# HipGraph/iSpLib

Hardware: AMD Instinct MI355X
Metric: edges_aggregated_per_sec (higher is better)
Workload: dtype f32

## Files before the change

include/isplib_hip.h:

```cpp
#ifndef ISPLIB_HIP_H
#define ISPLIB_HIP_H

#include <stddef.h>
#include <stdint.h>

#ifdef __cplusplus
extern "C" {
#endif

#define ISPLIB_HIP_ABI_VERSION 1
#define ISPLIB_MAX_SLICES 4096

#define ISPLIB_VOP_COPY_RHS 0x2
#define ISPLIB_ROP_NOOP     0x00
#define ISPLIB_SOP_COPY     0x100
#define ISPLIB_VSC_MUL      0x1000
#define ISPLIB_VSC_MEAN     0x3000
#define ISPLIB_AOP_ADD      0x10000
#define ISPLIB_AOP_MAX      0x20000
#define ISPLIB_AOP_MIN      0x30000
#define ISPLIB_MSG_SPMM_SUM  (ISPLIB_VOP_COPY_RHS | ISPLIB_ROP_NOOP | ISPLIB_SOP_COPY | ISPLIB_VSC_MUL  | ISPLIB_AOP_ADD)
#define ISPLIB_MSG_SPMM_MEAN (ISPLIB_VOP_COPY_RHS | ISPLIB_ROP_NOOP | ISPLIB_SOP_COPY | ISPLIB_VSC_MEAN | ISPLIB_AOP_ADD)
#define ISPLIB_MSG_SPMM_MAX  (ISPLIB_VOP_COPY_RHS | ISPLIB_ROP_NOOP | ISPLIB_SOP_COPY | ISPLIB_VSC_MUL  | ISPLIB_AOP_MAX)
#define ISPLIB_MSG_SPMM_MIN  (ISPLIB_VOP_COPY_RHS | ISPLIB_ROP_NOOP | ISPLIB_SOP_COPY | ISPLIB_VSC_MUL  | ISPLIB_AOP_MIN)
// ... 37 lines not shown
          (k % 2) == 0 && (ldy % 2) == 0 && (ldz % 2) == 0;
}
#define ISPLIB_MINMAX_BW_PAIRS_END     0xFFFFFFFEu
#define ISPLIB_MINMAX_BW_KEYS_MAX      0xFFFFFFFEu
#define ISPLIB_OWNER_WORLD_MAX         64
static inline int isplib_product_within(int64_t rows, int64_t k, uint64_t most) {
   return rows <= 0 || k <= 0 || (uint64_t)k <= most / (uint64_t)rows;
}
static inline int isplib_owner_exchange_serves(int64_t m, int64_t k, int world, const int64_t *cuts) {
   if (world < 1 || world > ISPLIB_OWNER_WORLD_MAX || m < 0 || k < 0 || !isplib_product_within(m, k, ISPLIB_MINMAX_BW_PAIRS_END - 1u)) return 0;
   for (int p = 0; p < world; p++)
      if (cuts[p + 1] < cuts[p] || !isplib_product_within(cuts[p + 1] - cuts[p], k, ISPLIB_MINMAX_BW_KEYS_MAX)) return 0;
   return 1;
}

int isplib_hip_set_empty_row(int init);
int isplib_hip_get_empty_row(void);

int fusedMM_csr_hip(int32_t imessage, int64_t m, int64_t n, int64_t k,
                    float alpha, int64_t nnz, int64_t rows, int64_t cols,
                    const float *val ,
                    const int64_t *indx ,
                    const int64_t *pntrb ,
                    const int64_t *pntre ,
                    const float *x , int64_t ldx,
                    const float *y , int64_t ldy, float beta,
                    float *z , int64_t ldz,
                    int64_t *z_arg , void *stream);

enum isplib_sop_udef {
   ISPLIB_SOP_NONE = 0,
   ISPLIB_SOP_SIGMOID = 1,
   ISPLIB_SOP_ONE_MINUS_SIGMOID = 2,
   ISPLIB_SOP_TDIST = 3,
   ISPLIB_SOP_SCALE = 4,
   ISPLIB_SOP_EXP = 5,
   ISPLIB_SOP_LEAKY_EXP = 6
};
int fusedMM_csr_udef_hip(int32_t imessage, int64_t m, int64_t n, int64_t k, float alpha, int64_t nnz,
                         int64_t rows, int64_t cols, const float *val ,
                         const int64_t *indx, const int64_t *pntrb, const int64_t *pntre,
                         const float *x , int64_t ldx,
                         const float *y , int64_t ldy, float beta,
                         float *z , int64_t ldz, int64_t *z_arg ,
                         int sop_udef , float sop_param, void *stream);

int fusedMM_csr_udef_tasks_hip(int32_t imessage, int64_t m, int64_t n, int64_t k, int64_t nnz,
                               const float *val, const int64_t *indx, const int32_t *indx32 ,
                               const int64_t *pntrb, const int64_t *pntre,
                               const float *x, int64_t ldx, int64_t n_tasks, const int32_t *task_row,
                               const int64_t *task_b, const int32_t *task_len, const int32_t *seg_off,
                               int slices, const int64_t *lane_off_host ,
                               const float *y, int64_t ldy, float *z, int64_t ldz, int64_t *z_arg,
                               int sop_udef, float sop_param, void *workspace, size_t workspace_bytes,
                               void *stream);

size_t isplib_spmm_slices_bytes(int64_t m, int slices);
int    isplib_spmm_slices_build_hip(int64_t m, int64_t n, int64_t nnz,
                                    const int64_t *pntrb, const int64_t *pntre,
                                    const int64_t *indx, int slices,
                                    int64_t *sliceptr ,
                                    int32_t *unsorted_flag ,
                                    void *stream);
size_t isplib_spmm_sliced_workspace_bytes(int32_t imessage, int64_t m, int64_t k, int slices);
int    fusedMM_csr_sliced_hip(int32_t imessage, int64_t m, int64_t n, int64_t k,
                              int64_t nnz, const float *val, const int64_t *indx,
                              const int64_t *pntrb, const int64_t *pntre,
                              const int64_t *sliceptr, int slices,
                              const float *y, int64_t ldy, float *z, int64_t ldz,
                              int64_t *z_arg, void *workspace,
                              size_t workspace_bytes, void *stream);

int    fusedMM_csr_sliced_phase_hip(int32_t imessage, int64_t m, int64_t n, int64_t k,
                                    int64_t nnz, const float *val, const int64_t *indx,
                                    const int64_t *pntrb, const int64_t *pntre,
                                    const int64_t *sliceptr, int slices,
                                    int slice_first, int slice_count, int combine,
                                    const float *y, int64_t ldy, float *z, int64_t ldz,
                                    int64_t *z_arg, void *workspace,
                                    size_t workspace_bytes, void *stream);

typedef struct isplib_task_plan_info {
   int64_t n_tasks;
   int64_t lane_off[9];
   int32_t slices, chunk, short_row, reserved;
} isplib_task_plan_info;

size_t isplib_spmm_tasks_plan_workspace_bytes(int64_t m, int slices);
int    isplib_spmm_tasks_count_hip(int64_t m, const int64_t *pntrb, const int64_t *pntre,
                                   const int64_t *sliceptr, int slices, int chunk, int short_row,
                                   int32_t *seg_off , void *workspace,
                                   size_t workspace_bytes, isplib_task_plan_info *info ,
                                   void *stream);
int    isplib_spmm_tasks_fill_hip(int64_t m, const int64_t *pntrb, const int64_t *pntre,
                                  const int64_t *sliceptr, const isplib_task_plan_info *info,
                                  const int32_t *seg_off, int32_t *task_row, int64_t *task_b,
                                  int32_t *task_len, void *stream);
size_t isplib_spmm_tasks_workspace_bytes(int32_t imessage, int64_t n_tasks, int64_t k);
int    isplib_pack_indices_hip(int64_t nnz, const int64_t *indx, int32_t *indx32, void *stream);
int    fusedMM_csr_tasks_hip(int32_t imessage, int64_t m, int64_t n, int64_t k, int64_t nnz,
                             const float *val, const int64_t *indx, const int32_t *indx32,
                             const int64_t *pntrb, const int64_t *pntre,
                             int64_t n_tasks, const int32_t *task_row,
                             const int64_t *task_b, const int32_t *task_len,
                             const int32_t *seg_off, int slices,
                             const int64_t *lane_off_host ,
                             const float *y, int64_t ldy, float *z, int64_t ldz,
                             int64_t *z_arg, void *workspace, size_t workspace_bytes,
                             void *stream);

typedef struct isplib_epilogue {
   const float *row_scale;
   const float *self;
   int64_t      ld_self;
   const float *bias;
   int          relu;
} isplib_epilogue;
int    fusedMM_csr_tasks_epilogue_hip(int32_t imessage, int64_t m, int64_t n, int64_t k, int64_t nnz,
                                      const float *val, const int64_t *indx, const int32_t *indx32,
                                      const int64_t *pntrb, const int64_t *pntre,
                                      int64_t n_tasks, const int32_t *task_row,
                                      const int64_t *task_b, const int32_t *task_len,
                                      const int32_t *seg_off, int slices,
                                      const int64_t *lane_off_host ,
                                      const float *y, int64_t ldy, float *z, int64_t ldz,
                                      void *workspace, size_t workspace_bytes,
                                      const isplib_epilogue *epilogue ,
                                      void *stream);

int    isplib_row_scale_hip(int64_t n, int64_t k, const float *x , int64_t ldx, const float *scale ,
                            float *y , int64_t ldy, void *stream);
size_t isplib_masked_scale_colsum_workspace_bytes(int64_t n, int64_t k);
int    isplib_masked_scale_colsum_hip(int64_t n, int64_t k, const float *dz, int64_t lddz, const float *out ,
                                      int64_t ldo, const float *scale , float *gy ,
                                      int64_t ldgy, float *grad_bias , void *workspace, size_t workspace_bytes,
                                      void *stream);

typedef struct isplib_stream_plan {
   int64_t rows, cols;
   int32_t slices, gens, waves_per_gen, rows_per_wave, streams , chunk ;
   int64_t n_steps, n_parts, n_hub;
   const int32_t *words;
   const float   *vals;
   const int64_t *wave_step_off;
   const int32_t *wave_row;
   const int32_t *wave_part;
   const int32_t *hub_row;
   const int32_t *hub_off;
   const int32_t *perm;
} isplib_stream_plan;
int  isplib_stream_plan_build_hip(int64_t m, int64_t n, int64_t nnz, const int64_t *rowptr, const int64_t *col,
                                  const float *val, int streams, int slices, int chunk, int waves_per_gen,
                                  isplib_stream_plan *out , void *stream);
int  isplib_stream_plan_set_values_hip(isplib_stream_plan *plan, const float *val , void *stream);
void isplib_stream_plan_free(isplib_stream_plan *plan);
int    isplib_spmm_stream_geometry(int streams, int *rows_per_wave , int *waves_resident );
int    isplib_suggest_stream(int64_t m, int64_t n, int64_t nnz, int64_t k, int *streams, int *slices, int *chunk);
int    isplib_suggest_stream_weighted(int64_t m, int64_t n, int64_t nnz, int64_t k, int weighted, int *streams, int *slices, int *chunk);
int    isplib_spmm_stream_minmax_geometry(int streams , int *rows_per_wave , int *waves_resident );
int    isplib_suggest_stream_minmax(int64_t m, int64_t n, int64_t nnz, int64_t k, int *streams, int *slices, int *chunk);
int    isplib_stream_plan_build_minmax_hip(int64_t m, int64_t n, int64_t nnz, const int64_t *rowptr, const int64_t *col,
                                           const float *val, int streams, int slices, int chunk, int waves_per_gen,
                                           isplib_stream_plan *out , void *stream);
size_t isplib_spmm_stream_minmax_workspace_bytes(const isplib_stream_plan *plan);
int    fusedMM_csr_stream_minmax_hip(int32_t imessage , int64_t m, int64_t n, int64_t k,
                                     int64_t nnz, const int64_t *pntrb, const int64_t *pntre,
                                     const isplib_stream_plan *plan ,
                                     const float *y, int64_t ldy, float *z, int64_t ldz, int64_t *z_arg,
                                     void *workspace, size_t workspace_bytes, void *stream);
size_t isplib_spmm_stream_workspace_bytes(const isplib_stream_plan *plan);
int    fusedMM_csr_stream_hip(int32_t imessage , int64_t m, int64_t n, int64_t k,
                              int64_t nnz, const int64_t *pntrb, const int64_t *pntre,
                              const isplib_stream_plan *plan ,
                              const float *y, int64_t ldy, float *z, int64_t ldz,
                              void *workspace, size_t workspace_bytes,
                              const isplib_epilogue *epilogue , void *stream);
#define ISPLIB_DTYPE_BF16 1
#define ISPLIB_DTYPE_F16  2
int    fusedMM_csr_stream16_hip(int32_t imessage , int dtype, int64_t m, int64_t n, int64_t k,
                                int64_t nnz, const int64_t *pntrb, const int64_t *pntre,
                                const isplib_stream_plan *plan ,
                                const void *y, int64_t ldy, void *z, int64_t ldz,
                                void *workspace, size_t workspace_bytes, void *stream);
static inline int isplib_stream16_native_pays(int streams, int weighted) {
   (void)streams; (void)weighted;
   return 0;
}
int    isplib_stream16_auto(int streams, int weighted);
int    fusedMM_csr_rows16_hip(int32_t imessage , int dtype ,
                              int64_t m, int64_t n, int64_t k, int64_t nnz, const float *val ,
                              const int64_t *indx, const int64_t *pntrb, const int64_t *pntre,
                              const int32_t *row_order , const void *y, int64_t ldy, void *z, int64_t ldz, void *stream);
static inline int isplib_rows16_native_pays(int64_t n, int64_t ldy, int ordered, int weighted) {
   const int beyond = n > 0 && ldy > 0 && (double)n * (double)ldy * 2.0 > 256.0 * 1048576.0;
   (void)weighted;
   return (beyond || !ordered) ? 1 : 0;
}
int    isplib_rows16_auto(int64_t n, int64_t ldy, int ordered, int weighted);
int    isplib_rows16_domain(int64_t n, int64_t k, int64_t ldy, int64_t ldz);
int    fusedMM_csr_rows16_colscale_hip(int32_t imessage , int dtype ,
                                       int64_t m, int64_t n, int64_t k, int64_t nnz, const float *col_scale ,
                                       const int64_t *indx, const int64_t *pntrb, const int64_t *pntre,
                                       const int32_t *row_order , const void *y, int64_t ldy, void *z, int64_t ldz, void *stream);
static inline int isplib_rows16_colscale_native_pays(int64_t n, int64_t ldy, int ordered) {
   const int beyond = n > 0 && ldy > 0 && (double)n * (double)ldy * 2.0 > 256.0 * 1048576.0;
   return (beyond || !ordered) ? 1 : 0;
}
int    isplib_rows16_colscale_auto(int64_t n, int64_t ldy, int ordered);
typedef struct isplib_epilogue16 {
   const float *row_scale;
   const float *self_scale;
   const float *bias;
   int          relu;
} isplib_epilogue16;
int    fusedMM_csr_rows16_epilogue_hip(int dtype , int64_t m, int64_t n, int64_t k, int64_t nnz,
                                       const float *col_scale , const int64_t *indx, const int64_t *pntrb,
                                       const int64_t *pntre, const int32_t *row_order , const void *y, int64_t ldy, void *z,
                                       int64_t ldz, const isplib_epilogue16 *epilogue , void *stream);
static inline int isplib_rows16_gcn_native_pays(int64_t n, int64_t ldy, int ordered) {
   (void)ordered;
   return (n > 0 && ldy > 0 && (double)n * (double)ldy * 2.0 > 256.0 * 1048576.0) ? 1 : 0;
}
int    isplib_rows16_gcn_auto(int64_t n, int64_t ldy, int ordered);
size_t isplib_masked_colsum16_workspace_bytes(int64_t n, int64_t k);
int    isplib_masked_colsum16_hip(int dtype, int64_t n, int64_t k, const void *dz, int64_t lddz, const void *out , int64_t ldo,
                                  void *g , int64_t ldg, float *grad_bias , void *workspace,
                                  size_t workspace_bytes, void *stream);
int    fusedMM_csr_rows16_minmax_hip(int32_t imessage , int dtype ,
                                     int64_t m, int64_t n, int64_t k, int64_t nnz, const float *val ,
                                     const int64_t *indx, const int64_t *pntrb, const int64_t *pntre,
                                     const int32_t *row_order , const void *y, int64_t ldy, void *z, int64_t ldz,
                                     int64_t *z_arg , int64_t ldarg, void *stream);
static inline int isplib_rows16_minmax_native_pays(int64_t n, int64_t ldy, int ordered, int weighted, int want_arg) {
   const int beyond = n > 0 && ldy > 0 && (double)n * (double)ldy * 2.0 > 256.0 * 1048576.0;
   (void)ordered; (void)weighted; (void)want_arg;
   return beyond ? 1 : 0;
}
int    isplib_rows16_minmax_auto(int64_t n, int64_t ldy, int ordered, int weighted, int want_arg);
int    isplib_sddmm_csr_rows16_hip(int dtype , int64_t m, int64_t n, int64_t k, int64_t nnz,
                                   const int64_t *indx, const int64_t *pntrb, const int64_t *pntre,
                                   const int32_t *row_order , const void *y, int64_t ldy,
                                   const void *g, int64_t ldg, int mean, float *dval, void *stream);
static inline int isplib_sddmm_rows16_serves(int64_t n, int64_t k, int64_t ldy, int64_t ldg) {
   return k <= ISPLIB_SDDMM_TASKS_K_MAX && isplib_rows16_serves(n, k, ldy, ldg);
}
static inline int isplib_sddmm_rows16_native_pays(int64_t n, int64_t ldy, int ordered) {
   const int beyond = n > 0 && ldy > 0 && (double)n * (double)ldy * 2.0 > 256.0 * 1048576.0;
   (void)ordered;
   return beyond ? 1 : 0;
}
int    isplib_sddmm_rows16_auto(int64_t n, int64_t ldy, int ordered);
static inline int isplib_attention_serves(int64_t rows_gathered, int64_t k, int64_t ld) {
   return k >= 1 && k <= ISPLIB_ATTENTION_K_MAX && ld >= k && rows_gathered < (1LL << 31) && isplib_dense_in_descriptor(rows_gathered, ld);
}
int    isplib_attention_domain(int64_t rows_gathered, int64_t k, int64_t ld);
int    isplib_attention_csr_hip(int64_t m, int64_t n, int64_t k, int64_t nnz, const int64_t *indx, const int64_t *pntrb,
                                const int64_t *pntre, const float *x, int64_t ldx, const float *y, int64_t ldy, float scale,
                                float *z, int64_t ldz, float *lse , void *stream);
int    isplib_attention_bw_rows_hip(int64_t m, int64_t n, int64_t k, int64_t nnz, const int64_t *indx, const int64_t *pntrb,
                                    const int64_t *pntre, const float *x, int64_t ldx, const float *y, int64_t ldy, float scale,
                                    const float *g, int64_t ldg, const float *z, int64_t ldz, const float *lse, float *dx,
                                    int64_t lddx, float *dsum , void *stream);
int    isplib_attention_bw_cols_hip(int64_t m, int64_t n, int64_t k, int64_t nnz, const int64_t *row_t, const int64_t *colb,
                                    const int64_t *cole, const float *x, int64_t ldx, const float *y, int64_t ldy, float scale,
                                    const float *g, int64_t ldg, const float *lse, const float *dsum, float *dy, int64_t lddy,
                                    void *stream);
#define ISPLIB_ATTENTION16_K_MIN       8
#define ISPLIB_ATTENTION16_K_MAX       512
static inline int isplib_attention16_serves(int64_t rows_gathered, int64_t k, int64_t ld) {
   return k >= ISPLIB_ATTENTION16_K_MIN && k <= ISPLIB_ATTENTION16_K_MAX && (k % 2) == 0 && (ld % 2) == 0 && ld >= k &&
          rows_gathered < (1LL << 31) && isplib_rows_within(rows_gathered, ld, 2ull * ISPLIB_DENSE_BYTES_MAX);
}
int    isplib_attention16_domain(int64_t rows_gathered, int64_t k, int64_t ld);
int    isplib_attention16_csr_hip(int dtype , int64_t m, int64_t n, int64_t k, int64_t nnz,
                                  const int64_t *indx, const int64_t *pntrb, const int64_t *pntre, const void *x, int64_t ldx,
                                  const void *y, int64_t ldy, float scale, void *z, int64_t ldz, float *lse , void *stream);
int    isplib_attention16_bw_rows_hip(int dtype, int64_t m, int64_t n, int64_t k, int64_t nnz, const int64_t *indx, const int64_t *pntrb,
                                      const int64_t *pntre, const void *x, int64_t ldx, const void *y, int64_t ldy, float scale,
                                      const void *g, int64_t ldg, const float *lse, void *dx, int64_t lddx, float *dsum ,
                                      void *stream);
int    isplib_attention16_bw_cols_hip(int dtype, int64_t m, int64_t n, int64_t k, int64_t nnz, const int64_t *row_t, const int64_t *colb,
                                      const int64_t *cole, const void *x, int64_t ldx, const void *y, int64_t ldy, float scale,
                                      const void *g, int64_t ldg, const float *lse, const float *dsum, void *dy, int64_t lddy,
                                      void *stream);
static inline int isplib_attention16_native_pays(int64_t rows_gathered, int64_t ld) {
   return (rows_gathered > 0 && ld > 0) ? 1 : 0;
}
int    isplib_attention16_auto(int64_t rows_gathered, int64_t ld);
#define ISPLIB_STAGE_OFF   0
#define ISPLIB_STAGE_FORCE 1
#define ISPLIB_STAGE_AUTO  2
#define ISPLIB_STREAM_STAGE_PITCH      512
#define ISPLIB_STREAM_STAGE_BYTES_MAX  (1u << 30)
#define ISPLIB_STREAM_STAGE_MIN_DEGREE 128
static inline int isplib_stream_stage_panel(uint64_t y_addr, int64_t ldy, int64_t c0, int64_t k, int streams, int64_t n, int64_t nnz,
                                            uint64_t room_bytes, int mode) {
   const uint64_t addr = y_addr + 4u * (uint64_t)c0;
   if (mode == ISPLIB_STAGE_OFF || streams != 4 || n <= 0 || c0 < 0 || c0 + 64 > k) return 0;
   if (((uint64_t)ldy * 4u) % ISPLIB_STREAM_STAGE_PITCH != 0 || (addr & 255u) != 0) return 0;
   if ((uint64_t)n > ISPLIB_STREAM_STAGE_BYTES_MAX / ISPLIB_STREAM_STAGE_PITCH || (uint64_t)n * ISPLIB_STREAM_STAGE_PITCH > room_bytes) return 0;
   if (mode == ISPLIB_STAGE_FORCE) return 1;
   if ((addr & 256u) == 0 || ((((uint64_t)ldy * 4u) % 1024u) == 0 && (addr & 512u) != 0)) return 0;
   return nnz / n >= ISPLIB_STREAM_STAGE_MIN_DEGREE;
}

int    isplib_fusedmm_stream_geometry(int streams, int *rows_per_wave , int *waves_resident );
// ... 102 lines not shown
```

isplib_amd/cabi.py:

```python
from __future__ import annotations

import ctypes
import os
from typing import Optional

import torch

from . import _lib

MSG_SPMM_SUM = 0x2 | 0x00 | 0x100 | 0x1000 | 0x10000
MSG_SPMM_MEAN = 0x2 | 0x00 | 0x100 | 0x3000 | 0x10000
MSG_SPMM_MAX = 0x2 | 0x00 | 0x100 | 0x1000 | 0x20000
MSG_SPMM_MIN = 0x2 | 0x00 | 0x100 | 0x1000 | 0x30000
MESSAGE = {"sum": MSG_SPMM_SUM, "add": MSG_SPMM_SUM, "mean": MSG_SPMM_MEAN, "max": MSG_SPMM_MAX, "min": MSG_SPMM_MIN}

SUCCESS, FAIL, NOT_ENOUGH_MEM, NO_OPT_IMPL, HIP_ERROR = 0, 1, -1, 128, 256
UNDEFINED_USER_FUNCTION = 64
ISPLIB_SUCCESS, ISPLIB_FAIL, ISPLIB_NOT_ENOUGH_MEM, ISPLIB_NO_OPT_IMPL, ISPLIB_HIP_ERROR = SUCCESS, FAIL, NOT_ENOUGH_MEM, NO_OPT_IMPL, HIP_ERROR

DENSE_BYTES_MAX = 7 * 2 ** 29
DENSE_OOB_OFFSET = 15 * 2 ** 28
STREAM_N_END = 2 ** 24
STREAM_LDY_END = 2 ** 22
STREAM_NNZ_END = 2 ** 31
STREAM_MINMAX_BYTES_END = 2 ** 31
K_MIN = 4
SDDMM_TASKS_K_MAX = 1024
MINMAX_BW_PAIRS_END = 2 ** 32 - 2
MINMAX_BW_KEYS_MAX = 2 ** 32 - 2
OWNER_WORLD_MAX = 64
DTYPE_BF16, DTYPE_F16 = 1, 2


def stream16_serves(n: int, k: int, ldy: int, ldz: int, nnz: int) -> bool:
    return (k >= K_MIN and n < STREAM_N_END and ldy < STREAM_LDY_END and nnz < STREAM_NNZ_END and
            (n <= 0 or n * ldy * 2 <= DENSE_BYTES_MAX) and k % 2 == 0 and ldy % 2 == 0 and ldz % 2 == 0)


def stream16_native_pays(streams: int, weighted: bool) -> bool:
    return False


ROWS16_K_MIN, ROWS16_K_END = 8, 2 ** 24


def rows16_serves(n: int, k: int, ldy: int, ldz: int) -> bool:
    return (ROWS16_K_MIN <= k < ROWS16_K_END and n < 2 ** 31 and (n <= 0 or n * ldy * 2 <= DENSE_BYTES_MAX) and
            k % 2 == 0 and ldy % 2 == 0 and ldz % 2 == 0)


def rows16_native_pays(n: int, ldy: int, ordered: bool, weighted: bool) -> bool:
    beyond = n > 0 and ldy > 0 and n * ldy * 2 > (256 << 20)
    return bool(beyond or not ordered)


def rows16_minmax_native_pays(n: int, ldy: int, ordered: bool, weighted: bool, want_arg: bool) -> bool:
    return bool(n > 0 and ldy > 0 and n * ldy * 2 > (256 << 20))


def rows16_colscale_native_pays(n: int, ldy: int, ordered: bool) -> bool:
    beyond = n > 0 and ldy > 0 and n * ldy * 2 > (256 << 20)
    return bool(beyond or not ordered)


def rows16_gcn_native_pays(n: int, ldy: int, ordered: bool) -> bool:
    return bool(n > 0 and ldy > 0 and n * ldy * 2 > (256 << 20))


def sddmm_rows16_serves(n: int, k: int, ldy: int, ldg: int) -> bool:
    return k <= SDDMM_TASKS_K_MAX and rows16_serves(n, k, ldy, ldg)


def sddmm_rows16_native_pays(n: int, ldy: int, ordered: bool) -> bool:
    return bool(n > 0 and ldy > 0 and n * ldy * 2 > (256 << 20))


ATTENTION_K_MAX = 512


def attention_serves(rows_gathered: int, k: int, ld: int) -> bool:
    return (1 <= k <= ATTENTION_K_MAX and ld >= k and rows_gathered < 2 ** 31 and
            (rows_gathered <= 0 or rows_gathered * ld * 4 <= DENSE_BYTES_MAX))


ATTENTION16_K_MIN, ATTENTION16_K_MAX = 8, 512


def attention16_serves(rows_gathered: int, k: int, ld: int) -> bool:
    return (ATTENTION16_K_MIN <= k <= ATTENTION16_K_MAX and k % 2 == 0 and ld % 2 == 0 and ld >= k and rows_gathered < 2 ** 31 and
            (rows_gathered <= 0 or rows_gathered * ld * 2 <= DENSE_BYTES_MAX))


def attention16_native_pays(rows_gathered: int, ld: int) -> bool:
    return bool(rows_gathered > 0 and ld > 0)


def owner_exchange_serves(m: int, k: int, world: int, cuts) -> bool:
    if not 1 <= world <= OWNER_WORLD_MAX or m < 0 or k < 0 or m * k >= MINMAX_BW_PAIRS_END:
        return False
    return all(cuts[p + 1] >= cuts[p] and (cuts[p + 1] - cuts[p]) * k <= MINMAX_BW_KEYS_MAX for p in range(world))


def scatter_keys_serves(total: int, n: int, k: int) -> bool:
    return 0 <= total < MINMAX_BW_PAIRS_END and n >= 0 and k >= 0 and n * k <= MINMAX_BW_KEYS_MAX

VOP = {"copy_lhs": 0x1, "copy_rhs": 0x2, "add": 0x3, "subl": 0x4, "subr": 0x5, "max": 0x6, "min": 0x7, "udef": 0xF}
ROP = {"noop": 0x00, "dot": 0x10, "add_lhs": 0x20, "add_rhs": 0x30, "norml": 0x40, "normr": 0x50, "udef": 0xF0}
SOP = {"noop": 0x000, "copy": 0x100, "udef": 0xF00}
VSC = {"noop": 0x0000, "mul": 0x1000, "add": 0x2000, "mean": 0x3000, "udef": 0xF000}
AOP = {"add": 0x10000, "max": 0x20000, "min": 0x30000, "udef": 0xF0000}
SOP_UDEF = {"none": 0, "sigmoid": 1, "one_minus_sigmoid": 2, "tdist": 3, "scale": 4, "exp": 5, "leaky_exp": 6}
PATTERNS = {
    "spmm": (MSG_SPMM_SUM, "none"),
    "sigmoid_embedding": (VOP["copy_rhs"] | ROP["dot"] | SOP["udef"] | VSC["mul"] | AOP["add"], "sigmoid"),
    "tdist_embedding": (VOP["subr"] | ROP["normr"] | SOP["udef"] | VSC["mul"] | AOP["add"], "tdist"),
    "attention_sum": (VOP["copy_rhs"] | ROP["dot"] | SOP["udef"] | VSC["mul"] | AOP["add"], "leaky_exp"),
}

EXPORTS = (
    "isplib_hip_abi_version", "isplib_hip_last_error", "isplib_hip_set_empty_row", "isplib_hip_get_empty_row", "fusedMM_csr_hip", "performDummySpMM_hip",
    "isplib_spmm_minmax_bw_hip", "isplib_sddmm_csr_hip", "isplib_csr_row_ids_hip",
    "isplib_csr2csc_workspace_bytes", "isplib_csr2csc_hip",
    "isplib_spmm_slices_bytes", "isplib_spmm_slices_build_hip", "isplib_spmm_sliced_workspace_bytes",
    "fusedMM_csr_sliced_hip", "fusedMM_csr_sliced_phase_hip", "isplib_hip_tune",
    "isplib_spmm_tasks_workspace_bytes", "fusedMM_csr_tasks_hip",
    "isplib_spmm_tasks_plan_workspace_bytes", "isplib_spmm_tasks_count_hip", "isplib_spmm_tasks_fill_hip",
    "isplib_sddmm_csr_tasks_hip", "fusedMM_csr_tasks_epilogue_hip", "fusedMM_csr_udef_hip", "fusedMM_csr_udef_tasks_hip", "isplib_pack_indices_hip",
    "isplib_suggest_slices", "isplib_graph_create", "isplib_graph_set_slices", "isplib_graph_set_values", "isplib_graph_spmm", "isplib_graph_spmm_backward",
    "isplib_graph_destroy", "isplib_suggest_slices_whole_rows", "isplib_graph_sddmm",
    "fusedMM_csr_stream_hip", "isplib_spmm_stream_workspace_bytes", "isplib_spmm_stream_geometry", "isplib_suggest_stream", "isplib_suggest_stream_weighted", "isplib_stream_plan_build_hip", "isplib_stream_plan_build_minmax_hip", "fusedMM_csr_stream_minmax_hip", "isplib_spmm_stream_minmax_geometry", "isplib_suggest_stream_minmax", "isplib_spmm_stream_minmax_workspace_bytes", "isplib_stream_plan_set_values_hip", "isplib_stream_plan_free", "isplib_spmm_minmax_bw_det_hip", "isplib_spmm_minmax_bw_workspace_bytes", "isplib_scatter_rows_det_hip",
    "isplib_minmax_bw_bucket_workspace_bytes", "isplib_minmax_bw_bucket_hip", "isplib_scatter_keys_workspace_bytes", "isplib_scatter_keys_det_hip",
    "isplib_fusedmm_stream_geometry", "isplib_suggest_fusedmm_stream", "isplib_stream_plan_build_fusedmm_hip", "fusedMM_csr_udef_stream_hip",
    "isplib_row_scale_hip", "isplib_masked_scale_colsum_hip", "isplib_masked_scale_colsum_workspace_bytes",
    "fusedMM_csr_ordered_hip", "isplib_community_order_hip", "isplib_community_order_workspace_bytes", "isplib_order_locality_hip",
    "isplib_graph_set_row_order", "isplib_plain_panels",
    "fusedMM_csr_stream16_hip", "isplib_stream16_auto",
    "fusedMM_csr_rows16_hip", "isplib_rows16_auto", "isplib_rows16_domain",
    "fusedMM_csr_rows16_minmax_hip", "isplib_rows16_minmax_auto",
    "fusedMM_csr_rows16_colscale_hip", "isplib_rows16_colscale_auto",
    "fusedMM_csr_rows16_epilogue_hip", "isplib_rows16_gcn_auto", "isplib_masked_colsum16_hip", "isplib_masked_colsum16_workspace_bytes",
    "isplib_sddmm_csr_rows16_hip", "isplib_sddmm_rows16_auto",
    "isplib_attention_csr_hip", "isplib_attention_bw_rows_hip", "isplib_attention_bw_cols_hip", "isplib_attention_domain",
    "isplib_attention16_csr_hip", "isplib_attention16_bw_rows_hip", "isplib_attention16_bw_cols_hip", "isplib_attention16_domain",
    "isplib_attention16_auto",
)

EXP_EXPORTS = ("fusedMM_csr_sweep_hip", "isplib_spmm_sweep_workspace_bytes", "isplib_spmm_sweep_resident_waves",
               "fusedMM_csr_hybrid_hip", "isplib_spmm_hybrid_geometry", "isplib_spmm_hybrid_workspace_bytes", "isplib_sddmm_stream_hip",
               "isplib_hip_tune_experimental")

_i64, _f32, _vp, _i32 = ctypes.c_int64, ctypes.c_float, ctypes.c_void_p, ctypes.c_int32


class Epilogue(ctypes.Structure):
    _fields_ = [("row_scale", ctypes.c_void_p), ("self", ctypes.c_void_p), ("ld_self", ctypes.c_int64),
                ("bias", ctypes.c_void_p), ("relu", ctypes.c_int)]


class TaskPlanInfo(ctypes.Structure):
    _fields_ = [("n_tasks", ctypes.c_int64), ("lane_off", ctypes.c_int64 * 9), ("slices", ctypes.c_int32),
                ("chunk", ctypes.c_int32), ("short_row", ctypes.c_int32), ("reserved", ctypes.c_int32)]


class SweepPlanStruct(ctypes.Structure):
    _fields_ = [("rows", ctypes.c_int64), ("slices", ctypes.c_int32), ("gens", ctypes.c_int32),
                ("waves_per_gen", ctypes.c_int32), ("rows_per_wave", ctypes.c_int32), ("n_tasks", ctypes.c_int64),
                ("n_parts", ctypes.c_int64), ("n_hub", ctypes.c_int64), ("wave_row", ctypes.c_void_p),
                ("wave_part", ctypes.c_void_p), ("wave_task_off", ctypes.c_void_p), ("task_b", ctypes.c_void_p),
                ("task_meta", ctypes.c_void_p), ("hub_row", ctypes.c_void_p), ("hub_off", ctypes.c_void_p)]


class StreamPlanStruct(ctypes.Structure):
    _fields_ = [("rows", ctypes.c_int64), ("cols", ctypes.c_int64), ("slices", ctypes.c_int32), ("gens", ctypes.c_int32),
                ("waves_per_gen", ctypes.c_int32), ("rows_per_wave", ctypes.c_int32), ("streams", ctypes.c_int32),
                ("chunk", ctypes.c_int32), ("n_steps", ctypes.c_int64), ("n_parts", ctypes.c_int64), ("n_hub", ctypes.c_int64),
                ("words", ctypes.c_void_p), ("vals", ctypes.c_void_p), ("wave_step_off", ctypes.c_void_p),
                ("wave_row", ctypes.c_void_p), ("wave_part", ctypes.c_void_p),
                ("hub_row", ctypes.c_void_p), ("hub_off", ctypes.c_void_p), ("perm", ctypes.c_void_p)]


class HybridPlanStruct(ctypes.Structure):
    _fields_ = [("cold", StreamPlanStruct), ("table_rows", ctypes.c_int32), ("hot_cap", ctypes.c_int32), ("n_hot_steps", ctypes.c_int64),
                ("hot_rows", ctypes.c_void_p), ("hot_words", ctypes.c_void_p), ("hot_step_off", ctypes.c_void_p),
                ("hot_perm", ctypes.c_void_p)]


_sigs_set = False


def lib() -> ctypes.CDLL:
    global _sigs_set
    L = _lib.cdll()
    if not _sigs_set:
        L.isplib_hip_abi_version.restype = ctypes.c_int
        L.isplib_hip_last_error.restype = ctypes.c_char_p
        L.fusedMM_csr_hip.restype = ctypes.c_int
        L.fusedMM_csr_hip.argtypes = [_i32, _i64, _i64, _i64, _f32, _i64, _i64, _i64, _vp, _vp, _vp, _vp,
                                      _vp, _i64, _vp, _i64, _f32, _vp, _i64, _vp, _vp]
        L.fusedMM_csr_udef_hip.restype = ctypes.c_int
        L.fusedMM_csr_udef_hip.argtypes = [_i32, _i64, _i64, _i64, _f32, _i64, _i64, _i64, _vp, _vp, _vp, _vp,
                                           _vp, _i64, _vp, _i64, _f32, _vp, _i64, _vp, ctypes.c_int, _f32, _vp]
        L.fusedMM_csr_udef_tasks_hip.restype = ctypes.c_int
        L.fusedMM_csr_udef_tasks_hip.argtypes = [_i32, _i64, _i64, _i64, _i64, _vp, _vp, _vp, _vp, _vp, _vp, _i64, _i64, _vp, _vp,
                                                 _vp, _vp, ctypes.c_int, _vp, _vp, _i64, _vp, _i64, _vp, ctypes.c_int, _f32,
                                                 _vp, ctypes.c_size_t, _vp]
        L.performDummySpMM_hip.restype = None
        L.performDummySpMM_hip.argtypes = [_i64, _vp]
        L.isplib_spmm_minmax_bw_hip.restype = ctypes.c_int
        L.isplib_spmm_minmax_bw_hip.argtypes = [_i64, _i64, _i64, _i64, _vp, _vp, _vp, _vp, _vp, _vp, _vp, _vp]
        L.isplib_sddmm_csr_hip.restype = ctypes.c_int
        L.isplib_sddmm_csr_hip.argtypes = [_i64, _i64, _vp, _vp, _vp, _vp, _i64, _vp, _i64, ctypes.c_int, _vp, _vp]
        L.isplib_csr_row_ids_hip.restype = ctypes.c_int
        L.isplib_csr_row_ids_hip.argtypes = [_i64, _i64, _vp, _vp, _vp]
        L.isplib_csr2csc_workspace_bytes.restype = ctypes.c_size_t
        L.isplib_csr2csc_workspace_bytes.argtypes = [_i64, _i64, _i64]
        L.isplib_csr2csc_hip.restype = ctypes.c_int
        L.isplib_csr2csc_hip.argtypes = [_i64, _i64, _i64, _vp, _vp, _vp, ctypes.c_int, _vp, _vp, _vp, _vp,
                                         _vp, ctypes.c_size_t, _vp]
        L.isplib_spmm_slices_bytes.restype = ctypes.c_size_t
        L.isplib_spmm_slices_bytes.argtypes = [_i64, ctypes.c_int]
        L.isplib_spmm_slices_build_hip.restype = ctypes.c_int
        L.isplib_spmm_slices_build_hip.argtypes = [_i64, _i64, _i64, _vp, _vp, _vp, ctypes.c_int, _vp, _vp, _vp]
        L.isplib_spmm_sliced_workspace_bytes.restype = ctypes.c_size_t
        L.isplib_spmm_sliced_workspace_bytes.argtypes = [_i32, _i64, _i64, ctypes.c_int]
        L.fusedMM_csr_sliced_hip.restype = ctypes.c_int
        L.fusedMM_csr_sliced_hip.argtypes = [_i32, _i64, _i64, _i64, _i64, _vp, _vp, _vp, _vp, _vp, ctypes.c_int,
                                             _vp, _i64, _vp, _i64, _vp, _vp, ctypes.c_size_t, _vp]
        L.fusedMM_csr_sliced_phase_hip.restype = ctypes.c_int
        L.fusedMM_csr_sliced_phase_hip.argtypes = [_i32, _i64, _i64, _i64, _i64, _vp, _vp, _vp, _vp, _vp, ctypes.c_int,
                                                   ctypes.c_int, ctypes.c_int, ctypes.c_int, _vp, _i64, _vp, _i64, _vp,
                                                   _vp, ctypes.c_size_t, _vp]
        L.isplib_spmm_tasks_workspace_bytes.restype = ctypes.c_size_t
        L.isplib_spmm_tasks_workspace_bytes.argtypes = [_i32, _i64, _i64]
        L.fusedMM_csr_tasks_hip.restype = ctypes.c_int
        L.isplib_pack_indices_hip.restype = ctypes.c_int
        L.isplib_pack_indices_hip.argtypes = [_i64, _vp, _vp, _vp]
        L.fusedMM_csr_tasks_hip.argtypes = [_i32, _i64, _i64, _i64, _i64, _vp, _vp, _vp, _vp, _vp, _i64, _vp, _vp, _vp, _vp,
                                            ctypes.c_int, _vp, _vp, _i64, _vp, _i64, _vp, _vp, ctypes.c_size_t, _vp]
        L.isplib_spmm_tasks_plan_workspace_bytes.restype = ctypes.c_size_t
        L.isplib_spmm_tasks_plan_workspace_bytes.argtypes = [_i64, ctypes.c_int]
        L.isplib_spmm_tasks_count_hip.restype = ctypes.c_int
        L.isplib_spmm_tasks_count_hip.argtypes = [_i64, _vp, _vp, _vp, ctypes.c_int, ctypes.c_int, ctypes.c_int, _vp, _vp,
                                                  ctypes.c_size_t, ctypes.POINTER(TaskPlanInfo), _vp]
        L.isplib_spmm_tasks_fill_hip.restype = ctypes.c_int
        L.isplib_spmm_tasks_fill_hip.argtypes = [_i64, _vp, _vp, _vp, ctypes.POINTER(TaskPlanInfo), _vp, _vp, _vp, _vp, _vp]
        L.isplib_sddmm_csr_tasks_hip.restype = ctypes.c_int
        L.isplib_sddmm_csr_tasks_hip.argtypes = [_i64, _i64, _i64, _vp, _vp, _vp, _vp, _i64, _vp, _vp, _vp, _vp, _vp, _i64, _vp,
                                                 _i64, ctypes.c_int, _vp, _vp]
        L.fusedMM_csr_tasks_epilogue_hip.restype = ctypes.c_int
        L.fusedMM_csr_tasks_epilogue_hip.argtypes = [_i32, _i64, _i64, _i64, _i64, _vp, _vp, _vp, _vp, _vp, _i64, _vp, _vp, _vp, _vp,
                                                     ctypes.c_int, _vp, _vp, _i64, _vp, _i64, _vp, ctypes.c_size_t,
                                                     ctypes.POINTER(Epilogue), _vp]
        L.isplib_suggest_slices.restype = ctypes.c_int
        L.isplib_suggest_slices.argtypes = [_i64, _i64, _i64, _i64, ctypes.c_int]
        L.isplib_graph_create.restype = ctypes.c_int
        L.isplib_graph_create.argtypes = [_i64, _i64, _i64, _vp, _vp, _vp, ctypes.POINTER(_vp)]
        L.isplib_graph_set_slices.restype = ctypes.c_int
        L.isplib_graph_set_slices.argtypes = [_vp, ctypes.c_int]
        L.isplib_graph_set_values.restype = ctypes.c_int
        L.isplib_graph_set_values.argtypes = [_vp, _vp]
        L.isplib_graph_spmm.restype = ctypes.c_int
        L.isplib_graph_spmm.argtypes = [_vp, _i32, _i64, _vp, _i64, _vp, _i64, _vp, _vp]
        L.isplib_graph_spmm_backward.restype = ctypes.c_int
        L.isplib_graph_spmm_backward.argtypes = [_vp, ctypes.c_int, _i64, _vp, _i64, _vp, _i64, _vp]
        L.isplib_suggest_slices_whole_rows.restype = ctypes.c_int
        L.isplib_suggest_slices_whole_rows.argtypes = [_i64, _i64, _i64, _i64]
        L.isplib_graph_sddmm.restype = ctypes.c_int
        L.isplib_graph_sddmm.argtypes = [_vp, ctypes.c_int, _i64, _vp, _i64, _vp, _i64, _vp, _vp]
        L.isplib_graph_destroy.restype = None
        L.isplib_graph_destroy.argtypes = [_vp]
        L.isplib_hip_tune.restype = ctypes.c_int
        L.isplib_hip_tune.argtypes = [ctypes.c_int, ctypes.c_int]
        L.isplib_spmm_minmax_bw_workspace_bytes.restype = ctypes.c_size_t
        L.isplib_spmm_minmax_bw_workspace_bytes.argtypes = [_i64, _i64, _i64]
        L.isplib_spmm_minmax_bw_det_hip.restype = ctypes.c_int
        L.isplib_spmm_minmax_bw_det_hip.argtypes = [_i64, _i64, _i64, _i64, _vp, _vp, _vp, _vp, _vp, _vp, _vp, _vp, ctypes.c_size_t, _vp]
        L.isplib_fusedmm_stream_geometry.restype = ctypes.c_int
        L.isplib_fusedmm_stream_geometry.argtypes = [ctypes.c_int, ctypes.POINTER(ctypes.c_int), ctypes.POINTER(ctypes.c_int)]
        L.isplib_suggest_fusedmm_stream.restype = ctypes.c_int
        L.isplib_suggest_fusedmm_stream.argtypes = [_i32, _i64, _i64, _i64, _i64] + [ctypes.POINTER(ctypes.c_int)] * 3
        L.isplib_stream_plan_build_fusedmm_hip.restype = ctypes.c_int
        L.isplib_stream_plan_build_fusedmm_hip.argtypes = [_i64, _i64, _i64, _vp, _vp, ctypes.c_int, ctypes.c_int, ctypes.c_int, ctypes.c_int,
                                                           ctypes.POINTER(StreamPlanStruct), _vp]
        L.fusedMM_csr_udef_stream_hip.restype = ctypes.c_int
        L.fusedMM_csr_udef_stream_hip.argtypes = [_i32, _i64, _i64, _i64, _i64, _vp, _vp, ctypes.POINTER(StreamPlanStruct), _vp, _i64, _vp, _i64,
                                                  _vp, _i64, ctypes.c_int, _f32, _vp, ctypes.c_size_t, _vp]
        L.isplib_row_scale_hip.restype = ctypes.c_int
        L.isplib_row_scale_hip.argtypes = [_i64, _i64, _vp, _i64, _vp, _vp, _i64, _vp]
        L.isplib_masked_scale_colsum_workspace_bytes.restype = ctypes.c_size_t
        L.isplib_masked_scale_colsum_workspace_bytes.argtypes = [_i64, _i64]
        L.isplib_masked_scale_colsum_hip.restype = ctypes.c_int
        L.isplib_masked_scale_colsum_hip.argtypes = [_i64, _i64, _vp, _i64, _vp, _i64, _vp, _vp, _i64, _vp, _vp, ctypes.c_size_t, _vp]
        L.isplib_scatter_rows_det_hip.restype = ctypes.c_int
        L.isplib_scatter_rows_det_hip.argtypes = [_i64, _i64, _i64, _i64, _vp, _vp, _vp, _vp, ctypes.c_size_t, _vp]
        L.isplib_minmax_bw_bucket_workspace_bytes.restype = ctypes.c_size_t
        L.isplib_minmax_bw_bucket_workspace_bytes.argtypes = [_i64, _i64, ctypes.c_int]
        L.isplib_minmax_bw_bucket_hip.restype = ctypes.c_int
        L.isplib_minmax_bw_bucket_hip.argtypes = [_i64, _i64, _i64, _i64, _vp, _vp, _vp, _vp, ctypes.c_int, ctypes.POINTER(_i64), _vp, _vp, _vp,
                                                  _vp, ctypes.c_size_t, _vp]
        L.isplib_scatter_keys_workspace_bytes.restype = ctypes.c_size_t
        L.isplib_scatter_keys_workspace_bytes.argtypes = [_i64, _i64, _i64]
        L.isplib_scatter_keys_det_hip.restype = ctypes.c_int
        L.isplib_scatter_keys_det_hip.argtypes = [_i64, _i64, _i64, _vp, _vp, _vp, _vp, ctypes.c_size_t, _vp]
        L.isplib_stream_plan_build_hip.restype = ctypes.c_int
        L.isplib_stream_plan_build_hip.argtypes = [_i64, _i64, _i64, _vp, _vp, _vp, ctypes.c_int, ctypes.c_int, ctypes.c_int, ctypes.c_int,
                                                   ctypes.POINTER(StreamPlanStruct), _vp]
        L.isplib_stream_plan_build_minmax_hip.restype = ctypes.c_int
        L.isplib_stream_plan_build_minmax_hip.argtypes = [_i64, _i64, _i64, _vp, _vp, _vp, ctypes.c_int, ctypes.c_int, ctypes.c_int, ctypes.c_int,
                                                          ctypes.POINTER(StreamPlanStruct), _vp]
        L.isplib_spmm_stream_minmax_geometry.restype = ctypes.c_int
        L.isplib_spmm_stream_minmax_geometry.argtypes = [ctypes.c_int, ctypes.POINTER(ctypes.c_int), ctypes.POINTER(ctypes.c_int)]
        L.isplib_suggest_stream_minmax.restype = ctypes.c_int
        L.isplib_suggest_stream_minmax.argtypes = [_i64, _i64, _i64, _i64, ctypes.POINTER(ctypes.c_int), ctypes.POINTER(ctypes.c_int), ctypes.POINTER(ctypes.c_int)]
        L.isplib_spmm_stream_minmax_workspace_bytes.restype = ctypes.c_size_t
        L.isplib_spmm_stream_minmax_workspace_bytes.argtypes = [ctypes.POINTER(StreamPlanStruct)]
        L.fusedMM_csr_stream_minmax_hip.restype = ctypes.c_int
        L.fusedMM_csr_stream_minmax_hip.argtypes = [_i32, _i64, _i64, _i64, _i64, _vp, _vp, ctypes.POINTER(StreamPlanStruct), _vp, _i64,
                                                    _vp, _i64, _vp, _vp, ctypes.c_size_t, _vp]
        L.isplib_stream_plan_set_values_hip.restype = ctypes.c_int
        L.isplib_stream_plan_set_values_hip.argtypes = [ctypes.POINTER(StreamPlanStruct), _vp, _vp]
        L.isplib_stream_plan_free.restype = None
        L.isplib_stream_plan_free.argtypes = [ctypes.POINTER(StreamPlanStruct)]
        L.isplib_community_order_workspace_bytes.restype = ctypes.c_size_t
        L.isplib_community_order_workspace_bytes.argtypes = [_i64, _i64]
        L.isplib_community_order_hip.restype = ctypes.c_int
        L.isplib_community_order_hip.argtypes = [_i64, _i64, _vp, _vp, ctypes.c_int, ctypes.c_int, _vp, _vp, ctypes.POINTER(ctypes.c_int), _vp,
                                                 ctypes.c_size_t, _vp]
        L.isplib_order_locality_hip.restype = ctypes.c_int
        L.isplib_order_locality_hip.argtypes = [_i64, _i64, _vp, _vp, _vp, _i64, ctypes.POINTER(ctypes.c_double), _vp, ctypes.c_size_t, _vp]
        L.isplib_graph_set_row_order.restype = ctypes.c_int
        L.isplib_graph_set_row_order.argtypes = [_vp, _vp, _vp]
        L.fusedMM_csr_ordered_hip.restype = ctypes.c_int
        L.fusedMM_csr_ordered_hip.argtypes = [_i32, _i64, _i64, _i64, _i64, _vp, _vp, _vp, _vp, _vp, _vp, _i64, _vp, _i64, _vp, _vp]
        L.isplib_plain_panels.restype = ctypes.c_int
        L.isplib_plain_panels.argtypes = [_i64, _i64]
        L.isplib_suggest_stream.restype = ctypes.c_int
        L.isplib_suggest_stream.argtypes = [_i64, _i64, _i64, _i64, ctypes.POINTER(ctypes.c_int), ctypes.POINTER(ctypes.c_int), ctypes.POINTER(ctypes.c_int)]
        L.isplib_suggest_stream_weighted.restype = ctypes.c_int
        L.isplib_suggest_stream_weighted.argtypes = [_i64, _i64, _i64, _i64, ctypes.c_int, ctypes.POINTER(ctypes.c_int), ctypes.POINTER(ctypes.c_int), ctypes.POINTER(ctypes.c_int)]
        L.isplib_spmm_stream_geometry.restype = ctypes.c_int
        L.isplib_spmm_stream_geometry.argtypes = [ctypes.c_int, ctypes.POINTER(ctypes.c_int), ctypes.POINTER(ctypes.c_int)]
        L.isplib_spmm_stream_workspace_bytes.restype = ctypes.c_size_t
        L.isplib_spmm_stream_workspace_bytes.argtypes = [ctypes.POINTER(StreamPlanStruct)]
        L.fusedMM_csr_stream_hip.restype = ctypes.c_int
        L.fusedMM_csr_stream_hip.argtypes = [_i32, _i64, _i64, _i64, _i64, _vp, _vp, ctypes.POINTER(StreamPlanStruct), _vp, _i64,
                                             _vp, _i64, _vp, ctypes.c_size_t, ctypes.POINTER(Epilogue), _vp]
        L.fusedMM_csr_stream16_hip.restype = ctypes.c_int
        L.fusedMM_csr_stream16_hip.argtypes = [_i32, ctypes.c_int, _i64, _i64, _i64, _i64, _vp, _vp, ctypes.POINTER(StreamPlanStruct), _vp, _i64,
                                               _vp, _i64, _vp, ctypes.c_size_t, _vp]
        L.isplib_stream16_auto.restype = ctypes.c_int
        L.isplib_stream16_auto.argtypes = [ctypes.c_int, ctypes.c_int]
        L.fusedMM_csr_rows16_hip.restype = ctypes.c_int
        L.fusedMM_csr_rows16_hip.argtypes = [_i32, ctypes.c_int, _i64, _i64, _i64, _i64, _vp, _vp, _vp, _vp, _vp, _vp, _i64, _vp, _i64, _vp]
        L.isplib_rows16_auto.restype = ctypes.c_int
        L.isplib_rows16_auto.argtypes = [_i64, _i64, ctypes.c_int, ctypes.c_int]
        L.isplib_rows16_domain.restype = ctypes.c_int
        L.isplib_rows16_domain.argtypes = [_i64, _i64, _i64, _i64]
        L.fusedMM_csr_rows16_minmax_hip.restype = ctypes.c_int
        L.fusedMM_csr_rows16_minmax_hip.argtypes = [_i32, ctypes.c_int, _i64, _i64, _i64, _i64, _vp, _vp, _vp, _vp, _vp, _vp, _i64, _vp, _i64, _vp, _i64, _vp]
        L.isplib_rows16_minmax_auto.restype = ctypes.c_int
        L.isplib_rows16_minmax_auto.argtypes = [_i64, _i64, ctypes.c_int, ctypes.c_int, ctypes.c_int]
        L.fusedMM_csr_rows16_colscale_hip.restype = ctypes.c_int
        L.fusedMM_csr_rows16_colscale_hip.argtypes = [_i32, ctypes.c_int, _i64, _i64, _i64, _i64, _vp, _vp, _vp, _vp, _vp, _vp, _i64, _vp, _i64, _vp]
        L.isplib_rows16_colscale_auto.restype = ctypes.c_int
        L.isplib_rows16_colscale_auto.argtypes = [_i64, _i64, ctypes.c_int]
        L.fusedMM_csr_rows16_epilogue_hip.restype = ctypes.c_int
        L.fusedMM_csr_rows16_epilogue_hip.argtypes = [ctypes.c_int, _i64, _i64, _i64, _i64, _vp, _vp, _vp, _vp, _vp, _vp, _i64, _vp, _i64, _vp, _vp]
        L.isplib_rows16_gcn_auto.restype = ctypes.c_int
        L.isplib_rows16_gcn_auto.argtypes = [_i64, _i64, ctypes.c_int]
        L.isplib_masked_colsum16_workspace_bytes.restype = ctypes.c_size_t
        L.isplib_masked_colsum16_workspace_bytes.argtypes = [_i64, _i64]
        L.isplib_masked_colsum16_hip.restype = ctypes.c_int
        L.isplib_masked_colsum16_hip.argtypes = [ctypes.c_int, _i64, _i64, _vp, _i64, _vp, _i64, _vp, _i64, _vp, _vp, ctypes.c_size_t, _vp]
        L.isplib_sddmm_csr_rows16_hip.restype = ctypes.c_int
        L.isplib_sddmm_csr_rows16_hip.argtypes = [ctypes.c_int, _i64, _i64, _i64, _i64, _vp, _vp, _vp, _vp, _vp, _i64, _vp, _i64, ctypes.c_int, _vp, _vp]
        L.isplib_sddmm_rows16_auto.restype = ctypes.c_int
        L.isplib_sddmm_rows16_auto.argtypes = [_i64, _i64, ctypes.c_int]
        L.isplib_attention_domain.restype = ctypes.c_int
        L.isplib_attention_domain.argtypes = [_i64, _i64, _i64]
        L.isplib_attention_csr_hip.restype = ctypes.c_int
        L.isplib_attention_csr_hip.argtypes = [_i64, _i64, _i64, _i64, _vp, _vp, _vp, _vp, _i64, _vp, _i64, _f32, _vp, _i64, _vp, _vp]
        L.isplib_attention_bw_rows_hip.restype = ctypes.c_int
        L.isplib_attention_bw_rows_hip.argtypes = [_i64, _i64, _i64, _i64, _vp, _vp, _vp, _vp, _i64, _vp, _i64, _f32, _vp, _i64, _vp, _i64, _vp,
                                                   _vp, _i64, _vp, _vp]
        L.isplib_attention_bw_cols_hip.restype = ctypes.c_int
        L.isplib_attention_bw_cols_hip.argtypes = [_i64, _i64, _i64, _i64, _vp, _vp, _vp, _vp, _i64, _vp, _i64, _f32, _vp, _i64, _vp, _vp, _vp,
                                                   _i64, _vp]
        L.isplib_attention16_domain.restype = ctypes.c_int
        L.isplib_attention16_domain.argtypes = [_i64, _i64, _i64]
        L.isplib_attention16_auto.restype = ctypes.c_int
        L.isplib_attention16_auto.argtypes = [_i64, _i64]
        L.isplib_attention16_csr_hip.restype = ctypes.c_int
        L.isplib_attention16_csr_hip.argtypes = [ctypes.c_int, _i64, _i64, _i64, _i64, _vp, _vp, _vp, _vp, _i64, _vp, _i64, _f32, _vp, _i64, _vp, _vp]
        L.isplib_attention16_bw_rows_hip.restype = ctypes.c_int
        L.isplib_attention16_bw_rows_hip.argtypes = [ctypes.c_int, _i64, _i64, _i64, _i64, _vp, _vp, _vp, _vp, _i64, _vp, _i64, _f32, _vp, _i64, _vp,
                                                     _vp, _i64, _vp, _vp]
        L.isplib_attention16_bw_cols_hip.restype = ctypes.c_int
        L.isplib_attention16_bw_cols_hip.argtypes = [ctypes.c_int, _i64, _i64, _i64, _i64, _vp, _vp, _vp, _vp, _i64, _vp, _i64, _f32, _vp, _i64, _vp,
                                                     _vp, _vp, _i64, _vp]
        _sigs_set = True
    return L


_exp = None


def exp_lib() -> ctypes.CDLL:
    global _exp
    if _exp is None:
        lib()
        path = os.path.join(os.path.dirname(_lib.CABI_PATH), "libisplib_hip_exp.so")
        if not os.path.exists(path):
            raise ImportError(f"isplib_amd: '{os.path.basename(path)}' not found; build it with `make -C isplib_amd/csrc`")
        L = ctypes.CDLL(path, mode=ctypes.RTLD_GLOBAL)
        L.isplib_hip_tune_experimental.restype = ctypes.c_int
        L.isplib_hip_tune_experimental.argtypes = [ctypes.c_int, ctypes.c_int]
        L.isplib_spmm_hybrid_geometry.restype = ctypes.c_int
        L.isplib_spmm_hybrid_geometry.argtypes = [ctypes.c_int] + [ctypes.POINTER(ctypes.c_int)] * 4
        L.isplib_spmm_hybrid_workspace_bytes.restype = ctypes.c_size_t
        L.isplib_spmm_hybrid_workspace_bytes.argtypes = [ctypes.POINTER(HybridPlanStruct)]
        L.fusedMM_csr_hybrid_hip.restype = ctypes.c_int
        L.fusedMM_csr_hybrid_hip.argtypes = [_i32, _i64, _i64, _i64, _i64, _vp, _vp, ctypes.POINTER(HybridPlanStruct), _vp, _i64, _vp, _i64,
                                             _vp, ctypes.c_size_t, _vp, _vp]
        L.isplib_sddmm_stream_hip.restype = ctypes.c_int
        L.isplib_sddmm_stream_hip.argtypes = [_i64, _i64, _i64, _i64, _vp, _vp, ctypes.POINTER(StreamPlanStruct), _vp, _i64, _vp, _i64,
                                              ctypes.c_int, _vp, _vp]
        L.isplib_spmm_sweep_resident_waves.restype = ctypes.c_int
        L.isplib_spmm_sweep_resident_waves.argtypes = [_i32, _i64, ctypes.c_int]
        L.isplib_spmm_sweep_workspace_bytes.restype = ctypes.c_size_t
        L.isplib_spmm_sweep_workspace_bytes.argtypes = [_i32, ctypes.POINTER(SweepPlanStruct), _i64]
        L.fusedMM_csr_sweep_hip.restype = ctypes.c_int
        L.fusedMM_csr_sweep_hip.argtypes = [_i32, _i64, _i64, _i64, _i64, _vp, _vp, _vp, _vp, _vp, ctypes.POINTER(SweepPlanStruct),
                                            _vp, _i64, _vp, _i64, _vp, _vp, ctypes.c_size_t, ctypes.POINTER(Epilogue), _vp]
        _exp = L
    return _exp


def last_error() -> str:
    return lib().isplib_hip_last_error().decode()


class IsplibError(RuntimeError):

    def __init__(self, status: int, what: str, message: str):
        super().__init__(f"{what} failed with status {status}: {message}")
        self.status = int(status)


def _check(status: int, what: str) -> None:
    if status != 0:
        raise IsplibError(status, what, last_error())


def _ptr(t: Optional[torch.Tensor]):
    return None if t is None else ctypes.c_void_p(t.data_ptr())


def _stream(device) -> ctypes.c_void_p:
    return ctypes.c_void_p(torch.cuda.current_stream(device).cuda_stream)
# ... 1204 lines not shown
            dsum.zero_()
        return dx, dsum
    rp = rowptr.data_ptr()
    with torch.cuda.device(x.device):
        st = lib().isplib_attention16_bw_rows_hip(HALF_DTYPES[x.dtype], m, n, k, col.numel(), _ptr(col), ctypes.c_void_p(rp),
                                                  ctypes.c_void_p(rp + 8), _ptr(x), ldx, _ptr(y), ldy, _attn_scale(scale, k), _ptr(g), ldg,
                                                  _ptr(lse), _ptr(dx), lddx, _ptr(dsum), _stream(x.device))
    _check(st, "isplib_attention16_bw_rows_hip")
    return dx, dsum


def attention16_bw_cols(colptr, row_t, x, y, g, lse, dsum, scale: Optional[float] = None, *, out=None, check: bool = True):
    if not isinstance(colptr, torch.Tensor) or colptr.dim() != 1 or colptr.numel() < 1:
        raise ValueError("isplib_amd: `colptr` (n + 1 entries) must be a 1-D tensor")
    n = colptr.numel() - 1
    ldy = _attn16_dense(y, "y", n, None, "one row per column of the sparse operand")
    k = y.size(1)
    if not isinstance(x, torch.Tensor) or x.dim() != 2:
        raise ValueError("isplib_amd: `x` must be a 2-D tensor [m, k]")
    m = x.size(0)
    ldx = _attn16_dense(x, "x", m, k, "y's width", y.dtype)
    ldg = _attn16_dense(g, "g", m, k, "the gradient of z", y.dtype)
    _attn_vector(lse, "lse", m)
    _attn_vector(dsum, "dsum", m)
    colptr, row_t = _attn_structure(colptr, row_t, "colptr", "row_t", m, check)
    if out is not None:
        lddy = _attn16_dense(out, "out", n, k, "dy", y.dtype)
    _attn16_domain(m, k, (ldx, ldg))
    _same_gpu((("x", x), ("y", y), ("g", g), ("lse", lse), ("dsum", dsum), ("colptr", colptr), ("row_t", row_t), ("out", out)))
    if out is None:
        out = torch.empty((n, k), dtype=y.dtype, device=y.device)
        lddy = max(k, 1)
    if n == 0 or k == 0:
        return out
    cp = colptr.data_ptr()
    with torch.cuda.device(y.device):
        st = lib().isplib_attention16_bw_cols_hip(HALF_DTYPES[y.dtype], m, n, k, row_t.numel(), _ptr(row_t), ctypes.c_void_p(cp),
                                                  ctypes.c_void_p(cp + 8), _ptr(x), ldx, _ptr(y), ldy, _attn_scale(scale, k), _ptr(g), ldg,
                                                  _ptr(lse), _ptr(dsum), _ptr(out), lddy, _stream(y.device))
    _check(st, "isplib_attention16_bw_cols_hip")
    return out


def fusedMM_csr_rows16_minmax_hip(imessage: int, rowptr, col, val, order, y, z, z_arg=None, check: bool = True, dtype=None, k=None, ldy=None,
                                  ldz=None, ldarg=None) -> int:
    if ldarg is None:
        m, kk = rowptr.numel() - 1, y.size(1) if k is None else int(k)
        ldarg = 0 if z_arg is None else (z_arg.stride(0) if m > 1 else max(kk, z_arg.stride(0)))
    return _rows16_raw("fusedMM_csr_rows16_minmax_hip", imessage, rowptr, col, val, order, y, z, check, dtype, k, ldy, ldz, _ptr(z_arg), int(ldarg))


def spmm_rows16_minmax(rowptr, col, val, y, reduce: str = "max", order=None, out=None, arg=None, want_arg: bool = True):
    if reduce not in ("max", "min"):
        raise ValueError(f"isplib_amd: spmm_rows16_minmax serves max / min, got '{reduce}' (sum / mean: spmm_rows16)")
    rowptr, col, val, order, out, arg = _rows16_operands(rowptr, col, val, False, y, order, out, arg, want_arg)
    fusedMM_csr_rows16_minmax_hip(MESSAGE[reduce], rowptr, col, val, order, y, out, arg)
    return out, arg


def fusedMM_csr_stream_minmax_hip(imessage: int, rowptr, nnz: int, plan, y, z, z_arg=None, workspace=None, check: bool = True) -> int:
    assert y.is_cuda and y.dtype == torch.float32 and y.dim() == 2 and y.stride(1) == 1
    m, n, k = rowptr.numel() - 1, y.size(0), y.size(1)
    rp = rowptr.data_ptr()
    ps = plan.struct()
    with torch.cuda.device(y.device):
        st = lib().fusedMM_csr_stream_minmax_hip(int(imessage), m, n, k, int(nnz), ctypes.c_void_p(rp), ctypes.c_void_p(rp + 8),
                                                 ctypes.byref(ps), _ptr(y), y.stride(0) if n > 1 else max(k, y.stride(0)), _ptr(z),
                                                 z.stride(0) if m > 1 else max(k, z.stride(0)), _ptr(z_arg), _ptr(workspace),
                                                 0 if workspace is None else workspace.numel(), _stream(y.device))
    if check:
        _check(st, "fusedMM_csr_stream_minmax_hip")
    return st


def spmm_stream_minmax(rowptr, nnz: int, plan, y, reduce: str = "max", workspace=None, want_arg: bool = True):
    rowptr = _dev(rowptr, "rowptr", torch.int64)
    y = y.contiguous()
    m, k = rowptr.numel() - 1, y.size(1)
    out = torch.empty((m, k), dtype=torch.float32, device=y.device)
    arg = torch.empty((m, k), dtype=torch.int64, device=y.device) if want_arg else None
    if workspace is None:
        workspace = plan.workspace(minmax=True)
    fusedMM_csr_stream_minmax_hip(MESSAGE[reduce], rowptr, nnz, plan, y, out, arg, workspace)
    return out, arg


def suggest_stream_minmax(m: int, n: int, nnz: int, k: int):
    st, sl, ch = ctypes.c_int(0), ctypes.c_int(0), ctypes.c_int(0)
    if not lib().isplib_suggest_stream_minmax(int(m), int(n), int(nnz), int(k), ctypes.byref(st), ctypes.byref(sl), ctypes.byref(ch)):
        return None
    return st.value, sl.value, ch.value


def stream_minmax_geometry(streams: int = 4):
    rpw, res = ctypes.c_int(0), ctypes.c_int(0)
    _check(lib().isplib_spmm_stream_minmax_geometry(int(streams), ctypes.byref(rpw), ctypes.byref(res)), "isplib_spmm_stream_minmax_geometry")
    return rpw.value, res.value


def hybrid_geometry(streams: int = 4):
    v = [ctypes.c_int(0) for _ in range(4)]
    _check(exp_lib().isplib_spmm_hybrid_geometry(int(streams), *[ctypes.byref(x) for x in v]), "isplib_spmm_hybrid_geometry")
    return tuple(x.value for x in v)


def fusedMM_csr_hybrid_hip(imessage: int, rowptr, nnz: int, plan, y, z, workspace=None, epilogue=None, check: bool = True) -> int:
    assert y.is_cuda and y.dtype == torch.float32 and y.dim() == 2 and y.stride(1) == 1
    m, n, k = rowptr.numel() - 1, y.size(0), y.size(1)
    rp = rowptr.data_ptr()
    ps = plan.struct()
    with torch.cuda.device(y.device):
        st = exp_lib().fusedMM_csr_hybrid_hip(int(imessage), m, n, k, int(nnz), ctypes.c_void_p(rp), ctypes.c_void_p(rp + 8),
                                          ctypes.byref(ps), _ptr(y), y.stride(0) if n > 1 else max(k, y.stride(0)), _ptr(z),
                                          z.stride(0) if m > 1 else max(k, z.stride(0)), _ptr(workspace),
                                          0 if workspace is None else workspace.numel(),
                                          None if epilogue is None else ctypes.byref(epilogue), _stream(y.device))
    if check:
        _check(st, "fusedMM_csr_hybrid_hip")
    return st


def spmm_hybrid(rowptr, nnz: int, plan, y, reduce: str = "sum", workspace=None, row_scale=None, self_term=None, bias=None, relu=False):
    rowptr = _dev(rowptr, "rowptr", torch.int64)
    y = y.contiguous()
    m, k = rowptr.numel() - 1, y.size(1)
    out = torch.empty((m, k), dtype=torch.float32, device=y.device)
    if workspace is None:
        workspace = plan.workspace()
    ep = None
    if row_scale is not None or self_term is not None or bias is not None or relu:
        ep = Epilogue(None if row_scale is None else row_scale.data_ptr(), None if self_term is None else self_term.data_ptr(),
                      k if self_term is None else self_term.stride(0), None if bias is None else bias.data_ptr(), int(bool(relu)))
    fusedMM_csr_hybrid_hip(MESSAGE[reduce], rowptr, nnz, plan, y, out, workspace, ep)
    return out


def suggest_stream(m: int, n: int, nnz: int, k: int, weighted: bool = False):
    st, sl, ch = ctypes.c_int(0), ctypes.c_int(0), ctypes.c_int(0)
    if not lib().isplib_suggest_stream_weighted(int(m), int(n), int(nnz), int(k), int(bool(weighted)), ctypes.byref(st), ctypes.byref(sl), ctypes.byref(ch)):
        return None
    return st.value, sl.value, ch.value


class _DevView:

    def __init__(self, ptr: int, count: int, typestr: str, owner=None):
        self.__cuda_array_interface__ = {"shape": (count,), "typestr": typestr, "data": (ptr, False), "version": 2}
        self._owner = owner


class NativeStreamPlan:

    def __init__(self, rowptr, col, val, ncols: int, streams: int, slices: int, chunk: int, waves_per_gen: int = 0,
                 minmax: bool = False, fusedmm: bool = False):
        self._s = StreamPlanStruct()
        self.device = col.device
        m = rowptr.numel() - 1
        with torch.cuda.device(col.device):
            if fusedmm:
                _check(lib().isplib_stream_plan_build_fusedmm_hip(m, int(ncols), col.numel(), _ptr(rowptr), _ptr(col), int(streams), int(slices),
                                                                  int(chunk), int(waves_per_gen), ctypes.byref(self._s), _stream(col.device)),
                       "isplib_stream_plan_build_fusedmm_hip")
            elif minmax:
                _check(lib().isplib_stream_plan_build_minmax_hip(m, int(ncols), col.numel(), _ptr(rowptr), _ptr(col), _ptr(val),
                                                                 int(streams), int(slices), int(chunk), int(waves_per_gen), ctypes.byref(self._s),
                                                                 _stream(col.device)), "isplib_stream_plan_build_minmax_hip")
            else:
                _check(lib().isplib_stream_plan_build_hip(m, int(ncols), col.numel(), _ptr(rowptr), _ptr(col), _ptr(val), int(streams),
                                                          int(slices), int(chunk), int(waves_per_gen), ctypes.byref(self._s),
                                                          _stream(col.device)), "isplib_stream_plan_build_hip")
        for name in ("rows", "cols", "slices", "gens", "waves_per_gen", "rows_per_wave", "streams", "n_steps", "n_parts", "n_hub"):
            setattr(self, name, int(getattr(self._s, name)))

    def struct(self):
        return self._s

    def workspace(self, minmax: bool = False):
        L = lib()
        nbytes = (L.isplib_spmm_stream_minmax_workspace_bytes if minmax else L.isplib_spmm_stream_workspace_bytes)(ctypes.byref(self._s))
        return torch.empty(nbytes, dtype=torch.uint8, device=self.device)

    def set_values(self, val):
        with torch.cuda.device(self.device):
            _check(lib().isplib_stream_plan_set_values_hip(ctypes.byref(self._s), _ptr(val), _stream(self.device)), "isplib_stream_plan_set_values_hip")

    def array(self, name: str) -> torch.Tensor:
        nw = self.gens * self.waves_per_gen
        count, typestr = {"words": (self.n_steps * self.streams, "<i4"), "perm": (self.n_steps * self.streams, "<i4"),
                          "vals": (self.n_steps * self.streams, "<f4"), "wave_step_off": (nw + 1, "<i8"),
                          "wave_row": (nw * self.rows_per_wave, "<i4"), "wave_part": (nw * self.rows_per_wave, "<i4"),
                          "hub_row": (self.n_hub, "<i4"), "hub_off": (self.n_hub + 1, "<i4")}[name]
        ptr = getattr(self._s, name)
        if not ptr or count == 0:
            return torch.empty(0, device=self.device)
        return torch.as_tensor(_DevView(ptr, count, typestr), device=self.device).clone()

    def view(self, name: str, dtype: torch.dtype) -> torch.Tensor:
        nw = self.gens * self.waves_per_gen
        count, typestr = {"words": (self.n_steps * self.streams, "<i4"), "perm": (self.n_steps * self.streams, "<i4"),
                          "wave_step_off": (nw + 1, "<i8"), "wave_row": (nw * self.rows_per_wave, "<i4"),
                          "wave_part": (nw * self.rows_per_wave, "<i4"), "hub_row": (self.n_hub, "<i4"),
                          "hub_off": (self.n_hub + 1, "<i4")}[name]
        ptr = getattr(self._s, name)
        if not ptr or count == 0:
            return torch.empty(0, dtype=dtype, device=self.device)
        t = torch.as_tensor(_DevView(ptr, count, typestr, owner=self), device=self.device)
        assert t.dtype == dtype and t.data_ptr() == ptr, "zero-copy view of a library array"
        return t

    def close(self):
        if self._s.words or self._s.wave_row:
            lib().isplib_stream_plan_free(ctypes.byref(self._s))

    def __del__(self):
        try:
            self.close()
        except Exception:
            pass


def stream_geometry(streams: int = 4):
    rpw, res = ctypes.c_int(0), ctypes.c_int(0)
    _check(lib().isplib_spmm_stream_geometry(int(streams), ctypes.byref(rpw), ctypes.byref(res)), "isplib_spmm_stream_geometry")
    return rpw.value, res.value


def sweep_resident_waves(reduce: str, k: int, rows_per_wave: int = 16) -> int:
    return int(exp_lib().isplib_spmm_sweep_resident_waves(MESSAGE[reduce], int(k), int(rows_per_wave)))


class GraphHandle:

    def __init__(self, rowptr, col, val, ncols: int):
        self.rowptr = _dev(rowptr, "rowptr", torch.int64)
        self.col = _dev(col, "col", torch.int64)
        self.val = None if val is None else _dev(val, "val", torch.float32)
        self.m, self.n = self.rowptr.numel() - 1, int(ncols)
        self._cols_ok = None
        self._h = ctypes.c_void_p()
        with torch.cuda.device(self.col.device):
            _check(lib().isplib_graph_create(self.m, self.n, self.col.numel(), _ptr(self.rowptr), _ptr(self.col),
                                             _ptr(self.val), ctypes.byref(self._h)), "isplib_graph_create")

    def set_slices(self, slices: int) -> None:
        _check(lib().isplib_graph_set_slices(self._h, int(slices)), "isplib_graph_set_slices")

    def set_row_order(self, order, order_t=None) -> None:
        self.order = None if order is None else _dev(order, "order", torch.int32)
        self.order_t = None if order_t is None else _dev(order_t, "order_t", torch.int32)
        assert self.order is None or self.order.numel() == self.m
        assert self.order_t is None or self.order_t.numel() == self.n
        _check(lib().isplib_graph_set_row_order(self._h, _ptr(self.order), _ptr(self.order_t)), "isplib_graph_set_row_order")

    def set_values(self, val) -> None:
        self.val = None if val is None else _dev(val, "val", torch.float32)
        assert self.val is None or self.val.numel() == self.col.numel()
        _check(lib().isplib_graph_set_values(self._h, _ptr(self.val)), "isplib_graph_set_values")

    def spmm(self, y: torch.Tensor, reduce: str = "sum"):
        if not (y.is_cuda and y.dtype == torch.float32 and y.dim() == 2 and y.stride(1) == 1 and y.stride(0) >= y.size(1)):
            y = _dev(y, "y", torch.float32)
        k = y.size(1)
        ldy = y.stride(0) if y.size(0) > 1 else max(k, y.stride(0))
        out = torch.empty((self.m, k), dtype=torch.float32, device=y.device)
        arg = torch.empty((self.m, k), dtype=torch.int64, device=y.device) if reduce in ("max", "min") else None
        with torch.cuda.device(y.device):
            _check(lib().isplib_graph_spmm(self._h, MESSAGE[reduce], k, _ptr(y), ldy, _ptr(out), k, _ptr(arg), _stream(y.device)),
                   "isplib_graph_spmm")
        return out, arg

    def spmm_backward(self, dy: torch.Tensor, mean: bool = False) -> torch.Tensor:
        dy = _dev(dy, "dy", torch.float32)
        k = dy.size(1)
        dx = torch.empty((self.n, k), dtype=torch.float32, device=dy.device)
        with torch.cuda.device(dy.device):
            _check(lib().isplib_graph_spmm_backward(self._h, int(bool(mean)), k, _ptr(dy), k, _ptr(dx), k, _stream(dy.device)),
                   "isplib_graph_spmm_backward")
        return dx

    def sddmm(self, y: torch.Tensor, g: torch.Tensor, mean: bool = False, *, out=None, check: bool = True) -> torch.Tensor:
        _, _, out, ldy, ldg = _sddmm_operands(self.rowptr, self.col, y, g, out, False, self.n, "the handle")
        if check and self._cols_ok is None:
            self._cols_ok = self.col.numel() == 0 or (int(self.col.min()) >= 0 and int(self.col.max()) < self.n)
        if check and not self._cols_ok:
            raise ValueError(f"isplib_amd: the handle's column ids must lie in [0, {self.n})")
        k = y.size(1)
        with torch.cuda.device(y.device):
            _check(lib().isplib_graph_sddmm(self._h, int(bool(mean)), k, _ptr(y), ldy, _ptr(g), ldg, _ptr(out), _stream(y.device)),
                   "isplib_graph_sddmm")
        return out

    def close(self) -> None:
        if self._h:
            lib().isplib_graph_destroy(self._h)
            self._h = ctypes.c_void_p()

    def __del__(self):
        try:
            self.close()
        except Exception:
            pass
```

isplib_amd/csrc/common.h:

```cpp
#pragma once
#include <hip/hip_runtime.h>
#include <stdio.h>
#include <string.h>

#include "../../include/isplib_hip.h"

namespace isplib {

char *error_buffer();
int empty_row_init();

int stream_stage_mode();
void stream_stage_report(unsigned panels);

inline void clear_error() { error_buffer()[0] = '\0'; }

inline int fail(int code, const char *msg) {
   snprintf(error_buffer(), 512, "%s", msg);
   return code;
}

inline int fail(int code, const char *entry, const char *msg) {
   snprintf(error_buffer(), 512, "%s: %s", entry, msg);
   return code;
}

inline int hip_fail(hipError_t e, const char *what) {
   snprintf(error_buffer(), 512, "%s: %s", what, hipGetErrorString(e));
   return ISPLIB_HIP_ERROR;
}

__attribute__((noinline)) inline int check_launch(const char *what) {
   const hipError_t e = hipGetLastError();
   return e == hipSuccess ? ISPLIB_SUCCESS : hip_fail(e, what);
}

#define ISPLIB_HIP_TRY(expr)                                        \
   do {                                                             \
      const hipError_t e_ = (expr);                                 \
      if (e_ != hipSuccess) return ::isplib::hip_fail(e_, #expr);   \
   } while (0)

}
```

isplib_amd/csrc/runtime.hip:

```cpp
#include <stdlib.h>
#include <string.h>

#include "common.h"

namespace isplib {
char *error_buffer() {
   static thread_local char buf[512] = {0};
   return buf;
}
}

namespace isplib {
static int g_empty_row = -1;
int empty_row_init() {
   if (g_empty_row < 0) {
      const char *e = getenv("ISPLIB_EMPTY_ROW");
      g_empty_row = (e && (strcmp(e, "init") == 0 || strcmp(e, "1") == 0)) ? 1 : 0;
   }
   return g_empty_row;
}
}

extern "C" int isplib_hip_set_empty_row(int init) {
   isplib::clear_error();
   if (init != 0 && init != 1) return isplib::fail(ISPLIB_FAIL, "isplib_hip_set_empty_row: 0 (zero) or 1 (the launcher's init value)");
   isplib::g_empty_row = init;
   return ISPLIB_SUCCESS;
}
extern "C" int isplib_hip_get_empty_row(void) { return isplib::empty_row_init(); }

namespace isplib {
static int g_stream_stage = -1;
static thread_local unsigned g_stream_stage_last = 0;
int stream_stage_mode() {
   if (g_stream_stage < 0) {
      const char *e = getenv("ISPLIB_STREAM_STAGE");
      g_stream_stage = !e ? ISPLIB_STAGE_AUTO : strcmp(e, "0") == 0 ? ISPLIB_STAGE_OFF : strcmp(e, "1") == 0 ? ISPLIB_STAGE_FORCE : ISPLIB_STAGE_AUTO;
   }
   return g_stream_stage;
}
void stream_stage_report(unsigned panels) { g_stream_stage_last = panels; }
}

extern "C" int isplib_stream_stage_set(int mode) {
   isplib::clear_error();
   if (mode != ISPLIB_STAGE_OFF && mode != ISPLIB_STAGE_FORCE && mode != ISPLIB_STAGE_AUTO) return isplib::fail(ISPLIB_FAIL, "isplib_stream_stage_set: 0 (off), 1 (force) or 2 (auto)");
   isplib::g_stream_stage = mode;
   return ISPLIB_SUCCESS;
}
extern "C" unsigned isplib_stream_stage_last(void) { return isplib::g_stream_stage_last; }

extern "C" int isplib_hip_abi_version(void) { return ISPLIB_HIP_ABI_VERSION; }
extern "C" const char *isplib_hip_last_error(void) { return isplib::error_buffer(); }
```

isplib_amd/csrc/spmm_sweep.hip:

```cpp
#include "sweep_common.h"

namespace isplib {

template <int LPR, bool HAS_VAL, int NVMAX, int NBW, int WGS>
__global__ __launch_bounds__(256, (stream_wgs_per_cu<LPR, NVMAX, WGS>())) void spmm_stream_kernel(const SweepArgs a) {
   using Wave = StreamWave<LPR, NVMAX, NBW>;
   constexpr int WAVES = Wave::WAVES, G = Wave::G, PANEL = Wave::PANEL, U = Wave::U, PER = Wave::PER;
   constexpr int WAVE_FLOATS = NVMAX * PANEL;
   static_assert(NVMAX <= 256 && NVMAX % G == 0, "the local row is the top byte of a word");
   __shared__ __attribute__((aligned(16))) float s_all[WAVES * WAVE_FLOATS];
   Wave sw;
   if (!stream_wave_id(a, sw)) return;
   const int lane = sw.lane;
#ifdef ISPLIB_EXP_WAVE_TIMES
   const unsigned long long t_start = __builtin_amdgcn_s_memtime();
#endif
   float *my = s_all + sw.wave * WAVE_FLOATS;
   for (int i = lane * 4; i < WAVE_FLOATS; i += 256)
      *reinterpret_cast<float4 *>(my + i) = make_float4(0.0f, 0.0f, 0.0f, 0.0f);
   __amdgpu_buffer_rsrc_t rsrc = dense_rsrc(a);
   stream_columns<true>(a, sw);
   float *lane_base = my + sw.lc * 4;
   stream_bounds(a, sw);
   const float *vp = HAS_VAL ? a.vals + sw.s0 * G : nullptr;
   unsigned w1[NBW], w2[NBW];
   float v0[NBW] = {}, v1[NBW] = {};
   v4i_t t[U];
   unsigned la[U];
   const unsigned pad_word = stream_pad_own_row(a, sw);
   stream_load_batch(sw, sw.wp, 0, pad_word, w1);
   if (HAS_VAL) stream_load_batch(sw, vp, 0, 0.0f, v0);
#pragma unroll
   for (int u = 0; u < U; u++) stream_issue<ISPLIB_EXP_GATHER_AUX>(sw, rsrc, w1, u, la[u], t[u]);
   stream_load_batch(sw, sw.wp, 64 * NBW, pad_word, w1);
   if (HAS_VAL) stream_load_batch(sw, vp, 64 * NBW, 0.0f, v1);
   stream_load_batch(sw, sw.wp, 128 * NBW, pad_word, w2);
   unsigned cur = (unsigned)(sw.g * PER * PANEL);
   float acc[4] = {0.0f, 0.0f, 0.0f, 0.0f};
   const int64_t nb = (sw.nwords + 64 * NBW - 1) / (64 * NBW);
#ifdef ISPLIB_EXP_WAVE_TIMES
   const unsigned long long t_loop = __builtin_amdgcn_s_memtime();
#endif
   for (int64_t b = 0; b < nb; b++) {
      float vnext = HAS_VAL ? __shfl(v0[0], sw.g) : 0.0f;
#pragma unroll
      for (int u = 0; u < U; u++) {
         const float vcur = vnext;
         if (HAS_VAL && u + 1 < U) vnext = __shfl(v0[((u + 1) * G) / 64], ((u + 1) * G) % 64 + sw.g);
         if (la[u] != cur) {
            stream_flush(lane_base + cur, acc);
            cur = la[u];
            acc[0] = acc[1] = acc[2] = acc[3] = 0.0f;
         }
#pragma unroll
         for (int v = 0; v < 4; v++) {
            const float x = __int_as_float(t[u][v]);
            acc[v] = HAS_VAL ? fmaf(vcur, x, acc[v]) : acc[v] + x;
         }
         stream_issue<ISPLIB_EXP_GATHER_AUX>(sw, rsrc, w1, u, la[u], t[u]);
      }
#pragma unroll
      for (int q = 0; q < NBW; q++) { w1[q] = w2[q]; v0[q] = v1[q]; }
      stream_load_batch(sw, sw.wp, (b + 3) * 64 * NBW, pad_word, w2);
      if (HAS_VAL) stream_load_batch(sw, vp, (b + 2) * 64 * NBW, 0.0f, v1);
   }
   stream_flush(lane_base + cur, acc);
#ifdef ISPLIB_EXP_WAVE_TIMES
   const unsigned long long t_loop_end = __builtin_amdgcn_s_memtime();
#endif
   int row_[PER], part_[PER];
#pragma unroll
   for (int jj = 0; jj < PER; jj++) {
      row_[jj] = sw.cok ? a.wave_row[(size_t)sw.w * NVMAX + sw.g * PER + jj] : -1;
      part_[jj] = a.wave_part[(size_t)sw.w * NVMAX + sw.g * PER + jj];
   }
#pragma unroll 4
   for (int jj = 0; jj < PER; jj++) {
      const int lrow = sw.g * PER + jj;
      const int row = row_[jj];
      if (row < 0) continue;
      const int part = part_[jj];
      const float4 t4 = *reinterpret_cast<const float4 *>(lane_base + lrow * PANEL);
      float v[4] = {t4.x, t4.y, t4.z, t4.w};
      int bi[4] = {INT_MAX, INT_MAX, INT_MAX, INT_MAX};
      const int c = sw.ccol;
      if (part >= 0) {
         store_tail<4>(a.part_val + (size_t)part * (size_t)a.k + c, v, sw.vfirst);
         continue;
      }
      int64_t arg[4];
      finish_row<OP_ADD>(a, row, c, v, bi, arg);
      store_tail<4>(a.z + (size_t)row * (size_t)a.ldz + c, v, sw.vfirst);
   }
#ifdef ISPLIB_EXP_WAVE_TIMES
   if (a.dbg && lane == 0) {
      a.dbg[(size_t)sw.wl * 4 + 0] = t_start;
      a.dbg[(size_t)sw.wl * 4 + 1] = t_loop;
      a.dbg[(size_t)sw.wl * 4 + 2] = t_loop_end;
      a.dbg[(size_t)sw.wl * 4 + 3] = __builtin_amdgcn_s_memtime();
   }
#endif
}

typedef float v2f_t __attribute__((ext_vector_type(2)));

template <int OP, int LPR, bool HAS_VAL, int NVMAX, int NBW, int WGS, bool ARG>
__global__ __launch_bounds__(256, (stream_wgs_per_cu<LPR, 2 * (NVMAX + 1), WGS>())) void spmm_stream_minmax_kernel(const SweepArgs a) {
   using Wave = StreamWave<LPR, NVMAX, NBW>;
   constexpr int WAVES = Wave::WAVES, G = Wave::G, PANEL = Wave::PANEL, U = Wave::U, PER = Wave::PER;
   constexpr int ROWS = NVMAX + 1;
   constexpr int WAVE_DWORDS = 2 * ROWS * PANEL;
   constexpr int IDX0 = ROWS * PANEL;
   constexpr int NONE = INT_MAX;
   static_assert(ROWS <= 256 && NVMAX % G == 0, "the local row (and the spare row) is the top byte of a word");
   __shared__ __attribute__((aligned(16))) float s_all[WAVES * WAVE_DWORDS];
   Wave sw;
   if (!stream_wave_id(a, sw)) return;
   const int lane = sw.lane;
   float *my = s_all + sw.wave * WAVE_DWORDS;
   for (int i = lane * 4; i < ROWS * PANEL; i += 256)
      *reinterpret_cast<float4 *>(my + i) = make_float4(identity<OP>(), identity<OP>(), identity<OP>(), identity<OP>());
   if (ARG)
      for (int i = lane * 4; i < ROWS * PANEL; i += 256)
         *reinterpret_cast<int4 *>(my + IDX0 + i) = make_int4(INT_MAX, INT_MAX, INT_MAX, INT_MAX);
   __amdgpu_buffer_rsrc_t rsrc = dense_rsrc(a);
   stream_columns<true>(a, sw);
   const unsigned cbyte = sw.cok ? sw.cbyte : 0x80000000u;
   float *lane_base = my + sw.lc * 4;
   int *lane_idx = reinterpret_cast<int *>(my + IDX0) + sw.lc * 4;
   stream_bounds(a, sw);
   const float *vp = HAS_VAL ? a.vals + sw.s0 * G : nullptr;
   const unsigned pad_word = stream_pad_spare_row(a, sw);
   const int g4 = sw.g * 4;
   unsigned w1[NBW], w2[NBW];
   float v0[NBW] = {}, v1[NBW] = {};
   v4i_t t[U];
   unsigned la[U];
   auto fetch = [&](int u, const unsigned (&word_l)[NBW]) {
      return (unsigned)__builtin_amdgcn_ds_bpermute(g4 + (int)(((u * G) % 64) * 4), (int)word_l[(u * G) / 64]);
   };
   auto issue = [&](int u, unsigned word) {
      const unsigned o = __umul24(word, sw.ldyb) + cbyte;
      la[u] = word;
      t[u] = __builtin_amdgcn_raw_buffer_load_b128(rsrc, (int)o, 0, 0);
   };
   stream_load_batch(sw, sw.wp, 0, pad_word, w1);
   if (HAS_VAL) stream_load_batch(sw, vp, 0, 0.0f, v0);
#pragma unroll
   for (int u = 0; u < U; u++) issue(u, fetch(u, w1));
   stream_load_batch(sw, sw.wp, 64 * NBW, pad_word, w1);
   if (HAS_VAL) stream_load_batch(sw, vp, 64 * NBW, 0.0f, v1);
   stream_load_batch(sw, sw.wp, 128 * NBW, pad_word, w2);
   unsigned cur = (unsigned)(sw.g * PER * PANEL);
   unsigned curw = (unsigned)(sw.g * PER) << 24;
   float acc[4];
   int bi[4];
#pragma unroll
   for (int v = 0; v < 4; v++) { acc[v] = identity<OP>(); bi[v] = NONE; }
   auto swap_to = [&](unsigned nxt_word) {
      asm volatile("" : "+v"(nxt_word));
      const unsigned nxt = (nxt_word >> 24) * (unsigned)PANEL;
      curw = nxt_word;
      const float4 o = *reinterpret_cast<const float4 *>(lane_base + nxt);
      if constexpr (ARG) {
         const int4 oi = *reinterpret_cast<const int4 *>(lane_idx + nxt);
         *reinterpret_cast<float4 *>(lane_base + cur) = make_float4(acc[0], acc[1], acc[2], acc[3]);
         *reinterpret_cast<int4 *>(lane_idx + cur) = make_int4(bi[0], bi[1], bi[2], bi[3]);
         bi[0] = oi.x; bi[1] = oi.y; bi[2] = oi.z; bi[3] = oi.w;
      } else {
         *reinterpret_cast<float4 *>(lane_base + cur) = make_float4(acc[0], acc[1], acc[2], acc[3]);
      }
      acc[0] = o.x; acc[1] = o.y; acc[2] = o.z; acc[3] = o.w;
      cur = nxt;
   };
   const int64_t nb = (sw.nwords + 64 * NBW - 1) / (64 * NBW);
   for (int64_t b = 0; b < nb; b++) {
      const int widx0 = (int)(b * (64 * NBW)) + sw.g;
      float vnext = HAS_VAL ? __int_as_float(__builtin_amdgcn_ds_bpermute(g4, __float_as_int(v0[0]))) : 0.0f;
      unsigned wnext = fetch(0, w1);
#pragma unroll
      for (int u = 0; u < U; u++) {
         const float vcur = vnext;
         const unsigned wcur = wnext;
         if (HAS_VAL && u + 1 < U)
            vnext = __int_as_float(__builtin_amdgcn_ds_bpermute(g4 + (int)((((u + 1) * G) % 64) * 4), __float_as_int(v0[((u + 1) * G) / 64])));
         if (u + 1 < U) wnext = fetch(u + 1, w1);
         unsigned long long row_changes;
         asm("v_cmp_ne_u32_sdwa %0, %1, %2 src0_sel:BYTE_3 src1_sel:BYTE_3" : "=s"(row_changes) : "v"(la[u]), "v"(curw));
         if (__builtin_amdgcn_inverse_ballot_w64(row_changes)) swap_to(la[u]);
         const int mark = widx0 + u * G;
         v2f_t x01 = {__int_as_float(t[u][0]), __int_as_float(t[u][1])};
         v2f_t x23 = {__int_as_float(t[u][2]), __int_as_float(t[u][3])};
         if (HAS_VAL) {
            const v2f_t vv = {vcur, vcur};
            x01 *= vv;
            x23 *= vv;
         }
         const float tt[4] = {x01.x, x01.y, x23.x, x23.y};
#pragma unroll
         for (int v = 0; v < 4; v++) {
            const bool win = OP == OP_MAX ? tt[v] > acc[v] : tt[v] < acc[v];
            acc[v] = win ? tt[v] : acc[v];
            if (ARG) bi[v] = win ? mark : bi[v];
         }
         issue(u, wcur);
      }
#pragma unroll
      for (int q = 0; q < NBW; q++) { w1[q] = w2[q]; v0[q] = v1[q]; }
      stream_load_batch(sw, sw.wp, (b + 3) * 64 * NBW, pad_word, w2);
      if (HAS_VAL) stream_load_batch(sw, vp, (b + 2) * 64 * NBW, 0.0f, v1);
   }
   *reinterpret_cast<float4 *>(lane_base + cur) = make_float4(acc[0], acc[1], acc[2], acc[3]);
   if (ARG) *reinterpret_cast<int4 *>(lane_idx + cur) = make_int4(bi[0], bi[1], bi[2], bi[3]);
   const int32_t *ids = a.ids + sw.s0 * G;
   int row_[PER], part_[PER], best_[PER][4];
   float val_[PER][4];
#pragma unroll
   for (int jj = 0; jj < PER; jj++) {
      const int lrow = sw.g * PER + jj;
      row_[jj] = sw.cok ? a.wave_row[(size_t)sw.w * NVMAX + lrow] : -1;
      part_[jj] = a.wave_part[(size_t)sw.w * NVMAX + lrow];
      const float4 t4 = *reinterpret_cast<const float4 *>(lane_base + lrow * PANEL);
      val_[jj][0] = t4.x; val_[jj][1] = t4.y; val_[jj][2] = t4.z; val_[jj][3] = t4.w;
      if constexpr (ARG) {
         const int4 i4 = *reinterpret_cast<const int4 *>(lane_idx + lrow * PANEL);
         best_[jj][0] = i4.x; best_[jj][1] = i4.y; best_[jj][2] = i4.z; best_[jj][3] = i4.w;
      } else {
         best_[jj][0] = best_[jj][1] = best_[jj][2] = best_[jj][3] = INT_MAX;
      }
   }
   if constexpr (ARG) {
#pragma unroll
      for (int jj = 0; jj < PER; jj++)
#pragma unroll
         for (int i = 0; i < 4; i++)
            best_[jj][i] = (row_[jj] >= 0 && (unsigned)best_[jj][i] < (unsigned)sw.nwords) ? ids[best_[jj][i]] : INT_MAX;
   }
#pragma unroll
   for (int jj = 0; jj < PER; jj++) {
      const int row = row_[jj];
      if (row < 0) continue;
      const int c = sw.ccol;
      if (part_[jj] >= 0) {
         const size_t po = (size_t)part_[jj] * (size_t)a.k + c;
         store_tail<4>(a.part_val + po, val_[jj], sw.vfirst);
         if constexpr (ARG) {
#pragma unroll
            for (int i = 0; i < 4; i++) if (i >= sw.vfirst) a.part_idx[po + i] = best_[jj][i];
         }
         continue;
      }
      int64_t arg[4];
      finish_row<OP>(a, row, c, val_[jj], best_[jj], arg);
      store_tail<4>(a.z + (size_t)row * (size_t)a.ldz + c, val_[jj], sw.vfirst);
      if (a.z_arg) {
         int64_t *ar = a.z_arg + (size_t)row * (size_t)a.ldz + c;
#pragma unroll
         for (int i = 0; i < 4; i++) if (i >= sw.vfirst) ar[i] = arg[i];
      }
   }
}


__global__ __launch_bounds__(256) void stream_stage_copy_kernel(const float *__restrict__ y, int64_t ldy, int64_t n, float *__restrict__ dst) {
   const int64_t total = n * 16;
   const int64_t stride = (int64_t)gridDim.x * blockDim.x;
   for (int64_t i = (int64_t)blockIdx.x * blockDim.x + threadIdx.x; i < total; i += stride) {
      const int64_t r = i >> 4;
      const int j = (int)(i & 15) * 4;
      *reinterpret_cast<float4 *>(dst + r * (ISPLIB_STREAM_STAGE_PITCH / 4) + j) = *reinterpret_cast<const float4 *>(y + r * ldy + j);
   }
}

static int launch_stage_copy(const float *y, int64_t ldy, int64_t n, float *dst, hipStream_t st) {
   int64_t blocks = (n * 16 + 255) / 256;
   if (blocks > 4096) blocks = 4096;
   if (blocks <= 0) return ISPLIB_SUCCESS;
   hipLaunchKernelGGL(stream_stage_copy_kernel, dim3((unsigned)blocks), dim3(256), 0, st, y, ldy, n, dst);
   return check_launch("stream_stage_copy_kernel");
}

#ifdef ISPLIB_EXP_WAVE_TIMES
static unsigned long long *g_dbg = nullptr;
static int g_dbg_launch = 0;
#endif
template <int STREAMS, bool HAS_VAL>
static int launch_stream(const SweepArgs &a_in, hipStream_t st) {
   constexpr StreamGeom ge = stream_geom(STREAM_SUM, STREAMS);
   SweepArgs a = a_in;
#ifdef ISPLIB_EXP_WAVE_TIMES
   a.dbg = g_dbg ? g_dbg + (size_t)(g_dbg_launch++ % 4) * (size_t)a.wave_count * 4 : nullptr;
#endif
   const unsigned blocks = (unsigned)((a.wave_count + 3) / 4);
   if (blocks == 0) return ISPLIB_SUCCESS;
   hipLaunchKernelGGL((spmm_stream_kernel<ge.lpr, HAS_VAL, ge.nvmax, ge.nbw, ge.wgs>), dim3(blocks), dim3(256), 0, st, a);
   return check_launch("spmm_stream_kernel");
}

template <int OP, int STREAMS, bool HAS_VAL, bool ARG>
static void launch_minmax_kernel(const SweepArgs &a, unsigned blocks, hipStream_t st) {
   constexpr StreamGeom ge = stream_geom(STREAM_MINMAX, STREAMS);
   hipLaunchKernelGGL((spmm_stream_minmax_kernel<OP, ge.lpr, HAS_VAL, ge.nvmax, ge.nbw, ge.wgs, ARG>), dim3(blocks), dim3(256), 0, st, a);
}

template <int OP, bool HAS_VAL>
static int launch_stream_minmax(const SweepArgs &a, hipStream_t st, int streams) {
   const unsigned blocks = (unsigned)((a.wave_count + 3) / 4);
   if (blocks == 0) return ISPLIB_SUCCESS;
   return with_streams<STREAM_MINMAX>(streams, [&](auto s) {
      if (a.z_arg) launch_minmax_kernel<OP, s(), HAS_VAL, true>(a, blocks, st);
      else launch_minmax_kernel<OP, s(), HAS_VAL, false>(a, blocks, st);
      return check_launch("spmm_stream_minmax_kernel");
   });
}

}

using namespace isplib;


extern "C" int isplib_spmm_stream_geometry(int streams, int *rows_per_wave, int *waves_resident) {
   return stream_geometry("isplib_spmm_stream_geometry", STREAM_SUM, streams, rows_per_wave, waves_resident);
}

extern "C" int isplib_spmm_stream_minmax_geometry(int streams, int *rows_per_wave, int *waves_resident) {
   return stream_geometry("isplib_spmm_stream_minmax_geometry", STREAM_MINMAX, streams, rows_per_wave, waves_resident);
}

extern "C" int isplib_suggest_stream_weighted(int64_t m, int64_t n, int64_t nnz, int64_t k, int weighted, int *streams, int *slices, int *chunk) {
   clear_error();
   if (m <= 0 || n <= 0 || nnz < STREAM_MIN_NNZ) return 0;
   if (!isplib_stream_serves(n, k, k, nnz, 0)) return 0;
   int st = k <= 32 ? 8 : (k <= 64 ? 4 : (k < 128 ? 2 : 4));
   if (weighted && k >= 128 && (k % 128) == 0) st = 2;
   int rpw = 0, resident = 0;
   if (isplib_spmm_stream_geometry(st, &rpw, &resident) != ISPLIB_SUCCESS || rpw <= 0 || resident <= 0) return 0;
   if (!suggest_stream_geom(m, n, nnz, st, rpw, resident, 1.9e6, 3.4, slices, chunk)) {
      if (st != 2 || k < 128) return 0;
      st = 4;
      if (isplib_spmm_stream_geometry(st, &rpw, &resident) != ISPLIB_SUCCESS || rpw <= 0 || resident <= 0) return 0;
      if (!suggest_stream_geom(m, n, nnz, st, rpw, resident, 1.9e6, 3.4, slices, chunk)) return 0;
   }
   if (streams) *streams = st;
   return 1;
}

extern "C" int isplib_suggest_stream(int64_t m, int64_t n, int64_t nnz, int64_t k, int *streams, int *slices, int *chunk) {
   return isplib_suggest_stream_weighted(m, n, nnz, k, 0, streams, slices, chunk);
}

extern "C" int isplib_suggest_stream_minmax(int64_t m, int64_t n, int64_t nnz, int64_t k, int *streams, int *slices, int *chunk) {
   clear_error();
   if (m <= 0 || n <= 0 || nnz < STREAM_MIN_NNZ) return 0;
   if (!isplib_stream_serves(n, k, k, nnz, 1)) return 0;
   const int st = k <= 32 ? 8 : 4;
   int rpw = 0, resident = 0;
   if (isplib_spmm_stream_minmax_geometry(st, &rpw, &resident) != ISPLIB_SUCCESS || rpw <= 0 || resident <= 0) return 0;
   if (!suggest_stream_geom(m, n, nnz, st, rpw, resident, 3.3e6, st == 8 ? 1.7 : 1.17, slices, chunk)) return 0;
   if (streams) *streams = st;
   return 1;
}

extern "C" size_t isplib_spmm_stream_workspace_bytes(const isplib_stream_plan *plan) {
   size_t bytes = stream_parts_bytes(plan);
   if (plan && plan->streams == 4 && plan->cols > 0 && (uint64_t)plan->cols <= (ISPLIB_STREAM_STAGE_BYTES_MAX - ISPLIB_STREAM_STAGE_PITCH) / ISPLIB_STREAM_STAGE_PITCH)
      bytes += (size_t)plan->cols * ISPLIB_STREAM_STAGE_PITCH + ISPLIB_STREAM_STAGE_PITCH;
   return bytes;
}

extern "C" size_t isplib_spmm_stream_minmax_workspace_bytes(const isplib_stream_plan *plan) {
   return 2 * stream_parts_bytes(plan);
}

static int stream_run(int32_t imessage, int64_t m, int64_t n, int64_t k, int64_t nnz, const int64_t *pntrb, const int64_t *pntre,
                      const isplib_stream_plan *plan, const float *y, int64_t ldy, float *z, int64_t ldz, int64_t *z_arg,
                      void *workspace, size_t workspace_bytes, const isplib_epilogue *ep, void *stream) {
   clear_error();
   const char *entry = "fusedMM_csr_stream_hip";
   const bool mm = imessage == ISPLIB_MSG_SPMM_MAX || imessage == ISPLIB_MSG_SPMM_MIN;
   if (imessage != ISPLIB_MSG_SPMM_SUM && imessage != ISPLIB_MSG_SPMM_MEAN && !mm) return fail(ISPLIB_NO_OPT_IMPL, entry, "message outside the SpMM set");
   const StreamCall c = {entry, "fusedMM_csr_hip", mm ? STREAM_MINMAX : STREAM_SUM, m, n, k, nnz,  m == 0 || k == 0, pntrb, pntre, plan, y, ldy,
                          ldz,  z != nullptr,  true, workspace, workspace_bytes, (mm ? 2 : 1) * stream_parts_bytes(plan)};
   bool done;
   int rc = check_stream_call(c, &done);
   if (done) return rc;
   if (mm && plan->n_steps > 0 && !plan->perm) return fail(ISPLIB_FAIL, entry, "max / min need the plan's perm array (the winners' CSR positions)");
   if (mm && nnz >= ISPLIB_STREAM_NNZ_END) return fail(ISPLIB_FAIL, entry, "max / min need nnz < 2^31");
   if (mm && !isplib_rows_within(n, ldy, ISPLIB_STREAM_MINMAX_BYTES_END - 1u))
      return fail(ISPLIB_FAIL, "fusedMM_csr_stream_minmax_hip", "dense operand of 2 GiB or more (use fusedMM_csr_tasks_hip)");
   if ((rc = check_stream_workspace(c)) != ISPLIB_SUCCESS) return rc;
   SweepArgs a = stream_args(c, z, ldz);
   a.z_arg = z_arg;
   a.mean = imessage == ISPLIB_MSG_SPMM_MEAN ? 1 : 0;
   a.part_idx = mm && workspace ? (int *)((char *)workspace + stream_parts_bytes(plan)) : nullptr;
   if ((rc = set_epilogue(entry, ep, a)) != ISPLIB_SUCCESS) return rc;
   hipStream_t st = (hipStream_t)stream;
   const bool has_val = plan->vals != nullptr;
   const int stage_mode = mm ? ISPLIB_STAGE_OFF : stream_stage_mode();
   float *stage_base = nullptr;
   uint64_t stage_room = 0;
   if (stage_mode != ISPLIB_STAGE_OFF && workspace) {
      const uintptr_t lo = ((uintptr_t)workspace + stream_parts_bytes(plan) + (ISPLIB_STREAM_STAGE_PITCH - 1)) & ~(uintptr_t)(ISPLIB_STREAM_STAGE_PITCH - 1);
      const uintptr_t hi = (uintptr_t)workspace + workspace_bytes;
      if (lo < hi) { stage_base = (float *)lo; stage_room = hi - lo; }
   }
   unsigned staged = 0;
   auto stage = [&](SweepArgs &p, int64_t c0) {
      if (!isplib_stream_stage_panel((uint64_t)(uintptr_t)y, ldy, c0, k, plan->streams, n, nnz, stage_room, stage_mode)) return (int)ISPLIB_SUCCESS;
      const int rc = launch_stage_copy(p.y, ldy, n, stage_base, st);
      if (rc) return rc;
      p.y = stage_base;
      p.ldy = ISPLIB_STREAM_STAGE_PITCH / 4;
      p.ybytes = (unsigned)((uint64_t)n * ISPLIB_STREAM_STAGE_PITCH);
      staged |= 1u << ((c0 / 64) & 31);
      return (int)ISPLIB_SUCCESS;
   };
   const int rc_run = run_stream_panels(plan, a,
      [&](const SweepArgs &p) {
         if (imessage == ISPLIB_MSG_SPMM_MAX) return has_val ? launch_stream_minmax<OP_MAX, true>(p, st, plan->streams) : launch_stream_minmax<OP_MAX, false>(p, st, plan->streams);
         if (imessage == ISPLIB_MSG_SPMM_MIN) return has_val ? launch_stream_minmax<OP_MIN, true>(p, st, plan->streams) : launch_stream_minmax<OP_MIN, false>(p, st, plan->streams);
         return with_streams<STREAM_SUM>(plan->streams, [&](auto s) { return has_val ? launch_stream<s(), true>(p, st) : launch_stream<s(), false>(p, st); });
      },
      [&](const SweepArgs &p) {
         return imessage == ISPLIB_MSG_SPMM_MAX ? launch_hub_fold<OP_MAX, true>(p, st)
              : imessage == ISPLIB_MSG_SPMM_MIN ? launch_hub_fold<OP_MIN, true>(p, st) : launch_hub_fold<OP_ADD, true>(p, st);
      }, stage);
   if (!mm) stream_stage_report(staged);
   return rc_run;
}

extern "C" int fusedMM_csr_stream_hip(int32_t imessage, int64_t m, int64_t n, int64_t k, int64_t nnz,
                                      const int64_t *pntrb, const int64_t *pntre, const isplib_stream_plan *plan,
                                      const float *y, int64_t ldy, float *z, int64_t ldz, void *workspace,
                                      size_t workspace_bytes, const isplib_epilogue *ep, void *stream) {
   if (imessage != ISPLIB_MSG_SPMM_SUM && imessage != ISPLIB_MSG_SPMM_MEAN) {
      clear_error();
      return fail(ISPLIB_NO_OPT_IMPL, "fusedMM_csr_stream_hip: sum and mean only (max / min: fusedMM_csr_stream_minmax_hip)");
   }
   return stream_run(imessage, m, n, k, nnz, pntrb, pntre, plan, y, ldy, z, ldz, nullptr, workspace, workspace_bytes, ep, stream);
}

extern "C" int fusedMM_csr_stream_minmax_hip(int32_t imessage, int64_t m, int64_t n, int64_t k, int64_t nnz,
                                             const int64_t *pntrb, const int64_t *pntre, const isplib_stream_plan *plan,
                                             const float *y, int64_t ldy, float *z, int64_t ldz, int64_t *z_arg,
                                             void *workspace, size_t workspace_bytes, void *stream) {
   if (imessage != ISPLIB_MSG_SPMM_MAX && imessage != ISPLIB_MSG_SPMM_MIN) {
      clear_error();
      return fail(ISPLIB_NO_OPT_IMPL, "fusedMM_csr_stream_minmax_hip: max and min only");
   }
   return stream_run(imessage, m, n, k, nnz, pntrb, pntre, plan, y, ldy, z, ldz, z_arg, workspace, workspace_bytes, nullptr, stream);
}

#ifdef ISPLIB_EXP_WAVE_TIMES
extern "C" void isplib_debug_wave_times(unsigned long long *buf) { isplib::g_dbg = buf; isplib::g_dbg_launch = 0; }
#endif
```

isplib_amd/csrc/stream_plan.hip:

```cpp
#include <hip/hip_runtime.h>
#include <stdint.h>
#include <string.h>

#include <new>
#include <vector>

#include "../../include/isplib_hip.h"
#include "common.h"

#include "prims.h"

namespace isplib {

static inline unsigned sp_grid(int64_t n) {
   int64_t b = (n + 255) / 256;
   if (b < 1) b = 1;
   if (b > 256 * 64) b = 256 * 64;
   return (unsigned)b;
}

static inline unsigned sp_bits(uint64_t n) {
   unsigned b = 1;
   while (b < 32 && ((uint64_t)1 << b) < n) b++;
   return b;
}

__global__ __launch_bounds__(256) void sp_row_chunks_kernel(int64_t m, int64_t chunk, const int64_t *__restrict__ rowptr,
                                                            int *__restrict__ nchunk, int *__restrict__ hub_flag) {
   const int64_t stride = (int64_t)gridDim.x * blockDim.x;
   for (int64_t i = (int64_t)blockIdx.x * blockDim.x + threadIdx.x; i < m; i += stride) {
      const int64_t deg = rowptr[i + 1] - rowptr[i];
      const int64_t c = (deg + chunk - 1) / chunk;
      nchunk[i] = c < 1 ? 1 : (int)c;
      hub_flag[i] = c > 1 ? 1 : 0;
   }
}

__global__ __launch_bounds__(256) void sp_vrows_kernel(int64_t m, const int64_t *__restrict__ rowptr, const int *__restrict__ nchunk,
                                                       const int *__restrict__ first, const int *__restrict__ hub_idx,
                                                       const int *__restrict__ hub_flag, int *__restrict__ vrow_row,
                                                       int *__restrict__ vlen, uint32_t *__restrict__ sort_key,
                                                       uint32_t *__restrict__ sort_val, int *__restrict__ vhub,
                                                       int *__restrict__ hub_row) {
   const int64_t stride = (int64_t)gridDim.x * blockDim.x;
   for (int64_t i = (int64_t)blockIdx.x * blockDim.x + threadIdx.x; i < m; i += stride) {
      const int64_t deg = rowptr[i + 1] - rowptr[i];
      const int nc = nchunk[i], f = first[i];
      for (int ci = 0; ci < nc; ci++) {
         const int len = (int)((deg - ci + nc - 1) / nc);
         vrow_row[f + ci] = (int)i;
         vlen[f + ci] = len;
         sort_key[f + ci] = ~(uint32_t)len;
         sort_val[f + ci] = (uint32_t)(f + ci);
         vhub[f + ci] = nc > 1 ? 1 : 0;
      }
      if (hub_flag[i]) hub_row[hub_idx[i]] = (int)i;
   }
}

__global__ __launch_bounds__(256) void sp_iota_kernel(int64_t n, uint32_t *__restrict__ out) {
   const int64_t stride = (int64_t)gridDim.x * blockDim.x;
   for (int64_t i = (int64_t)blockIdx.x * blockDim.x + threadIdx.x; i < n; i += stride) out[i] = (uint32_t)i;
}

__global__ __launch_bounds__(256) void sp_deal_kernel(int64_t cnt, int round, const uint32_t *__restrict__ order,
                                                      const uint32_t *__restrict__ streams_by_load, const int *__restrict__ vlen,
                                                      int *__restrict__ sid, int *__restrict__ rnd, uint32_t *loads) {
   const int64_t stride = (int64_t)gridDim.x * blockDim.x;
   for (int64_t i = (int64_t)blockIdx.x * blockDim.x + threadIdx.x; i < cnt; i += stride) {
      const uint32_t item = order[i], s = streams_by_load[i];
      sid[item] = (int)s;
      rnd[item] = round;
      loads[s] += (uint32_t)vlen[item];
   }
}

__global__ __launch_bounds__(256) void sp_wave_steps_kernel(int64_t nw, int streams, const uint32_t *__restrict__ loads,
                                                            int64_t *__restrict__ steps, int64_t *__restrict__ loads64) {
   const int64_t stride = (int64_t)gridDim.x * blockDim.x;
   for (int64_t w = (int64_t)blockIdx.x * blockDim.x + threadIdx.x; w < nw; w += stride) {
      uint32_t mx = 0;
      for (int g = 0; g < streams; g++) {
         const uint32_t l = loads[w * streams + g];
         loads64[w * streams + g] = (int64_t)l;
         mx = l > mx ? l : mx;
      }
      steps[w] = (int64_t)mx;
   }
}

__device__ __forceinline__ int64_t sp_row_of(int64_t e, int64_t m, const int64_t *rowptr) {
   int64_t lo = 0, hi = m;
   while (hi - lo > 1) {
      const int64_t mid = lo + (hi - lo) / 2;
      if (rowptr[mid] <= e) lo = mid; else hi = mid;
   }
   return lo;
}

__global__ __launch_bounds__(256) void sp_edge_keys_kernel(int64_t m, int64_t nnz, int64_t width, int slices, int per, int snake,
                                                           const int64_t *__restrict__ rowptr, const int64_t *__restrict__ col,
                                                           const int *__restrict__ nchunk, const int *__restrict__ first,
                                                           const int *__restrict__ sid, const int *__restrict__ rnd,
                                                           uint32_t *__restrict__ keys, uint32_t *__restrict__ vals) {
   const int64_t stride = (int64_t)gridDim.x * blockDim.x;
   for (int64_t e = (int64_t)blockIdx.x * blockDim.x + threadIdx.x; e < nnz; e += stride) {
      const int64_t row = sp_row_of(e, m, rowptr);
      const int v = first[row] + (int)((e - rowptr[row]) % nchunk[row]);
      const int64_t sl = col[e] / width;
      keys[e] = (uint32_t)(((int64_t)sid[v] * slices + sl) * per + ((snake && (sl & 1)) ? per - 1 - rnd[v] : rnd[v]));
      vals[e] = (uint32_t)e;
   }
}

__global__ __launch_bounds__(256) void sp_pad_kernel(int64_t n_words, int streams, int per, int pad_row, uint32_t null_col, int32_t *__restrict__ words,
                                                     int32_t *__restrict__ perm, float *__restrict__ vals) {
   const int64_t stride = (int64_t)gridDim.x * blockDim.x;
   for (int64_t i = (int64_t)blockIdx.x * blockDim.x + threadIdx.x; i < n_words; i += stride) {
      const uint32_t lrow = pad_row >= 0 ? (uint32_t)pad_row : (uint32_t)(i % streams) * (uint32_t)per;
      words[i] = (int32_t)((lrow << 24) | null_col);
      perm[i] = -1;
      if (vals) vals[i] = 0.0f;
   }
}

__global__ __launch_bounds__(256) void sp_place_kernel(int64_t m, int64_t nnz, int streams, int per, const int64_t *__restrict__ rowptr,
                                                       const int64_t *__restrict__ col, const float *__restrict__ val,
                                                       const int *__restrict__ nchunk, const int *__restrict__ first,
                                                       const int *__restrict__ sid, const int *__restrict__ rnd,
                                                       const uint32_t *__restrict__ sorted_e, const int64_t *__restrict__ stream_start,
                                                       const int64_t *__restrict__ wave_step_off, int32_t *__restrict__ words,
                                                       int32_t *__restrict__ perm, float *__restrict__ vals) {
   const int64_t stride = (int64_t)gridDim.x * blockDim.x;
   for (int64_t q = (int64_t)blockIdx.x * blockDim.x + threadIdx.x; q < nnz; q += stride) {
      const int64_t e = (int64_t)sorted_e[q];
      const int64_t row = sp_row_of(e, m, rowptr);
      const int v = first[row] + (int)((e - rowptr[row]) % nchunk[row]);
      const int s = sid[v];
      const int64_t p = q - stream_start[s];
      const int64_t idx = (wave_step_off[s / streams] + p) * streams + s % streams;
      const uint32_t lrow = (uint32_t)((s % streams) * per + rnd[v]);
      words[idx] = (int32_t)((lrow << 24) | (uint32_t)col[e]);
      perm[idx] = (int32_t)e;
      if (vals) vals[idx] = val[e];
   }
}

__global__ __launch_bounds__(256) void sp_wave_rows_kernel(int64_t nv, int streams, int per, int rows_per_wave,
                                                           const int *__restrict__ vrow_row, const int *__restrict__ vhub,
                                                           const int *__restrict__ part_of, const int *__restrict__ sid,
                                                           const int *__restrict__ rnd, int32_t *__restrict__ wave_row,
                                                           int32_t *__restrict__ wave_part, const int *__restrict__ first,
                                                           const int *__restrict__ hub_idx, int32_t *__restrict__ hub_off) {
   const int64_t stride = (int64_t)gridDim.x * blockDim.x;
   for (int64_t v = (int64_t)blockIdx.x * blockDim.x + threadIdx.x; v < nv; v += stride) {
      const int s = sid[v];
      const int64_t at = (int64_t)(s / streams) * rows_per_wave + (s % streams) * per + rnd[v];
      const int row = vrow_row[v];
      wave_row[at] = row;
      wave_part[at] = vhub[v] ? part_of[v] : -1;
      if (vhub[v] && first[row] == (int)v) hub_off[hub_idx[row]] = part_of[v];
   }
}

__global__ __launch_bounds__(256) void sp_gather_vals_kernel(int64_t n_words, const int32_t *__restrict__ perm, const float *__restrict__ src,
                                                             float *__restrict__ vals) {
   const int64_t stride = (int64_t)gridDim.x * blockDim.x;
   for (int64_t i = (int64_t)blockIdx.x * blockDim.x + threadIdx.x; i < n_words; i += stride) vals[i] = perm[i] >= 0 ? src[perm[i]] : 0.0f;
}

struct SpTemp {
   std::vector<void *> ptrs;
   ~SpTemp() { for (void *p : ptrs) (void)hipFree(p); }
   template <class T> bool alloc(T **out, size_t count) {
      void *p = nullptr;
      if (hipMalloc(&p, (count ? count : 1) * sizeof(T)) != hipSuccess) { (void)hipGetLastError(); *out = nullptr; return false; }
      ptrs.push_back(p);
      *out = (T *)p;
      return true;
   }
};

template <class T> static bool sp_alloc_out(T **out, size_t count) {
   void *p = nullptr;
   if (hipMalloc(&p, (count ? count : 1) * sizeof(T)) != hipSuccess) { (void)hipGetLastError(); *out = nullptr; return false; }
   *out = (T *)p;
   return true;
}

static hipError_t sp_sort(void *temp, size_t &temp_bytes, const uint32_t *kin, uint32_t *kout, const uint32_t *vin, uint32_t *vout,
                          size_t n, unsigned bits, hipStream_t st) {
   return sort_pairs_u32(temp, temp_bytes, kin, kout, vin, vout, n, 0u, bits, st);
}

}

using namespace isplib;

extern "C" void isplib_stream_plan_free(isplib_stream_plan *plan) {
   if (!plan) return;
   (void)hipDeviceSynchronize();
   (void)hipFree(const_cast<int32_t *>(plan->words)); (void)hipFree(const_cast<float *>(plan->vals));
   (void)hipFree(const_cast<int64_t *>(plan->wave_step_off)); (void)hipFree(const_cast<int32_t *>(plan->wave_row));
   (void)hipFree(const_cast<int32_t *>(plan->wave_part)); (void)hipFree(const_cast<int32_t *>(plan->hub_row));
   (void)hipFree(const_cast<int32_t *>(plan->hub_off)); (void)hipFree(const_cast<int32_t *>(plan->perm));
   memset(plan, 0, sizeof(*plan));
}

extern "C" int isplib_stream_plan_set_values_hip(isplib_stream_plan *plan, const float *val, void *stream) {
   clear_error();
   if (!plan || !plan->perm) return fail(ISPLIB_FAIL, "isplib_stream_plan_set_values_hip: not a plan built by isplib_stream_plan_build_hip");
   const int64_t n_words = plan->n_steps * plan->streams;
   if (!val) {
      if (plan->vals) { (void)hipStreamSynchronize((hipStream_t)stream); (void)hipFree(const_cast<float *>(plan->vals)); plan->vals = nullptr; }
      return ISPLIB_SUCCESS;
   }
   if (!plan->vals) {
      float *v = nullptr;
      if (!sp_alloc_out(&v, (size_t)n_words)) return fail(ISPLIB_NOT_ENOUGH_MEM, "isplib_stream_plan_set_values_hip: device allocation failed");
      plan->vals = v;
   }
   if (n_words > 0) {
      hipLaunchKernelGGL(sp_gather_vals_kernel, dim3(sp_grid(n_words)), dim3(256), 0, (hipStream_t)stream, n_words, plan->perm, val,
                         const_cast<float *>(plan->vals));
      return check_launch("sp_gather_vals_kernel");
   }
   return ISPLIB_SUCCESS;
}

static int stream_plan_build(int64_t m, int64_t n, int64_t nnz, const int64_t *rowptr, const int64_t *col, const float *val,
                             int streams, int rpw, int resident, int slices, int chunk, int waves_per_gen,
                             isplib_stream_plan *out, void *stream, int pad_row = -1) {
   if (!out) return fail(ISPLIB_FAIL, "isplib_stream_plan_build_hip: out is NULL");
   memset(out, 0, sizeof(*out));
   if (m <= 0 || n <= 0 || nnz < 0 || !rowptr || (nnz > 0 && !col)) return fail(ISPLIB_FAIL, "isplib_stream_plan_build_hip: bad operand");
   if (n >= ISPLIB_STREAM_N_END || nnz >= ISPLIB_STREAM_NNZ_END || m >= (1LL << 31)) return fail(ISPLIB_FAIL, "isplib_stream_plan_build_hip: n < 2^24, nnz < 2^31, m < 2^31 required");
   if (slices < 1 || slices > 4096 || chunk < 1 || chunk >= (1 << 24)) return fail(ISPLIB_FAIL, "isplib_stream_plan_build_hip: slices in [1, 4096], chunk in [1, 2^24)");
   if (waves_per_gen <= 0) waves_per_gen = resident;
   const int per = rpw / streams;
   hipStream_t st = (hipStream_t)stream;
   SpTemp T;
   int *nchunk, *hub_flag, *first, *hub_idx;
   if (!T.alloc(&nchunk, (size_t)m) || !T.alloc(&hub_flag, (size_t)m) || !T.alloc(&first, (size_t)m + 1) || !T.alloc(&hub_idx, (size_t)m + 1))
      return fail(ISPLIB_NOT_ENOUGH_MEM, "isplib_stream_plan_build_hip: device allocation failed");
   hipLaunchKernelGGL(sp_row_chunks_kernel, dim3(sp_grid(m)), dim3(256), 0, st, m, (int64_t)chunk, rowptr, nchunk, hub_flag);
   int rc = check_launch("sp_row_chunks_kernel");
   if (rc) return rc;
   size_t scan_bytes = 0;
   ISPLIB_HIP_TRY(scan_exclusive_i32(nullptr, scan_bytes, nullptr, nullptr, (size_t)m, st));
   void *scan_tmp;
   {
      char *p;
      if (!T.alloc(&p, scan_bytes + 256)) return fail(ISPLIB_NOT_ENOUGH_MEM, "isplib_stream_plan_build_hip: device allocation failed");
      scan_tmp = p;
   }
   size_t sb = scan_bytes;
   ISPLIB_HIP_TRY(scan_exclusive_i32(scan_tmp, sb, (const int *)nchunk, first, (size_t)m, st));
   sb = scan_bytes;
   ISPLIB_HIP_TRY(scan_exclusive_i32(scan_tmp, sb, (const int *)hub_flag, hub_idx, (size_t)m, st));
   int last[4];
   ISPLIB_HIP_TRY(hipMemcpyAsync(&last[0], first + (m - 1), sizeof(int), hipMemcpyDeviceToHost, st));
   ISPLIB_HIP_TRY(hipMemcpyAsync(&last[1], nchunk + (m - 1), sizeof(int), hipMemcpyDeviceToHost, st));
   ISPLIB_HIP_TRY(hipMemcpyAsync(&last[2], hub_idx + (m - 1), sizeof(int), hipMemcpyDeviceToHost, st));
   ISPLIB_HIP_TRY(hipMemcpyAsync(&last[3], hub_flag + (m - 1), sizeof(int), hipMemcpyDeviceToHost, st));
   ISPLIB_HIP_TRY(hipStreamSynchronize(st));
   const int64_t nv = (int64_t)last[0] + last[1], n_hub = (int64_t)last[2] + last[3];
   const int64_t per_gen = (int64_t)waves_per_gen * rpw;
   const int64_t gens = (nv + per_gen - 1) / per_gen;
   const int64_t nw = gens * waves_per_gen, ns = nw * streams;
   if (gens > 4096 || ns >= (1LL << 31) || (double)ns * slices * per >= 4294967295.0)
      return fail(ISPLIB_FAIL, "isplib_stream_plan_build_hip: graph too large for this geometry (32-bit stream keys)");
   int *vrow_row, *vlen, *vhub, *part_of, *sid, *rnd;
   uint32_t *k_in, *k_out, *v_in, *v_out, *loads, *lk_out, *lv_in, *lv_out;
   const size_t big = (size_t)(nnz > nv ? nnz : nv) + 1;
   if (!T.alloc(&vrow_row, (size_t)nv) || !T.alloc(&vlen, (size_t)nv) || !T.alloc(&vhub, (size_t)nv) || !T.alloc(&part_of, (size_t)nv + 1) ||
       !T.alloc(&sid, (size_t)nv) || !T.alloc(&rnd, (size_t)nv) || !T.alloc(&k_in, big) || !T.alloc(&k_out, big) || !T.alloc(&v_in, big) ||
       !T.alloc(&v_out, big) || !T.alloc(&loads, (size_t)ns) || !T.alloc(&lk_out, (size_t)ns) || !T.alloc(&lv_in, (size_t)ns) ||
       !T.alloc(&lv_out, (size_t)ns))
      return fail(ISPLIB_NOT_ENOUGH_MEM, "isplib_stream_plan_build_hip: device allocation failed");
   int32_t *hub_row = nullptr, *hub_off = nullptr;
   if (!sp_alloc_out(&hub_row, (size_t)n_hub) || !sp_alloc_out(&hub_off, (size_t)n_hub + 1)) {
      (void)hipFree(hub_row); (void)hipFree(hub_off);
      return fail(ISPLIB_NOT_ENOUGH_MEM, "isplib_stream_plan_build_hip: device allocation failed");
   }
   out->hub_row = hub_row; out->hub_off = hub_off;
#define SP_FAIL(code, msg) do { const int c_ = fail(code, msg); isplib_stream_plan_free(out); return c_; } while (0)
#define SP_TRY(expr) do { const hipError_t e_ = (expr); if (e_ != hipSuccess) { const int c_ = hip_fail(e_, #expr); isplib_stream_plan_free(out); return c_; } } while (0)
#define SP_LAUNCHED(name) do { const int c_ = check_launch(name); if (c_) { isplib_stream_plan_free(out); return c_; } } while (0)
   hipLaunchKernelGGL(sp_vrows_kernel, dim3(sp_grid(m)), dim3(256), 0, st, m, rowptr, nchunk, first, hub_idx, hub_flag, vrow_row, vlen, k_in, v_in,
                      vhub, hub_row);
   SP_LAUNCHED("sp_vrows_kernel");
   size_t sbv = 0;
   SP_TRY(scan_exclusive_i32(nullptr, sbv, nullptr, nullptr, (size_t)nv, st));
   char *scan_tmp2;
   if (!T.alloc(&scan_tmp2, sbv + 256)) SP_FAIL(ISPLIB_NOT_ENOUGH_MEM, "isplib_stream_plan_build_hip: device allocation failed");
   SP_TRY(scan_exclusive_i32(scan_tmp2, sbv, (const int *)vhub, part_of, (size_t)nv, st));
   int part_last[2];
   SP_TRY(hipMemcpyAsync(&part_last[0], part_of + (nv - 1), sizeof(int), hipMemcpyDeviceToHost, st));
   SP_TRY(hipMemcpyAsync(&part_last[1], vhub + (nv - 1), sizeof(int), hipMemcpyDeviceToHost, st));
   size_t sort_bytes = 0, sort_small = 0;
   SP_TRY(sp_sort(nullptr, sort_bytes, nullptr, nullptr, nullptr, nullptr, big, 32, st));
   SP_TRY(sp_sort(nullptr, sort_small, nullptr, nullptr, nullptr, nullptr, (size_t)ns, 32, st));
   char *sort_tmp;
   if (!T.alloc(&sort_tmp, (sort_bytes > sort_small ? sort_bytes : sort_small) + 256)) SP_FAIL(ISPLIB_NOT_ENOUGH_MEM, "isplib_stream_plan_build_hip: device allocation failed");
   size_t tb = sort_bytes;
   SP_TRY(sp_sort(sort_tmp, tb, k_in, k_out, v_in, v_out, (size_t)nv, 32, st));
   SP_TRY(hipMemsetAsync(loads, 0, (size_t)ns * sizeof(uint32_t), st));
   hipLaunchKernelGGL(sp_iota_kernel, dim3(sp_grid(ns)), dim3(256), 0, st, ns, lv_in);
   SP_LAUNCHED("sp_iota_kernel");
   const int rounds = (int)((nv + ns - 1) / ns);
   if (rounds > per) SP_FAIL(ISPLIB_FAIL, "isplib_stream_plan_build_hip: internal: more rounds than rows per stream");
   for (int r = 0; r < rounds; r++) {
      const int64_t cnt = nv - (int64_t)r * ns < ns ? nv - (int64_t)r * ns : ns;
      tb = sort_small;
      SP_TRY(sp_sort(sort_tmp, tb, loads, lk_out, lv_in, lv_out, (size_t)ns, 32, st));
      hipLaunchKernelGGL(sp_deal_kernel, dim3(sp_grid(cnt)), dim3(256), 0, st, cnt, r, v_out + (int64_t)r * ns, lv_out, vlen, sid, rnd, loads);
      SP_LAUNCHED("sp_deal_kernel");
   }
   int64_t *steps, *loads64, *stream_start, *wave_step_off = nullptr;
   if (!T.alloc(&steps, (size_t)nw) || !T.alloc(&loads64, (size_t)ns) || !T.alloc(&stream_start, (size_t)ns) || !sp_alloc_out(&wave_step_off, (size_t)nw + 1))
      SP_FAIL(ISPLIB_NOT_ENOUGH_MEM, "isplib_stream_plan_build_hip: device allocation failed");
   out->wave_step_off = wave_step_off;
   hipLaunchKernelGGL(sp_wave_steps_kernel, dim3(sp_grid(nw)), dim3(256), 0, st, nw, streams, loads, steps, loads64);
   SP_LAUNCHED("sp_wave_steps_kernel");
   size_t s64 = 0;
   SP_TRY(scan_exclusive_i64(nullptr, s64, nullptr, nullptr, (size_t)ns, st));
   char *scan_tmp3;
   if (!T.alloc(&scan_tmp3, s64 + 256)) SP_FAIL(ISPLIB_NOT_ENOUGH_MEM, "isplib_stream_plan_build_hip: device allocation failed");
   size_t s64b = s64;
   SP_TRY(scan_exclusive_i64(scan_tmp3, s64b, (const int64_t *)loads64, stream_start, (size_t)ns, st));
   s64b = s64;
   SP_TRY(scan_exclusive_i64(scan_tmp3, s64b, (const int64_t *)steps, wave_step_off, (size_t)nw, st));
   int64_t tail[2];
   SP_TRY(hipMemcpyAsync(&tail[0], wave_step_off + (nw - 1), sizeof(int64_t), hipMemcpyDeviceToHost, st));
   SP_TRY(hipMemcpyAsync(&tail[1], steps + (nw - 1), sizeof(int64_t), hipMemcpyDeviceToHost, st));
   SP_TRY(hipStreamSynchronize(st));
   const int64_t n_steps = tail[0] + tail[1];
   const int64_t n_parts = (int64_t)part_last[0] + part_last[1];
   SP_TRY(hipMemcpyAsync(wave_step_off + nw, &n_steps, sizeof(int64_t), hipMemcpyHostToDevice, st));
   const int32_t n_parts32 = (int32_t)n_parts;
   SP_TRY(hipMemcpyAsync(hub_off + n_hub, &n_parts32, sizeof(int32_t), hipMemcpyHostToDevice, st));
   const int64_t n_words = n_steps * streams;
   int32_t *words = nullptr, *perm = nullptr, *wave_row = nullptr, *wave_part = nullptr;
   float *vals = nullptr;
   if (!sp_alloc_out(&words, (size_t)n_words)) SP_FAIL(ISPLIB_NOT_ENOUGH_MEM, "isplib_stream_plan_build_hip: device allocation failed");
   out->words = words;
   if (!sp_alloc_out(&perm, (size_t)n_words)) SP_FAIL(ISPLIB_NOT_ENOUGH_MEM, "isplib_stream_plan_build_hip: device allocation failed");
   out->perm = perm;
   if (val) {
      if (!sp_alloc_out(&vals, (size_t)n_words)) SP_FAIL(ISPLIB_NOT_ENOUGH_MEM, "isplib_stream_plan_build_hip: device allocation failed");
      out->vals = vals;
   }
   if (!sp_alloc_out(&wave_row, (size_t)nw * rpw)) SP_FAIL(ISPLIB_NOT_ENOUGH_MEM, "isplib_stream_plan_build_hip: device allocation failed");
   out->wave_row = wave_row;
   if (!sp_alloc_out(&wave_part, (size_t)nw * rpw)) SP_FAIL(ISPLIB_NOT_ENOUGH_MEM, "isplib_stream_plan_build_hip: device allocation failed");
   out->wave_part = wave_part;
   SP_TRY(hipMemsetAsync(wave_row, 0xFF, (size_t)nw * rpw * sizeof(int32_t), st));
   SP_TRY(hipMemsetAsync(wave_part, 0xFF, (size_t)nw * rpw * sizeof(int32_t), st));
   hipLaunchKernelGGL(sp_wave_rows_kernel, dim3(sp_grid(nv)), dim3(256), 0, st, nv, streams, per, rpw, vrow_row, vhub, part_of, sid, rnd, wave_row,
                      wave_part, first, hub_idx, hub_off);
   SP_LAUNCHED("sp_wave_rows_kernel");
   if (n_words > 0) {
      hipLaunchKernelGGL(sp_pad_kernel, dim3(sp_grid(n_words)), dim3(256), 0, st, n_words, streams, per, pad_row, (uint32_t)n, words, perm, vals);
      SP_LAUNCHED("sp_pad_kernel");
   }
   if (nnz > 0) {
      const int64_t width = (n + slices - 1) / slices;
      hipLaunchKernelGGL(sp_edge_keys_kernel, dim3(sp_grid(nnz)), dim3(256), 0, st, m, nnz, width, slices, per, pad_row >= 0 ? 1 : 0, rowptr, col, nchunk, first,
                         sid, rnd, k_in, v_in);
      SP_LAUNCHED("sp_edge_keys_kernel");
      tb = sort_bytes;
      SP_TRY(sp_sort(sort_tmp, tb, k_in, k_out, v_in, v_out, (size_t)nnz, sp_bits((uint64_t)ns * slices * per + 1), st));
      hipLaunchKernelGGL(sp_place_kernel, dim3(sp_grid(nnz)), dim3(256), 0, st, m, nnz, streams, per, rowptr, col, val, nchunk, first, sid, rnd, v_out,
                         stream_start, wave_step_off, words, perm, vals);
      SP_LAUNCHED("sp_place_kernel");
   }
   SP_TRY(hipStreamSynchronize(st));
#undef SP_FAIL
#undef SP_TRY
#undef SP_LAUNCHED
   out->rows = m; out->cols = n; out->slices = slices; out->gens = (int32_t)gens; out->waves_per_gen = waves_per_gen;
   out->rows_per_wave = rpw; out->streams = streams; out->chunk = chunk;
   out->n_steps = n_steps; out->n_parts = n_parts; out->n_hub = n_hub;
   return ISPLIB_SUCCESS;
}

extern "C" int isplib_stream_plan_build_hip(int64_t m, int64_t n, int64_t nnz, const int64_t *rowptr, const int64_t *col,
                                            const float *val, int streams, int slices, int chunk, int waves_per_gen,
                                            isplib_stream_plan *out, void *stream) {
   clear_error();
   int rpw = 0, resident = 0;
   if (isplib_spmm_stream_geometry(streams, &rpw, &resident) != ISPLIB_SUCCESS) return ISPLIB_FAIL;
   return stream_plan_build(m, n, nnz, rowptr, col, val, streams, rpw, resident, slices, chunk, waves_per_gen, out, stream);
}

__global__ __launch_bounds__(256) void sp_unsorted_kernel(int64_t m, int64_t nnz, const int64_t *__restrict__ rowptr,
                                                          const int64_t *__restrict__ col, int *__restrict__ flag) {
   const int64_t stride = (int64_t)gridDim.x * blockDim.x;
   bool bad = false;
   for (int64_t e = (int64_t)blockIdx.x * blockDim.x + threadIdx.x + 1; e < nnz; e += stride)
      if (col[e] < col[e - 1] && e > rowptr[sp_row_of(e, m, rowptr)]) bad = true;
   if (bad) atomicOr(flag, 1);
}

extern "C" int isplib_stream_plan_build_minmax_hip(int64_t m, int64_t n, int64_t nnz, const int64_t *rowptr, const int64_t *col,
                                                   const float *val, int streams, int slices, int chunk, int waves_per_gen,
                                                   isplib_stream_plan *out, void *stream) {
   clear_error();
   int rpw = 0, resident = 0;
   if (isplib_spmm_stream_minmax_geometry(streams, &rpw, &resident) != ISPLIB_SUCCESS) return ISPLIB_FAIL;
   if (out) memset(out, 0, sizeof(*out));
   if (m <= 0 || nnz < 0 || !rowptr || (nnz > 0 && !col)) return fail(ISPLIB_FAIL, "isplib_stream_plan_build_minmax_hip: bad operand");
   if (nnz > 1) {
      int *flag = nullptr, host = 1;
      if (hipMalloc((void **)&flag, 256) != hipSuccess) { (void)hipGetLastError(); return fail(ISPLIB_NOT_ENOUGH_MEM, "isplib_stream_plan_build_minmax_hip: device allocation failed"); }
      hipStream_t st = (hipStream_t)stream;
      bool ok = hipMemsetAsync(flag, 0, sizeof(int), st) == hipSuccess;
      if (ok) {
         hipLaunchKernelGGL(sp_unsorted_kernel, dim3(sp_grid(nnz)), dim3(256), 0, st, m, nnz, rowptr, col, flag);
         ok = hipGetLastError() == hipSuccess && hipMemcpyAsync(&host, flag, sizeof(int), hipMemcpyDeviceToHost, st) == hipSuccess &&
              hipStreamSynchronize(st) == hipSuccess;
      }
      (void)hipFree(flag);
      if (!ok) return hip_fail(hipGetLastError(), "isplib_stream_plan_build_minmax_hip: sortedness check");
      if (host) return fail(ISPLIB_FAIL, "isplib_stream_plan_build_minmax_hip: rows are not column-sorted (use the task list)");
   }
   return stream_plan_build(m, n, nnz, rowptr, col, val, streams, rpw, resident, slices, chunk, waves_per_gen, out, stream,  rpw);
}

extern "C" int isplib_stream_plan_build_fusedmm_hip(int64_t m, int64_t n, int64_t nnz, const int64_t *rowptr, const int64_t *col,
                                                    int streams, int slices, int chunk, int waves_per_gen,
                                                    isplib_stream_plan *out, void *stream) {
   clear_error();
   int rpw = 0, resident = 0;
   if (isplib_fusedmm_stream_geometry(streams, &rpw, &resident) != ISPLIB_SUCCESS) return ISPLIB_FAIL;
   return stream_plan_build(m, n, nnz, rowptr, col, nullptr, streams, rpw, resident, slices, chunk, waves_per_gen, out, stream,  rpw);
}
```

isplib_amd/csrc/sweep_common.h:

```cpp
#pragma once
#include <hip/hip_runtime.h>
#include <stdint.h>
#include <float.h>
#include <limits.h>
#include <type_traits>

#include "../../include/isplib_hip.h"
#include "common.h"
#include "gather.h"

#ifndef ISPLIB_STREAM_NV4
#define ISPLIB_STREAM_NV4 64
#endif
#ifndef ISPLIB_STREAM_NBW4
#define ISPLIB_STREAM_NBW4 2
#endif
#ifndef ISPLIB_STREAM_WGS4
#define ISPLIB_STREAM_WGS4 2
#endif
#ifndef ISPLIB_EXP_GATHER_AUX
#define ISPLIB_EXP_GATHER_AUX 0
#endif
#ifndef ISPLIB_HYB4_NV
#define ISPLIB_HYB4_NV 64
#endif
#ifndef ISPLIB_HYB4_NBW
#define ISPLIB_HYB4_NBW 2
#endif
#ifndef ISPLIB_HYB4_HT
#define ISPLIB_HYB4_HT 128
#endif
#ifndef ISPLIB_HYB4_HWR
#define ISPLIB_HYB4_HWR 4
#endif
#ifndef ISPLIB_HYB8_NV
#define ISPLIB_HYB8_NV 128
#endif
#ifndef ISPLIB_HYB8_NBW
#define ISPLIB_HYB8_NBW 4
#endif
#ifndef ISPLIB_HYB8_HT
#define ISPLIB_HYB8_HT 256
#endif
#ifndef ISPLIB_HYB8_HWR
#define ISPLIB_HYB8_HWR 8
#endif
#ifndef ISPLIB_STREAM_NV8
#define ISPLIB_STREAM_NV8 128
#endif
#ifndef ISPLIB_STREAM_NBW8
#define ISPLIB_STREAM_NBW8 4
#endif
#ifndef ISPLIB_STREAM_WGS8
#define ISPLIB_STREAM_WGS8 2
#endif
#ifndef ISPLIB_STREAM_MM_NV
#define ISPLIB_STREAM_MM_NV 32
#endif
#ifndef ISPLIB_STREAM_MM_NBW
#define ISPLIB_STREAM_MM_NBW 2
#endif
#ifndef ISPLIB_STREAM_MM_WGS
#define ISPLIB_STREAM_MM_WGS 2
#endif
#ifndef ISPLIB_STREAM_MM8_NV
#define ISPLIB_STREAM_MM8_NV 64
#endif
#ifndef ISPLIB_STREAM_MM8_NBW
#define ISPLIB_STREAM_MM8_NBW 4
#endif
#ifndef ISPLIB_STREAM_MM8_WGS
#define ISPLIB_STREAM_MM8_WGS 2
#endif

namespace isplib {

struct SweepArgs {
   int64_t k, nnz;
   const float *val;
   const int64_t *indx, *pntrb, *pntre;
   const int32_t *indx32;
   const float *y;
   int64_t ldy;
   unsigned ybytes;
   float *z;
   int64_t ldz;
   int64_t *z_arg;
   int mean;
   int empty_init;
   const int32_t *wave_row;
   const int32_t *wave_part;
   const int64_t *wave_task_off;
   const int64_t *task_b;
   const int32_t *task_meta;
   int wave_base, wave_count;
   const int32_t *words;
   const float *vals;
   const int64_t *wave_step_off;
   unsigned null_word;
   const int32_t *ids;
   int abs_ids;
   const int32_t *hot_rows;
   const int32_t *hot_words;
   const int64_t *hot_step_off;
   int slices;
   const float *g;
   int64_t ldg;
   float *dval;
#ifdef ISPLIB_EXP_WAVE_TIMES
   unsigned long long *dbg;
#endif
   float *part_val;
   int *part_idx;
   const int32_t *hub_row, *hub_off;
   int64_t n_hub;
   const float *ep_row_scale, *ep_self, *ep_bias;
   int64_t ep_ld_self;
   int ep_relu;
};

template <int OP, int VEC>
__device__ __forceinline__ void finish_row(const SweepArgs &a, int row, int c, float (&v)[VEC], int (&bi)[VEC], int64_t (&arg)[VEC]) {
   const int64_t rb = a.pntrb[row];
   const int64_t deg = a.pntre[row] - rb;
   if (OP == OP_ADD) {
      if (a.mean) {
         const float d = (float)(deg > 1 ? deg : 1);
#pragma unroll
         for (int i = 0; i < VEC; i++) v[i] = v[i] / d;
      }
      if (a.ep_self) {
         const float *sr = a.ep_self + (size_t)row * (size_t)a.ep_ld_self + c;
#pragma unroll
         for (int i = 0; i < VEC; i++) v[i] += sr[i];
      }
      if (a.ep_row_scale) {
         const float rs = a.ep_row_scale[row];
#pragma unroll
         for (int i = 0; i < VEC; i++) v[i] *= rs;
      }
      if (a.ep_bias) {
#pragma unroll
         for (int i = 0; i < VEC; i++) v[i] += a.ep_bias[c + i];
      }
      if (a.ep_relu) {
#pragma unroll
         for (int i = 0; i < VEC; i++) v[i] = v[i] > 0.0f ? v[i] : 0.0f;
      }
   } else {
#pragma unroll
      for (int i = 0; i < VEC; i++) {
         if (deg <= 0) v[i] = a.empty_init ? identity<OP>() : 0.0f;
         arg[i] = bi[i] == INT_MAX ? a.nnz : (a.abs_ids ? (int64_t)bi[i] : rb + (int64_t)bi[i]);
      }
   }
}

template <int OP, int VEC>
__global__ __launch_bounds__(256) void sweep_hub_fold_kernel(const SweepArgs a) {
   const int64_t kv = a.k / VEC;
   const int64_t total = a.n_hub * kv;
   const int64_t stride = (int64_t)gridDim.x * blockDim.x;
   for (int64_t i = (int64_t)blockIdx.x * blockDim.x + threadIdx.x; i < total; i += stride) {
      const int64_t h = i / kv;
      const int c = (int)(i - h * kv) * VEC;
      float v[VEC];
      int bi[VEC];
#pragma unroll
      for (int q = 0; q < VEC; q++) { v[q] = identity<OP>(); bi[q] = INT_MAX; }
      const int p1 = a.hub_off[h + 1];
      for (int p = a.hub_off[h]; p < p1; p++) {
         const size_t po = (size_t)p * (size_t)a.k + c;
         float t[VEC];
         load_vec<VEC>(a.part_val + po, t);
#pragma unroll
         for (int q = 0; q < VEC; q++) {
            if (OP == OP_ADD) {
               v[q] += t[q];
            } else {
               const int oi = a.z_arg ? a.part_idx[po + q] : p;
               const bool take = better<OP>(t[q], oi, v[q], bi[q]);
               v[q] = take ? t[q] : v[q];
               bi[q] = take ? oi : bi[q];
            }
         }
      }
      const int row = a.hub_row[h];
      int64_t arg[VEC];
      finish_row<OP, VEC>(a, row, c, v, bi, arg);
      store_vec<VEC>(a.z + (size_t)row * (size_t)a.ldz + c, v);
      if (OP != OP_ADD && a.z_arg) {
         int64_t *ar = a.z_arg + (size_t)row * (size_t)a.ldz + c;
#pragma unroll
         for (int q = 0; q < VEC; q++) ar[q] = arg[q];
      }
   }
}

template <int LPR_, int NVMAX_, int NBW_, int WAVES_ = 4>
struct StreamWave {
   static constexpr int LPR = LPR_, NVMAX = NVMAX_, NBW = NBW_, WAVES = WAVES_;
   static constexpr int G = 64 / LPR, PANEL = LPR * 4, U = 64 * NBW / G, PER = NVMAX / G;
   int lane, wave, g, lc;
   int wl;
   int64_t w;
   bool cok;
   int ccol, vfirst;
   unsigned cbyte, poison;
   int64_t s0, nwords;
   const int32_t *wp;
   unsigned ldyb;
};

template <class SW> __device__ __forceinline__ bool stream_wave_id(const SweepArgs &a, SW &sw) {
   sw.lane = threadIdx.x & 63;
   sw.wave = __builtin_amdgcn_readfirstlane(threadIdx.x >> 6);
   sw.g = sw.lane / SW::LPR;
   sw.lc = sw.lane % SW::LPR;
   sw.wl = (int)blockIdx.x * SW::WAVES + sw.wave;
   sw.w = (int64_t)a.wave_base + sw.wl;
   return sw.wl < a.wave_count;
}

template <bool RAGGED, class SW> __device__ __forceinline__ void stream_columns(const SweepArgs &a, SW &sw) {
   sw.cok = sw.lc * 4 < a.k;
   sw.ccol = sw.lc * 4;
   sw.vfirst = 0;
   if (RAGGED && sw.cok && sw.ccol + 4 > (int)a.k) { sw.vfirst = sw.ccol + 4 - (int)a.k; sw.ccol = (int)a.k - 4; }
   sw.cbyte = (unsigned)sw.ccol * 4u;
   sw.poison = sw.cok ? 0u : BUF_OOB;
}

template <class SW> __device__ __forceinline__ void stream_bounds(const SweepArgs &a, SW &sw) {
   sw.s0 = a.wave_step_off[sw.w];
   const int64_t s1 = a.wave_step_off[sw.w + 1];
   sw.nwords = (s1 - sw.s0) * SW::G;
   sw.wp = a.words + sw.s0 * SW::G;
   sw.ldyb = (unsigned)a.ldy * 4u;
}

template <class SW> __device__ __forceinline__ unsigned stream_pad_own_row(const SweepArgs &a, const SW &sw) {
   return ((unsigned)((sw.lane % SW::G) * SW::PER) << 24) | a.null_word;
}
template <class SW> __device__ __forceinline__ unsigned stream_pad_spare_row(const SweepArgs &a, const SW &) {
   return ((unsigned)SW::NVMAX << 24) | a.null_word;
}

template <class SW, class S, class T>
__device__ __forceinline__ void stream_load_batch(const SW &sw, const S *src, int64_t first, T pad, T (&reg)[SW::NBW]) {
#pragma unroll
   for (int q = 0; q < SW::NBW; q++) {
      const int64_t i = first + q * 64 + sw.lane;
      reg[q] = i < sw.nwords ? (T)src[i] : pad;
   }
}

template <int AUX, class SW>
__device__ __forceinline__ void stream_issue(const SW &sw, __amdgpu_buffer_rsrc_t rsrc, const unsigned (&word_l)[SW::NBW], int u, unsigned &la, v4i_t &t) {
   const unsigned word = (unsigned)__shfl((int)word_l[(u * SW::G) / 64], (u * SW::G) % 64 + sw.g);
   const unsigned o = (__umul24(word & 0xFFFFFFu, sw.ldyb) + sw.cbyte) | sw.poison;
   la = (word >> 24) * (unsigned)SW::PANEL;
   t = __builtin_amdgcn_raw_buffer_load_b128(rsrc, (int)o, 0, AUX);
}

// ... 213 lines not shown
```

isplib_amd/plan.py:

```python
from __future__ import annotations

import os
from dataclasses import dataclass
from typing import Optional

import torch

from . import cabi


@dataclass
class TaskPlan:
    slices: int
    n_tasks: int
    task_row: torch.Tensor
    task_b: torch.Tensor
    task_len: torch.Tensor
    seg_off: torch.Tensor
    lane_off: list
    chunk: int
    short_row: int
    col32: Optional[torch.Tensor] = None
    ncols: Optional[int] = None

# ... 50 lines not shown
    n_tasks: int
    n_parts: int
    n_hub: int
    wave_row: torch.Tensor
    wave_part: torch.Tensor
    wave_task_off: torch.Tensor
    task_b: torch.Tensor
    task_meta: torch.Tensor
    hub_row: torch.Tensor
    hub_off: torch.Tensor
    chunk: int
    min_seg: int
    col32: Optional[torch.Tensor] = None

    def struct(self) -> "cabi.SweepPlanStruct":
        p = lambda t: t.data_ptr() if t is not None and t.numel() else None
        return cabi.SweepPlanStruct(self.rows, self.slices, self.gens, self.waves_per_gen, self.rows_per_wave, self.n_tasks,
                                    self.n_parts, self.n_hub, p(self.wave_row), p(self.wave_part), p(self.wave_task_off),
                                    p(self.task_b), p(self.task_meta), p(self.hub_row), p(self.hub_off))

    def workspace(self, reduce: str, k: int) -> torch.Tensor:
        import ctypes
        ps = self.struct()
        nbytes = cabi.exp_lib().isplib_spmm_sweep_workspace_bytes(cabi.MESSAGE[reduce], ctypes.byref(ps), k)
        return torch.empty(nbytes, dtype=torch.uint8, device=self.wave_row.device)


def sweep_plan_arrays(rowptr: torch.Tensor, table: torch.Tensor, slices: int, waves_per_gen: int, rows_per_wave: int = 16,
                      chunk: int = 2048, min_seg: int = 16) -> dict:
    assert 1 <= slices <= 4096 and rows_per_wave in (8, 16, 32) and waves_per_gen >= 1 and 1 <= chunk < (1 << 24)
    m = rowptr.numel() - 1
    dev = table.device
    table = table.view(m, slices + 1)
    i64 = dict(dtype=torch.int64, device=dev)
    deg = rowptr[1:] - rowptr[:-1]
    nchunk = ((deg + chunk - 1) // chunk).clamp(min=1)
    csize = (deg + nchunk - 1) // nchunk
    nv = int(nchunk.sum())
    vrow = torch.repeat_interleave(torch.arange(m, **i64), nchunk)
    first = torch.cumsum(nchunk, 0) - nchunk
    ci = torch.arange(nv, **i64) - first[vrow]
    vb = rowptr[vrow] + ci * csize[vrow]
    ve = torch.minimum(vb + csize[vrow], rowptr[vrow + 1])
    vb = torch.minimum(vb, ve)
    vlen = ve - vb
    gens = max(1, -(-nv // (waves_per_gen * rows_per_wave)))
    nw = gens * waves_per_gen
    order = torch.sort(vlen, descending=True, stable=True).indices
    rank = torch.empty(nv, **i64)
    rank[order] = torch.arange(nv, **i64)
    rnd, pos = rank // nw, rank % nw
    wave = torch.where(rnd % 2 == 0, pos, nw - 1 - pos)
    slot = rnd
    is_hub = nchunk[vrow] > 1
    part = torch.where(is_hub, torch.cumsum(is_hub.to(torch.int64), 0) - 1, torch.full((nv,), -1, **i64))
    wave_row = torch.full((nw * rows_per_wave,), -1, dtype=torch.int32, device=dev)
    wave_part = torch.full((nw * rows_per_wave,), -1, dtype=torch.int32, device=dev)
    at = wave * rows_per_wave + slot
    wave_row[at] = vrow.to(torch.int32)
    wave_part[at] = part.to(torch.int32)
    hub_rows = torch.nonzero(nchunk > 1).flatten()
    hub_off = torch.zeros(hub_rows.numel() + 1, dtype=torch.int32, device=dev)
    if hub_rows.numel():
        hub_off[1:] = torch.cumsum(nchunk[hub_rows], 0).to(torch.int32)
    s_r = (vlen // max(min_seg, 1)).clamp(min=1, max=slices)
    sl = torch.arange(slices, **i64)
    grp = (sl[None, :] * s_r[:, None]) // slices
    is_start = torch.ones((nv, slices), dtype=torch.bool, device=dev)
    is_start[:, 1:] = grp[:, 1:] != grp[:, :-1]
    e_slice = ((grp + 1) * slices + s_r[:, None] - 1) // s_r[:, None]
    tb = table[vrow]
    seg_b = torch.minimum(torch.maximum(tb[:, :-1], vb[:, None]), ve[:, None])
    seg_e = torch.minimum(torch.maximum(torch.gather(tb, 1, e_slice.clamp(max=slices)), vb[:, None]), ve[:, None])
    seg_len = seg_e - seg_b
    keep = is_start & (seg_len > 0)
    del grp, e_slice, tb, is_start
    vi, si = torch.nonzero(keep, as_tuple=True)
    t_b, t_len = seg_b[vi, si], seg_len[vi, si]
    del seg_b, seg_e, seg_len, keep
    t_wave, t_slot = wave[vi], slot[vi]
    key = (t_wave * slices + si) * rows_per_wave + t_slot
    perm = torch.sort(key).indices
    t_b, t_len, t_wave, t_slot = t_b[perm], t_len[perm], t_wave[perm], t_slot[perm]
    wave_task_off = torch.zeros(nw + 1, **i64)
    if t_wave.numel():
        wave_task_off[1:] = torch.cumsum(torch.bincount(t_wave, minlength=nw), 0)
    task_meta = ((t_slot << 24) | t_len).to(torch.int32)
    return dict(rows=m, slices=slices, gens=gens, waves_per_gen=waves_per_gen, rows_per_wave=rows_per_wave,
                n_tasks=int(t_b.numel()), n_parts=int(is_hub.sum()), n_hub=int(hub_rows.numel()), wave_row=wave_row,
                wave_part=wave_part, wave_task_off=wave_task_off, task_b=t_b.contiguous(), task_meta=task_meta.contiguous(),
                hub_row=hub_rows.to(torch.int32), hub_off=hub_off, chunk=chunk, min_seg=min_seg)


def build_sweep_plan(rowptr: torch.Tensor, col: torch.Tensor, ncols: int, slices: int, waves_per_gen: int,
                     rows_per_wave: int = 16, chunk: int = 2048, min_seg: int = 16,
                     col32: Optional[torch.Tensor] = None) -> Optional[SweepPlan]:
    table, ok = cabi.spmm_slices(rowptr, col, ncols, slices)
    if not ok:
        return None
    arrays = sweep_plan_arrays(rowptr, table, slices, waves_per_gen, rows_per_wave, chunk, min_seg)
    del table
    if col32 is None:
        col32 = cabi.pack_indices(col)
    return SweepPlan(col32=col32, **arrays)


@dataclass
class StreamPlan:
    rows: int
    cols: int
    slices: int
    gens: int
    waves_per_gen: int
    rows_per_wave: int
    streams: int
    n_steps: int
    n_parts: int
    n_hub: int
    words: torch.Tensor
    vals: Optional[torch.Tensor]
    perm: torch.Tensor
    wave_step_off: torch.Tensor
    wave_row: torch.Tensor
    wave_part: torch.Tensor
    hub_row: torch.Tensor
    hub_off: torch.Tensor
    chunk: int

    def struct(self) -> "cabi.StreamPlanStruct":
        p = lambda t: t.data_ptr() if t is not None and t.numel() else None
        return cabi.StreamPlanStruct(self.rows, self.cols, self.slices, self.gens, self.waves_per_gen, self.rows_per_wave,
                                     self.streams, int(self.chunk), self.n_steps, self.n_parts, self.n_hub, p(self.words), p(self.vals),
                                     p(self.wave_step_off), p(self.wave_row), p(self.wave_part), p(self.hub_row), p(self.hub_off),
                                     p(self.perm) if self.perm.dtype == torch.int32 else None)

    def workspace(self, minmax: bool = False) -> torch.Tensor:
        import ctypes
        ps = self.struct()
        L = cabi.lib()
        nbytes = (L.isplib_spmm_stream_minmax_workspace_bytes if minmax else L.isplib_spmm_stream_workspace_bytes)(ctypes.byref(ps))
        return torch.empty(nbytes, dtype=torch.uint8, device=self.words.device)

    def set_values(self, val: Optional[torch.Tensor]) -> None:
        if val is None:
            self.vals = None
            return
        ok = self.perm >= 0
        out = torch.zeros(self.perm.numel(), dtype=torch.float32, device=self.perm.device)
        out[ok] = val.detach().to(torch.float32)[self.perm[ok].to(torch.int64)]
        self.vals = out


def stream_plan_arrays(rowptr: torch.Tensor, col: torch.Tensor, ncols: int, slices: int, waves_per_gen: int,
                       rows_per_wave: int = 16, streams: int = 4, chunk: int = 2048, pad_row: Optional[int] = None) -> dict:
    assert 1 <= slices <= 4096 and streams in (2, 4, 8) and waves_per_gen >= 1
    assert rows_per_wave % streams == 0 and rows_per_wave <= 128
    assert ncols < (1 << 24), "column ids share a 32-bit word with the local row and are multiplied in 24 bits"
    m = rowptr.numel() - 1
    dev = col.device
    i64 = dict(dtype=torch.int64, device=dev)
    nnz = col.numel()
    deg = rowptr[1:] - rowptr[:-1]
    nchunk = ((deg + chunk - 1) // chunk).clamp(min=1)
    nv = int(nchunk.sum())
    vrow = torch.repeat_interleave(torch.arange(m, **i64), nchunk)
    first = torch.cumsum(nchunk, 0) - nchunk
    ci = torch.arange(nv, **i64) - first[vrow]
    vlen = (deg[vrow] - ci + nchunk[vrow] - 1) // nchunk[vrow]
    erow = torch.repeat_interleave(torch.arange(m, **i64), deg)
    ev = first[erow] + (torch.arange(nnz, **i64) - rowptr[erow]) % nchunk[erow]
    del erow
    per = rows_per_wave // streams
    gens = max(1, -(-nv // (waves_per_gen * rows_per_wave)))
    nw = gens * waves_per_gen
    ns = nw * streams
    order = torch.sort(vlen, descending=True, stable=True).indices
    sid = torch.empty(nv, **i64)
    rnd = torch.empty(nv, **i64)
    loads = torch.zeros(ns, **i64)
    bias = float(os.environ.get("ISPLIB_EXP_XCD_BIAS", "0"))
    cost = None
    if bias != 0.0:
        blk = (torch.arange(ns, **i64) // streams % waves_per_gen) // 4
        cost = torch.where(blk % 2 == 0, 1024 + int(round(1024 * bias)), 1024 - int(round(1024 * bias))).to(torch.int64)
    for r in range(-(-nv // ns)):
        items = order[r * ns:(r + 1) * ns]
        to = torch.sort(loads, stable=True).indices[:items.numel()]
        sid[items] = to
        rnd[items] = r
        loads[to] += vlen[items] if cost is None else vlen[items] * cost[to]
    wave, slot = sid // streams, sid % streams
    lrow = slot * per + rnd
    is_hub = nchunk[vrow] > 1
    part = torch.where(is_hub, torch.cumsum(is_hub.to(torch.int64), 0) - 1, torch.full((nv,), -1, **i64))
    wave_row = torch.full((nw * rows_per_wave,), -1, dtype=torch.int32, device=dev)
    wave_part = torch.full((nw * rows_per_wave,), -1, dtype=torch.int32, device=dev)
    at = wave * rows_per_wave + lrow
    wave_row[at] = vrow.to(torch.int32)
    wave_part[at] = part.to(torch.int32)
    hub_rows = torch.nonzero(nchunk > 1).flatten()
    hub_off = torch.zeros(hub_rows.numel() + 1, dtype=torch.int32, device=dev)
    if hub_rows.numel():
        hub_off[1:] = torch.cumsum(nchunk[hub_rows], 0).to(torch.int32)
    width = -(-ncols // slices)
    if os.environ.get("ISPLIB_EXP_STREAM_ORDER") == "col":
        key = (sid[ev] * slices + col // width) * width + col % width
    elif pad_row is not None or os.environ.get("ISPLIB_EXP_SNAKE") == "1":
        sl = col // width
        key = (sid[ev] * slices + sl) * per + torch.where(sl % 2 == 1, per - 1 - rnd[ev], rnd[ev])
    else:
        key = (sid[ev] * slices + col // width) * per + rnd[ev]
    perm = torch.sort(key, stable=True).indices
    del key
    e_sid = sid[ev][perm]
    lens = torch.bincount(e_sid, minlength=ns)
    start = torch.cumsum(lens, 0) - lens
    p = torch.arange(nnz, **i64) - start[e_sid]
    steps = lens.view(nw, streams).max(dim=1).values
    wave_step_off = torch.zeros(nw + 1, **i64)
    wave_step_off[1:] = torch.cumsum(steps, 0)
    n_steps = int(wave_step_off[-1])
    idx = (wave_step_off[e_sid // streams] + p) * streams + e_sid % streams
    del p, start
    if pad_row is None:
        pad = ((torch.arange(streams, **i64) * per) << 24) | int(ncols)
    else:
        pad = torch.full((streams,), (int(pad_row) << 24) | int(ncols), **i64)
    pad = torch.where(pad >= 2 ** 31, pad - 2 ** 32, pad)
    words = pad.to(torch.int32).repeat(n_steps)
    words[idx] = ((lrow[ev][perm] << 24) | col[perm]).to(torch.int32)
    perm_out = torch.full((n_steps * streams,), -1, dtype=torch.int32 if nnz < 2 ** 31 else torch.int64, device=dev)
    perm_out[idx] = perm.to(perm_out.dtype)
    return dict(rows=m, cols=int(ncols), slices=slices, gens=gens, waves_per_gen=waves_per_gen, rows_per_wave=rows_per_wave,
                streams=streams, n_steps=n_steps, n_parts=int(is_hub.sum()), n_hub=int(hub_rows.numel()), words=words, vals=None,
                perm=perm_out, wave_step_off=wave_step_off, wave_row=wave_row, wave_part=wave_part,
                hub_row=hub_rows.to(torch.int32), hub_off=hub_off, chunk=chunk)


def build_stream_plan(rowptr: torch.Tensor, col: torch.Tensor, val: Optional[torch.Tensor], ncols: int, slices: int,
                      waves_per_gen: Optional[int] = None, rows_per_wave: Optional[int] = None, streams: int = 4,
                      chunk: int = 512, minmax: bool = False) -> Optional[StreamPlan]:
    if ncols >= cabi.STREAM_N_END:
        return None
    if minmax:
        if col.numel() > 1:
            starts = torch.zeros(col.numel(), dtype=torch.bool, device=col.device)
            starts[rowptr[:-1][rowptr[:-1] < col.numel()]] = True
            if bool(((col[1:] < col[:-1]) & ~starts[1:]).any()):
                return None
        rpw, resident = cabi.stream_minmax_geometry(streams)
    else:
        rpw, resident = cabi.stream_geometry(streams)
    rows_per_wave = rpw if rows_per_wave is None else rows_per_wave
    waves_per_gen = resident if waves_per_gen is None else waves_per_gen
    plan = StreamPlan(**stream_plan_arrays(rowptr, col, ncols, slices, waves_per_gen, rows_per_wave, streams, chunk,
                                           pad_row=rows_per_wave if minmax else None))
    plan.set_values(val)
    return plan


def build_stream_plan_native(rowptr: torch.Tensor, col: torch.Tensor, ncols: int, slices: int, streams: int = 4,
                             chunk: int = 512, minmax: bool = False) -> Optional[StreamPlan]:
    if ncols >= cabi.STREAM_N_END or col.numel() >= cabi.STREAM_NNZ_END:
        return None
    try:
        native = cabi.NativeStreamPlan(rowptr, col, None, ncols, streams, slices, chunk, 0, minmax)
    except cabi.IsplibError as e:
        if e.status == cabi.ISPLIB_FAIL:
            return None
        if e.status == cabi.ISPLIB_NOT_ENOUGH_MEM:
            torch.cuda.empty_cache()
            return None
        raise
    i32, i64 = torch.int32, torch.int64
    plan = StreamPlan(rows=native.rows, cols=native.cols, slices=native.slices, gens=native.gens, waves_per_gen=native.waves_per_gen,
                      rows_per_wave=native.rows_per_wave, streams=native.streams, n_steps=native.n_steps, n_parts=native.n_parts,
                      n_hub=native.n_hub, words=native.view("words", i32), vals=None, perm=native.view("perm", i32),
                      wave_step_off=native.view("wave_step_off", i64), wave_row=native.view("wave_row", i32),
                      wave_part=native.view("wave_part", i32), hub_row=native.view("hub_row", i32),
                      hub_off=native.view("hub_off", i32), chunk=chunk)
    plan._native = native
    return plan


@dataclass
class HybridPlan:
    cold: StreamPlan
    table_rows: int
    hot_cap: int
    n_hot_steps: int
    hot_rows: torch.Tensor
    hot_words: torch.Tensor
    hot_step_off: torch.Tensor
    hot_perm: torch.Tensor
    hot_edges: int = 0

    def struct(self) -> "cabi.HybridPlanStruct":
        p = lambda t: t.data_ptr() if t is not None and t.numel() else None
        return cabi.HybridPlanStruct(self.cold.struct(), self.table_rows, self.hot_cap, self.n_hot_steps, p(self.hot_rows),
                                     p(self.hot_words), p(self.hot_step_off), p(self.hot_perm))

    def workspace(self) -> torch.Tensor:
        return self.cold.workspace()


def hybrid_plan_arrays(rowptr: torch.Tensor, col: torch.Tensor, ncols: int, slices: int, waves_per_gen: int, rows_per_wave: int,
                       streams: int, chunk: int, table_rows: int, hot_cap: int, min_refs: int = 2) -> dict:
    assert 1 <= slices <= 4096 and streams in (4, 8) and waves_per_gen >= 8 and waves_per_gen % 8 == 0
    assert rows_per_wave % streams == 0 and rows_per_wave <= 256 and 2 <= table_rows <= 65536 and hot_cap >= 1
    assert ncols < (1 << 24)
    m = rowptr.numel() - 1
    dev = col.device
    i64 = dict(dtype=torch.int64, device=dev)
    nnz = col.numel()
    assert nnz < 2 ** 31
    per = rows_per_wave // streams
    width = -(-ncols // slices)
    indeg = torch.bincount(col, minlength=ncols)
    cslice = torch.arange(ncols, **i64) // width
    top = int(indeg.max()) + 1 if ncols else 1
    order = torch.sort(cslice * top + (top - 1 - indeg), stable=True).indices
    s_sorted = cslice[order]
    counts = torch.bincount(cslice, minlength=slices)
    starts = torch.cumsum(counts, 0) - counts
    rank = torch.arange(ncols, **i64) - starts[s_sorted]
    is_top = (rank < table_rows - 1) & (indeg[order] >= min_refs)
    tidx = torch.full((ncols,), -1, **i64)
    tidx[order[is_top]] = rank[is_top]
    hot_rows = torch.full((slices * table_rows,), int(ncols), dtype=torch.int32, device=dev)
    hot_rows[s_sorted[is_top] * table_rows + rank[is_top]] = order[is_top].to(torch.int32)
    del order, s_sorted, rank, is_top, counts, starts, indeg, cslice
    e_hot = tidx[col] >= 0
    deg = rowptr[1:] - rowptr[:-1]
    nchunk = ((deg + chunk - 1) // chunk).clamp(min=1)
    nv = int(nchunk.sum())
    vrow = torch.repeat_interleave(torch.arange(m, **i64), nchunk)
    first = torch.cumsum(nchunk, 0) - nchunk
    erow = torch.repeat_interleave(torch.arange(m, **i64), deg)
    ev = first[erow] + (torch.arange(nnz, **i64) - rowptr[erow]) % nchunk[erow]
    del erow
    vlen = torch.bincount(ev[~e_hot], minlength=nv)
    gens = max(1, -(-nv // (waves_per_gen * rows_per_wave)))
    nw = gens * waves_per_gen
    ns = nw * streams
    order = torch.sort(vlen, descending=True, stable=True).indices
    sid = torch.empty(nv, **i64)
    rnd = torch.empty(nv, **i64)
    loads = torch.zeros(ns, **i64)
    for r in range(-(-nv // ns)):
        items = order[r * ns:(r + 1) * ns]
        to = torch.sort(loads, stable=True).indices[:items.numel()]
        sid[items] = to
        rnd[items] = r
        loads[to] += vlen[items]
    del order, loads
    wave, slot = sid // streams, sid % streams
    lrow = slot * per + rnd
    is_hub = nchunk[vrow] > 1
    part = torch.where(is_hub, torch.cumsum(is_hub.to(torch.int64), 0) - 1, torch.full((nv,), -1, **i64))
    wave_row = torch.full((nw * rows_per_wave,), -1, dtype=torch.int32, device=dev)
    wave_part = torch.full((nw * rows_per_wave,), -1, dtype=torch.int32, device=dev)
    at = wave * rows_per_wave + lrow
    wave_row[at] = vrow.to(torch.int32)
    wave_part[at] = part.to(torch.int32)
    hub_rows = torch.nonzero(nchunk > 1).flatten()
    hub_off = torch.zeros(hub_rows.numel() + 1, dtype=torch.int32, device=dev)
    if hub_rows.numel():
        hub_off[1:] = torch.cumsum(nchunk[hub_rows], 0).to(torch.int32)
    e_sid_all = sid[ev]
    e_rnd_all = rnd[ev]
    e_lrow_all = lrow[ev]
    del ev
    h_e = torch.nonzero(e_hot).flatten()
    hkey = (e_sid_all[h_e] * slices + col[h_e] // width) * per + e_rnd_all[h_e]
    hperm = torch.sort(hkey, stable=True).indices
    h_e = h_e[hperm]
    group = hkey[hperm] // per
    del hkey, hperm
    gcount = torch.bincount(group, minlength=ns * slices)
    gstart = torch.cumsum(gcount, 0) - gcount
    hrank = torch.arange(h_e.numel(), **i64) - gstart[group]
    over = hrank >= hot_cap
    if bool(over.any()):
        e_hot[h_e[over]] = False
        h_e, group, hrank = h_e[~over], group[~over], hrank[~over]
    hsteps = gcount.clamp(max=hot_cap).view(nw, streams, slices).max(dim=1).values
    hot_step_off = torch.zeros(nw * slices + 1, **i64)
    hot_step_off[1:] = torch.cumsum(hsteps.flatten(), 0)
    n_hot_steps = int(hot_step_off[-1])
    h_sid = group // slices
    h_slice = group % slices
    widx = (hot_step_off[(h_sid // streams) * slices + h_slice] + hrank) * streams + h_sid % streams
    pad = ((torch.arange(streams, **i64) * per) << 24) | int(table_rows - 1)
    hot_words = pad.to(torch.int32).repeat(n_hot_steps)
    hot_words[widx] = ((e_lrow_all[h_e] << 24) | tidx[col[h_e]]).to(torch.int32)
    hot_perm = torch.full((n_hot_steps * streams,), -1, dtype=torch.int32, device=dev)
    hot_perm[widx] = h_e.to(torch.int32)
    n_hot = int(h_e.numel())
    del h_e, group, hrank, gcount, gstart, widx, h_sid, h_slice, tidx
    c_e = torch.nonzero(~e_hot).flatten()
    c_sid = e_sid_all[c_e]
    key = (c_sid * slices + col[c_e] // width) * per + e_rnd_all[c_e]
    perm = torch.sort(key, stable=True).indices
    del key
    c_e, c_sid = c_e[perm], c_sid[perm]
    del perm
    lens = torch.bincount(c_sid, minlength=ns)
    start = torch.cumsum(lens, 0) - lens
    p = torch.arange(c_e.numel(), **i64) - start[c_sid]
    steps = lens.view(nw, streams).max(dim=1).values
    wave_step_off = torch.zeros(nw + 1, **i64)
    wave_step_off[1:] = torch.cumsum(steps, 0)
    n_steps = int(wave_step_off[-1])
    idx = (wave_step_off[c_sid // streams] + p) * streams + c_sid % streams
    del p, start
    pad = ((torch.arange(streams, **i64) * per) << 24) | int(ncols)
    words = pad.to(torch.int32).repeat(n_steps)
    words[idx] = ((e_lrow_all[c_e] << 24) | col[c_e]).to(torch.int32)
    perm_out = torch.full((n_steps * streams,), -1, dtype=torch.int32, device=dev)
# ... 21 lines not shown
```

Measured before the change: 45.35 billion.

## Level stream-plan row assignment by calibrated per-wave throughput capacities

```diff
diff --git a/include/isplib_hip.h b/include/isplib_hip.h
--- a/include/isplib_hip.h
+++ b/include/isplib_hip.h
@@ -213,6 +213,12 @@
 int  isplib_stream_plan_build_hip(int64_t m, int64_t n, int64_t nnz, const int64_t *rowptr, const int64_t *col,
                                   const float *val, int streams, int slices, int chunk, int waves_per_gen,
                                   isplib_stream_plan *out , void *stream);
+#define ISPLIB_STREAM_CAP_ONE 4096u
+int  isplib_stream_capacities_hip(int device, int streams, int waves_per_gen, int64_t nnz, uint32_t *caps ,
+                                  int *levelled , void *stream);
+int  isplib_stream_plan_build_caps_hip(int64_t m, int64_t n, int64_t nnz, const int64_t *rowptr, const int64_t *col,
+                                       const float *val, int streams, int slices, int chunk, int waves_per_gen,
+                                       const uint32_t *caps , isplib_stream_plan *out , void *stream);
 int  isplib_stream_plan_set_values_hip(isplib_stream_plan *plan, const float *val , void *stream);
 void isplib_stream_plan_free(isplib_stream_plan *plan);
 int    isplib_spmm_stream_geometry(int streams, int *rows_per_wave , int *waves_resident );
diff --git a/isplib_amd/cabi.py b/isplib_amd/cabi.py
--- a/isplib_amd/cabi.py
+++ b/isplib_amd/cabi.py
@@ -128,7 +128,7 @@
     "isplib_sddmm_csr_tasks_hip", "fusedMM_csr_tasks_epilogue_hip", "fusedMM_csr_udef_hip", "fusedMM_csr_udef_tasks_hip", "isplib_pack_indices_hip",
     "isplib_suggest_slices", "isplib_graph_create", "isplib_graph_set_slices", "isplib_graph_set_values", "isplib_graph_spmm", "isplib_graph_spmm_backward",
     "isplib_graph_destroy", "isplib_suggest_slices_whole_rows", "isplib_graph_sddmm",
-    "fusedMM_csr_stream_hip", "isplib_spmm_stream_workspace_bytes", "isplib_spmm_stream_geometry", "isplib_suggest_stream", "isplib_suggest_stream_weighted", "isplib_stream_plan_build_hip", "isplib_stream_plan_build_minmax_hip", "fusedMM_csr_stream_minmax_hip", "isplib_spmm_stream_minmax_geometry", "isplib_suggest_stream_minmax", "isplib_spmm_stream_minmax_workspace_bytes", "isplib_stream_plan_set_values_hip", "isplib_stream_plan_free", "isplib_spmm_minmax_bw_det_hip", "isplib_spmm_minmax_bw_workspace_bytes", "isplib_scatter_rows_det_hip",
+    "fusedMM_csr_stream_hip", "isplib_spmm_stream_workspace_bytes", "isplib_spmm_stream_geometry", "isplib_suggest_stream", "isplib_suggest_stream_weighted", "isplib_stream_plan_build_hip", "isplib_stream_plan_build_caps_hip", "isplib_stream_capacities_hip", "isplib_stream_plan_build_minmax_hip", "fusedMM_csr_stream_minmax_hip", "isplib_spmm_stream_minmax_geometry", "isplib_suggest_stream_minmax", "isplib_spmm_stream_minmax_workspace_bytes", "isplib_stream_plan_set_values_hip", "isplib_stream_plan_free", "isplib_spmm_minmax_bw_det_hip", "isplib_spmm_minmax_bw_workspace_bytes", "isplib_scatter_rows_det_hip",
     "isplib_minmax_bw_bucket_workspace_bytes", "isplib_minmax_bw_bucket_hip", "isplib_scatter_keys_workspace_bytes", "isplib_scatter_keys_det_hip",
     "isplib_fusedmm_stream_geometry", "isplib_suggest_fusedmm_stream", "isplib_stream_plan_build_fusedmm_hip", "fusedMM_csr_udef_stream_hip",
     "isplib_row_scale_hip", "isplib_masked_scale_colsum_hip", "isplib_masked_scale_colsum_workspace_bytes",
@@ -305,6 +305,13 @@
         L.isplib_stream_plan_build_hip.restype = ctypes.c_int
         L.isplib_stream_plan_build_hip.argtypes = [_i64, _i64, _i64, _vp, _vp, _vp, ctypes.c_int, ctypes.c_int, ctypes.c_int, ctypes.c_int,
                                                    ctypes.POINTER(StreamPlanStruct), _vp]
+        L.isplib_stream_plan_build_caps_hip.restype = ctypes.c_int
+        L.isplib_stream_plan_build_caps_hip.argtypes = [_i64, _i64, _i64, _vp, _vp, _vp, ctypes.c_int, ctypes.c_int, ctypes.c_int, ctypes.c_int,
+                                                        _vp, ctypes.POINTER(StreamPlanStruct), _vp]
+        L.isplib_stream_capacities_hip.restype = ctypes.c_int
+        L.isplib_stream_capacities_hip.argtypes = [ctypes.c_int, ctypes.c_int, ctypes.c_int, _i64, _vp, ctypes.POINTER(ctypes.c_int), _vp]
+        L.isplib_stream_level_set.restype = ctypes.c_int
+        L.isplib_stream_level_set.argtypes = [ctypes.c_int]
         L.isplib_stream_plan_build_minmax_hip.restype = ctypes.c_int
         L.isplib_stream_plan_build_minmax_hip.argtypes = [_i64, _i64, _i64, _vp, _vp, _vp, ctypes.c_int, ctypes.c_int, ctypes.c_int, ctypes.c_int,
                                                           ctypes.POINTER(StreamPlanStruct), _vp]
@@ -1815,7 +1822,8 @@
 class NativeStreamPlan:
 
     def __init__(self, rowptr, col, val, ncols: int, streams: int, slices: int, chunk: int, waves_per_gen: int = 0,
-                 minmax: bool = False, fusedmm: bool = False):
+                 minmax: bool = False, fusedmm: bool = False, capacities=None):
+        assert capacities is None or not (minmax or fusedmm), "max / min and FusedMM plans keep equal capacities"
         self._s = StreamPlanStruct()
         self.device = col.device
         m = rowptr.numel() - 1
@@ -1828,6 +1836,14 @@
                 _check(lib().isplib_stream_plan_build_minmax_hip(m, int(ncols), col.numel(), _ptr(rowptr), _ptr(col), _ptr(val),
                                                                  int(streams), int(slices), int(chunk), int(waves_per_gen), ctypes.byref(self._s),
                                                                  _stream(col.device)), "isplib_stream_plan_build_minmax_hip")
+            elif capacities is not None:
+                caps = (ctypes.c_uint32 * len(capacities))(*[int(c) for c in capacities])
+                rpw, resident = stream_geometry(streams)
+                if len(caps) != (int(waves_per_gen) if waves_per_gen > 0 else resident):
+                    raise ValueError("one capacity per wave of a generation")
+                _check(lib().isplib_stream_plan_build_caps_hip(m, int(ncols), col.numel(), _ptr(rowptr), _ptr(col), _ptr(val), int(streams),
+                                                               int(slices), int(chunk), int(waves_per_gen), ctypes.cast(caps, _vp),
+                                                               ctypes.byref(self._s), _stream(col.device)), "isplib_stream_plan_build_caps_hip")
             else:
                 _check(lib().isplib_stream_plan_build_hip(m, int(ncols), col.numel(), _ptr(rowptr), _ptr(col), _ptr(val), int(streams),
                                                           int(slices), int(chunk), int(waves_per_gen), ctypes.byref(self._s),
@@ -1882,6 +1898,27 @@
             pass
 
 
+STREAM_CAP_ONE = 4096
+
+
+def stream_capacities(device, streams: int, waves_per_gen: int, nnz: int):
+    device = torch.device(device)
+    if device.type != "cuda":
+        return None
+    _, resident = stream_geometry(streams)
+    wpg = int(waves_per_gen) if waves_per_gen > 0 else resident
+    caps = (ctypes.c_uint32 * wpg)()
+    levelled = ctypes.c_int(0)
+    with torch.cuda.device(device):
+        _check(lib().isplib_stream_capacities_hip(-1, int(streams), wpg, int(nnz), ctypes.cast(caps, _vp), ctypes.byref(levelled),
+                                                  _stream(device)), "isplib_stream_capacities_hip")
+    return list(caps) if levelled.value else None
+
+
+def stream_level_set(mode: int) -> None:
+    _check(lib().isplib_stream_level_set(int(mode)), "isplib_stream_level_set")
+
+
 def stream_geometry(streams: int = 4):
     rpw, res = ctypes.c_int(0), ctypes.c_int(0)
     _check(lib().isplib_spmm_stream_geometry(int(streams), ctypes.byref(rpw), ctypes.byref(res)), "isplib_spmm_stream_geometry")
diff --git a/isplib_amd/csrc/common.h b/isplib_amd/csrc/common.h
--- a/isplib_amd/csrc/common.h
+++ b/isplib_amd/csrc/common.h
@@ -12,6 +12,8 @@
 
 int stream_stage_mode();
 void stream_stage_report(unsigned panels);
+int stream_kernel_calibrate(int streams, int waves_per_gen, int launches, int degree, int col_mult, double *wave_ticks, hipStream_t st);
+int stream_level_mode();
 
 inline void clear_error() { error_buffer()[0] = '\0'; }
 
diff --git a/isplib_amd/csrc/runtime.hip b/isplib_amd/csrc/runtime.hip
--- a/isplib_amd/csrc/runtime.hip
+++ b/isplib_amd/csrc/runtime.hip
@@ -50,5 +50,23 @@
 }
 extern "C" unsigned isplib_stream_stage_last(void) { return isplib::g_stream_stage_last; }
 
+namespace isplib {
+static int g_stream_level = -1;
+int stream_level_mode() {
+   if (g_stream_level < 0) {
+      const char *e = getenv("ISPLIB_STREAM_LEVEL");
+      g_stream_level = !e ? 2 : strcmp(e, "0") == 0 ? 0 : strcmp(e, "1") == 0 ? 1 : 2;
+   }
+   return g_stream_level;
+}
+}
+
+extern "C" int isplib_stream_level_set(int mode) {
+   isplib::clear_error();
+   if (mode < 0 || mode > 2) return isplib::fail(ISPLIB_FAIL, "isplib_stream_level_set: 0 (off), 1 (on) or 2 (auto)");
+   isplib::g_stream_level = mode;
+   return ISPLIB_SUCCESS;
+}
+
 extern "C" int isplib_hip_abi_version(void) { return ISPLIB_HIP_ABI_VERSION; }
 extern "C" const char *isplib_hip_last_error(void) { return isplib::error_buffer(); }
diff --git a/isplib_amd/csrc/spmm_sweep.hip b/isplib_amd/csrc/spmm_sweep.hip
--- a/isplib_amd/csrc/spmm_sweep.hip
+++ b/isplib_amd/csrc/spmm_sweep.hip
@@ -1,8 +1,12 @@
+#include <vector>
+
 #include "sweep_common.h"
 
+extern "C" void isplib_debug_wave_times(unsigned long long *buf);
+
 namespace isplib {
 
-template <int LPR, bool HAS_VAL, int NVMAX, int NBW, int WGS>
+template <int LPR, bool HAS_VAL, int NVMAX, int NBW, int WGS, bool TIMED = false>
 __global__ __launch_bounds__(256, (stream_wgs_per_cu<LPR, NVMAX, WGS>())) void spmm_stream_kernel(const SweepArgs a) {
    using Wave = StreamWave<LPR, NVMAX, NBW>;
    constexpr int WAVES = Wave::WAVES, G = Wave::G, PANEL = Wave::PANEL, U = Wave::U, PER = Wave::PER;
@@ -12,9 +16,8 @@
    Wave sw;
    if (!stream_wave_id(a, sw)) return;
    const int lane = sw.lane;
-#ifdef ISPLIB_EXP_WAVE_TIMES
-   const unsigned long long t_start = __builtin_amdgcn_s_memtime();
-#endif
+   unsigned long long t_start = 0, t_loop = 0, t_loop_end = 0;
+   if constexpr (TIMED) t_start = __builtin_amdgcn_s_memtime();
    float *my = s_all + sw.wave * WAVE_FLOATS;
    for (int i = lane * 4; i < WAVE_FLOATS; i += 256)
       *reinterpret_cast<float4 *>(my + i) = make_float4(0.0f, 0.0f, 0.0f, 0.0f);
@@ -38,9 +41,7 @@
    unsigned cur = (unsigned)(sw.g * PER * PANEL);
    float acc[4] = {0.0f, 0.0f, 0.0f, 0.0f};
    const int64_t nb = (sw.nwords + 64 * NBW - 1) / (64 * NBW);
-#ifdef ISPLIB_EXP_WAVE_TIMES
-   const unsigned long long t_loop = __builtin_amdgcn_s_memtime();
-#endif
+   if constexpr (TIMED) t_loop = __builtin_amdgcn_s_memtime();
    for (int64_t b = 0; b < nb; b++) {
       float vnext = HAS_VAL ? __shfl(v0[0], sw.g) : 0.0f;
 #pragma unroll
@@ -65,9 +66,7 @@
       if (HAS_VAL) stream_load_batch(sw, vp, (b + 2) * 64 * NBW, 0.0f, v1);
    }
    stream_flush(lane_base + cur, acc);
-#ifdef ISPLIB_EXP_WAVE_TIMES
-   const unsigned long long t_loop_end = __builtin_amdgcn_s_memtime();
-#endif
+   if constexpr (TIMED) t_loop_end = __builtin_amdgcn_s_memtime();
    int row_[PER], part_[PER];
 #pragma unroll
    for (int jj = 0; jj < PER; jj++) {
@@ -92,14 +91,13 @@
       finish_row<OP_ADD>(a, row, c, v, bi, arg);
       store_tail<4>(a.z + (size_t)row * (size_t)a.ldz + c, v, sw.vfirst);
    }
-#ifdef ISPLIB_EXP_WAVE_TIMES
-   if (a.dbg && lane == 0) {
-      a.dbg[(size_t)sw.wl * 4 + 0] = t_start;
-      a.dbg[(size_t)sw.wl * 4 + 1] = t_loop;
-      a.dbg[(size_t)sw.wl * 4 + 2] = t_loop_end;
-      a.dbg[(size_t)sw.wl * 4 + 3] = __builtin_amdgcn_s_memtime();
-   }
-#endif
+   if constexpr (TIMED) if (a.dbg && lane == 0) {
+      a.dbg[(size_t)sw.wl * 5 + 0] = t_start;
+      a.dbg[(size_t)sw.wl * 5 + 1] = t_loop;
+      a.dbg[(size_t)sw.wl * 5 + 2] = t_loop_end;
+      a.dbg[(size_t)sw.wl * 5 + 3] = __builtin_amdgcn_s_memtime();
+      a.dbg[(size_t)sw.wl * 5 + 4] = (__builtin_amdgcn_s_getreg(20u | (3u << 11)) << 24) | ((__builtin_amdgcn_s_getreg(4u | (31u << 11)) >> 8) & 0xFFFFu);
+   }
 }
 
 typedef float v2f_t __attribute__((ext_vector_type(2)));
@@ -280,19 +278,21 @@
    return check_launch("stream_stage_copy_kernel");
 }
 
-#ifdef ISPLIB_EXP_WAVE_TIMES
-static unsigned long long *g_dbg = nullptr;
-static int g_dbg_launch = 0;
-#endif
+static thread_local unsigned long long *g_dbg = nullptr;
+static thread_local int g_dbg_launch = 0;
 template <int STREAMS, bool HAS_VAL>
 static int launch_stream(const SweepArgs &a_in, hipStream_t st) {
    constexpr StreamGeom ge = stream_geom(STREAM_SUM, STREAMS);
    SweepArgs a = a_in;
-#ifdef ISPLIB_EXP_WAVE_TIMES
-   a.dbg = g_dbg ? g_dbg + (size_t)(g_dbg_launch++ % 4) * (size_t)a.wave_count * 4 : nullptr;
-#endif
    const unsigned blocks = (unsigned)((a.wave_count + 3) / 4);
    if (blocks == 0) return ISPLIB_SUCCESS;
+   if constexpr (!HAS_VAL) {
+      if (g_dbg) {
+         a.dbg = g_dbg + (size_t)(g_dbg_launch++ % 4) * (size_t)a.wave_count * 5;
+         hipLaunchKernelGGL((spmm_stream_kernel<ge.lpr, false, ge.nvmax, ge.nbw, ge.wgs, true>), dim3(blocks), dim3(256), 0, st, a);
+         return check_launch("spmm_stream_kernel");
+      }
+   }
    hipLaunchKernelGGL((spmm_stream_kernel<ge.lpr, HAS_VAL, ge.nvmax, ge.nbw, ge.wgs>), dim3(blocks), dim3(256), 0, st, a);
    return check_launch("spmm_stream_kernel");
 }
@@ -451,6 +451,58 @@
    return stream_run(imessage, m, n, k, nnz, pntrb, pntre, plan, y, ldy, z, ldz, z_arg, workspace, workspace_bytes, nullptr, stream);
 }
 
-#ifdef ISPLIB_EXP_WAVE_TIMES
+namespace isplib {
+__global__ __launch_bounds__(256) void stream_calib_graph_kernel(int64_t n, int64_t ncols, int64_t degree, int64_t *__restrict__ rowptr, int64_t *__restrict__ col) {
+   const int64_t stride = (int64_t)gridDim.x * blockDim.x, nnz = n * degree;
+   for (int64_t i = (int64_t)blockIdx.x * blockDim.x + threadIdx.x; i <= n; i += stride) rowptr[i] = i * degree;
+   for (int64_t e = (int64_t)blockIdx.x * blockDim.x + threadIdx.x; e < nnz; e += stride) {
+      uint64_t h = (uint64_t)e * 0x9E3779B97F4A7C15ull;
+      h ^= h >> 29; h *= 0xBF58476D1CE4E5B9ull; h ^= h >> 32;
+      col[e] = (int64_t)(h % (uint64_t)ncols);
+   }
+}
+
+int stream_kernel_calibrate(int streams, int waves_per_gen, int launches, int degree, int col_mult, double *wave_ticks, hipStream_t st) {
+   int rpw = 0, resident = 0;
+   if (isplib_spmm_stream_geometry(streams, &rpw, &resident) != ISPLIB_SUCCESS) return ISPLIB_FAIL;
+   if (waves_per_gen < 4 || waves_per_gen % 4 != 0 || waves_per_gen > resident || launches < 1 || launches > 16 || degree < 1 || degree > 1024 ||
+       col_mult < 1 || col_mult > 8)
+      return fail(ISPLIB_FAIL, "stream calibration: whole workgroups of one resident generation, 1..16 launches");
+   const int64_t n = (int64_t)waves_per_gen * rpw, ncols = n * col_mult, nnz = n * degree, k = 256 / streams;
+   struct Temps {
+      std::vector<void *> p;
+      isplib_stream_plan plan;
+      unsigned long long *callers_dbg = g_dbg;
+      Temps() { memset(&plan, 0, sizeof(plan)); }
+      ~Temps() { isplib_debug_wave_times(callers_dbg); isplib_stream_plan_free(&plan); for (void *q : p) (void)hipFree(q); }
+      void *get(size_t bytes) { void *q = nullptr; if (hipMalloc(&q, bytes) != hipSuccess) { (void)hipGetLastError(); return nullptr; } p.push_back(q); return q; }
+   } T;
+   int64_t *rowptr = (int64_t *)T.get((size_t)(n + 1) * 8), *col = (int64_t *)T.get((size_t)nnz * 8);
+   float *y = (float *)T.get((size_t)ncols * k * 4), *z = (float *)T.get((size_t)n * k * 4);
+   unsigned long long *dbg = (unsigned long long *)T.get((size_t)4 * waves_per_gen * 5 * 8);
+   if (!rowptr || !col || !y || !z || !dbg) return fail(ISPLIB_NOT_ENOUGH_MEM, "stream calibration: device allocation failed");
+   hipLaunchKernelGGL(stream_calib_graph_kernel, dim3(4096), dim3(256), 0, st, n, ncols, (int64_t)degree, rowptr, col);
+   int rc = check_launch("stream_calib_graph_kernel");
+   if (rc) return rc;
+   ISPLIB_HIP_TRY(hipMemsetAsync(y, 0, (size_t)ncols * k * 4, st));
+   int slices = (int)((ncols * k * 4 + 1900000 - 1) / 1900000);
+   if (slices < 1) slices = 1;
+   if ((rc = isplib_stream_plan_build_caps_hip(n, ncols, nnz, rowptr, col, nullptr, streams, slices, 4 * degree, waves_per_gen, nullptr, &T.plan, st)) != ISPLIB_SUCCESS) return rc;
+   if (T.plan.gens != 1 || T.plan.n_hub != 0) return fail(ISPLIB_FAIL, "stream calibration: internal: the synthetic plan is not one generation");
+   std::vector<unsigned long long> h((size_t)waves_per_gen * 5);
+   for (int w = 0; w < waves_per_gen; w++) wave_ticks[w] = 0.0;
+   for (int l = 0; l <= launches; l++) {
+      isplib_debug_wave_times(l ? dbg : nullptr);
+      rc = fusedMM_csr_stream_hip(ISPLIB_MSG_SPMM_SUM, n, ncols, k, nnz, rowptr, rowptr + 1, &T.plan, y, k, z, k, nullptr, 0, nullptr, st);
+      isplib_debug_wave_times(nullptr);
+      if (rc) return rc;
+      if (!l) continue;
+      ISPLIB_HIP_TRY(hipMemcpyAsync(h.data(), dbg, h.size() * 8, hipMemcpyDeviceToHost, st));
+      ISPLIB_HIP_TRY(hipStreamSynchronize(st));
+      for (int w = 0; w < waves_per_gen; w++) wave_ticks[w] += (double)(h[(size_t)w * 5 + 2] - h[(size_t)w * 5 + 1]) / launches;
+   }
+   return ISPLIB_SUCCESS;
+}
+}
+
 extern "C" void isplib_debug_wave_times(unsigned long long *buf) { isplib::g_dbg = buf; isplib::g_dbg_launch = 0; }
-#endif
diff --git a/isplib_amd/csrc/stream_plan.hip b/isplib_amd/csrc/stream_plan.hip
--- a/isplib_amd/csrc/stream_plan.hip
+++ b/isplib_amd/csrc/stream_plan.hip
@@ -2,13 +2,17 @@
 #include <stdint.h>
 #include <string.h>
 
+#include <map>
+#include <mutex>
 #include <new>
+#include <tuple>
 #include <vector>
 
 #include "../../include/isplib_hip.h"
 #include "common.h"
 
 #include "prims.h"
+#include "sweep_common.h"
 
 namespace isplib {
 
@@ -75,6 +79,15 @@
    }
 }
 
+__global__ __launch_bounds__(256) void sp_deal_keys_kernel(int64_t ns, int streams, int waves_per_gen, const uint32_t *__restrict__ loads,
+                                                           const uint32_t *__restrict__ caps, uint32_t *__restrict__ keys) {
+   const int64_t stride = (int64_t)gridDim.x * blockDim.x;
+   for (int64_t s = (int64_t)blockIdx.x * blockDim.x + threadIdx.x; s < ns; s += stride) {
+      const uint64_t key = (uint64_t)loads[s] * ISPLIB_STREAM_CAP_ONE / caps[(s / streams) % waves_per_gen];
+      keys[s] = key > 0xFFFFFFFFull ? 0xFFFFFFFFu : (uint32_t)key;
+   }
+}
+
 __global__ __launch_bounds__(256) void sp_wave_steps_kernel(int64_t nw, int streams, const uint32_t *__restrict__ loads,
                                                             int64_t *__restrict__ steps, int64_t *__restrict__ loads64) {
    const int64_t stride = (int64_t)gridDim.x * blockDim.x;
@@ -230,7 +243,7 @@
 
 static int stream_plan_build(int64_t m, int64_t n, int64_t nnz, const int64_t *rowptr, const int64_t *col, const float *val,
                              int streams, int rpw, int resident, int slices, int chunk, int waves_per_gen,
-                             isplib_stream_plan *out, void *stream, int pad_row = -1) {
+                             isplib_stream_plan *out, void *stream, int pad_row = -1, const uint32_t *caps = nullptr) {
    if (!out) return fail(ISPLIB_FAIL, "isplib_stream_plan_build_hip: out is NULL");
    memset(out, 0, sizeof(*out));
    if (m <= 0 || n <= 0 || nnz < 0 || !rowptr || (nnz > 0 && !col)) return fail(ISPLIB_FAIL, "isplib_stream_plan_build_hip: bad operand");
@@ -240,6 +253,15 @@
    const int per = rpw / streams;
    hipStream_t st = (hipStream_t)stream;
    SpTemp T;
+   if (caps) {
+      bool equal = true;
+      for (int w = 0; w < waves_per_gen; w++) {
+         if (caps[w] < ISPLIB_STREAM_CAP_ONE / 16 || caps[w] > ISPLIB_STREAM_CAP_ONE * 16)
+            return fail(ISPLIB_FAIL, "isplib_stream_plan_build_caps_hip: a capacity outside [ISPLIB_STREAM_CAP_ONE / 16, ISPLIB_STREAM_CAP_ONE * 16]");
+         equal = equal && caps[w] == caps[0];
+      }
+      if (equal) caps = nullptr;
+   }
    int *nchunk, *hub_flag, *first, *hub_idx;
    if (!T.alloc(&nchunk, (size_t)m) || !T.alloc(&hub_flag, (size_t)m) || !T.alloc(&first, (size_t)m + 1) || !T.alloc(&hub_idx, (size_t)m + 1))
       return fail(ISPLIB_NOT_ENOUGH_MEM, "isplib_stream_plan_build_hip: device allocation failed");
@@ -271,12 +293,14 @@
    if (gens > 4096 || ns >= (1LL << 31) || (double)ns * slices * per >= 4294967295.0)
       return fail(ISPLIB_FAIL, "isplib_stream_plan_build_hip: graph too large for this geometry (32-bit stream keys)");
    int *vrow_row, *vlen, *vhub, *part_of, *sid, *rnd;
-   uint32_t *k_in, *k_out, *v_in, *v_out, *loads, *lk_out, *lv_in, *lv_out;
+   uint32_t *k_in, *k_out, *v_in, *v_out, *loads, *lk_out, *lv_in, *lv_out, *lk_in = nullptr, *d_caps = nullptr;
    const size_t big = (size_t)(nnz > nv ? nnz : nv) + 1;
    if (!T.alloc(&vrow_row, (size_t)nv) || !T.alloc(&vlen, (size_t)nv) || !T.alloc(&vhub, (size_t)nv) || !T.alloc(&part_of, (size_t)nv + 1) ||
        !T.alloc(&sid, (size_t)nv) || !T.alloc(&rnd, (size_t)nv) || !T.alloc(&k_in, big) || !T.alloc(&k_out, big) || !T.alloc(&v_in, big) ||
        !T.alloc(&v_out, big) || !T.alloc(&loads, (size_t)ns) || !T.alloc(&lk_out, (size_t)ns) || !T.alloc(&lv_in, (size_t)ns) ||
        !T.alloc(&lv_out, (size_t)ns))
+      return fail(ISPLIB_NOT_ENOUGH_MEM, "isplib_stream_plan_build_hip: device allocation failed");
+   if (caps && (!T.alloc(&lk_in, (size_t)ns) || !T.alloc(&d_caps, (size_t)waves_per_gen)))
       return fail(ISPLIB_NOT_ENOUGH_MEM, "isplib_stream_plan_build_hip: device allocation failed");
    int32_t *hub_row = nullptr, *hub_off = nullptr;
    if (!sp_alloc_out(&hub_row, (size_t)n_hub) || !sp_alloc_out(&hub_off, (size_t)n_hub + 1)) {
@@ -308,12 +332,17 @@
    SP_TRY(hipMemsetAsync(loads, 0, (size_t)ns * sizeof(uint32_t), st));
    hipLaunchKernelGGL(sp_iota_kernel, dim3(sp_grid(ns)), dim3(256), 0, st, ns, lv_in);
    SP_LAUNCHED("sp_iota_kernel");
+   if (caps) SP_TRY(hipMemcpyAsync(d_caps, caps, (size_t)waves_per_gen * sizeof(uint32_t), hipMemcpyHostToDevice, st));
    const int rounds = (int)((nv + ns - 1) / ns);
    if (rounds > per) SP_FAIL(ISPLIB_FAIL, "isplib_stream_plan_build_hip: internal: more rounds than rows per stream");
    for (int r = 0; r < rounds; r++) {
       const int64_t cnt = nv - (int64_t)r * ns < ns ? nv - (int64_t)r * ns : ns;
       tb = sort_small;
-      SP_TRY(sp_sort(sort_tmp, tb, loads, lk_out, lv_in, lv_out, (size_t)ns, 32, st));
+      if (caps) {
+         hipLaunchKernelGGL(sp_deal_keys_kernel, dim3(sp_grid(ns)), dim3(256), 0, st, ns, streams, waves_per_gen, loads, d_caps, lk_in);
+         SP_LAUNCHED("sp_deal_keys_kernel");
+      }
+      SP_TRY(sp_sort(sort_tmp, tb, caps ? lk_in : loads, lk_out, lv_in, lv_out, (size_t)ns, 32, st));
       hipLaunchKernelGGL(sp_deal_kernel, dim3(sp_grid(cnt)), dim3(256), 0, st, cnt, r, v_out + (int64_t)r * ns, lv_out, vlen, sid, rnd, loads);
       SP_LAUNCHED("sp_deal_kernel");
    }
@@ -385,13 +414,92 @@
    return ISPLIB_SUCCESS;
 }
 
+namespace isplib {
+constexpr int SP_CALIB_DEGREE = 512, SP_CALIB_COLS = 2;
+constexpr double SP_CAP_CLAMP = 0.08;
+static std::mutex g_caps_mutex;
+static std::map<std::tuple<int, int, int>, std::vector<uint32_t>> g_caps;
+
+static void caps_from_ticks(int streams, int waves_per_gen, const double *ticks, uint32_t *caps) {
+   const int wgs_per_cu = with_streams<STREAM_SUM>(streams, [&](auto s) {
+      constexpr StreamGeom ge = stream_geom(STREAM_SUM, s());
+      return lds_wgs_per_cu(stream_lds_bytes(ge.lpr, ge.nvmax), ge.wgs);
+   });
+   const int nwg = waves_per_gen / 4;
+   std::vector<double> sum((size_t)8 * wgs_per_cu, 0.0);
+   std::vector<int> cnt((size_t)8 * wgs_per_cu, 0);
+   double all = 0.0;
+   auto group = [&](int w) { const int wg = w / 4; return (wg % 8) * wgs_per_cu + (int)((int64_t)wg * wgs_per_cu / nwg); };
+   for (int w = 0; w < waves_per_gen; w++) { sum[group(w)] += ticks[w]; cnt[group(w)]++; all += ticks[w]; }
+   for (int w = 0; w < waves_per_gen; w++) {
+      double f = all > 0.0 && cnt[group(w)] ? (sum[group(w)] / cnt[group(w)]) / (all / waves_per_gen) - 1.0 : 0.0;
+      f = f > SP_CAP_CLAMP ? SP_CAP_CLAMP : (f < -SP_CAP_CLAMP ? -SP_CAP_CLAMP : f);
+      caps[w] = (uint32_t)((double)ISPLIB_STREAM_CAP_ONE / (1.0 + f) + 0.5);
+   }
+}
+}
+
+extern "C" int isplib_stream_calibrate_raw(int streams, int waves_per_gen, int launches, int degree, int col_mult, double *wave_ticks , void *stream) {
+   clear_error();
+   int rpw = 0, resident = 0;
+   if (isplib_spmm_stream_geometry(streams, &rpw, &resident) != ISPLIB_SUCCESS) return ISPLIB_FAIL;
+   if (!wave_ticks) return fail(ISPLIB_FAIL, "isplib_stream_calibrate_raw: wave_ticks is NULL");
+   std::lock_guard<std::mutex> lock(g_caps_mutex);
+   return stream_kernel_calibrate(streams, waves_per_gen, launches, degree, col_mult, wave_ticks, (hipStream_t)stream);
+}
+
+extern "C" int isplib_stream_capacities_hip(int device, int streams, int waves_per_gen, int64_t nnz, uint32_t *caps, int *levelled, void *stream) {
+   clear_error();
+   if (levelled) *levelled = 0;
+   int rpw = 0, resident = 0;
+   if (isplib_spmm_stream_geometry(streams, &rpw, &resident) != ISPLIB_SUCCESS) return ISPLIB_FAIL;
+   if (waves_per_gen <= 0) waves_per_gen = resident;
+   if (!caps) return fail(ISPLIB_FAIL, "isplib_stream_capacities_hip: caps is NULL");
+   for (int w = 0; w < waves_per_gen; w++) caps[w] = ISPLIB_STREAM_CAP_ONE;
+   const int mode = stream_level_mode();
+   if (mode == 0 || waves_per_gen != resident || resident % 32 != 0 || (mode == 2 && nnz < STREAM_MIN_NNZ)) return ISPLIB_SUCCESS;
+   int current = 0;
+   ISPLIB_HIP_TRY(hipGetDevice(&current));
+   if (device < 0) device = current;
+   std::lock_guard<std::mutex> lock(g_caps_mutex);
+   const auto key = std::make_tuple(device, streams, waves_per_gen);
+   auto it = g_caps.find(key);
+   if (it == g_caps.end()) {
+      std::vector<double> ticks((size_t)waves_per_gen);
+      if (device != current) ISPLIB_HIP_TRY(hipSetDevice(device));
+      const int rc = stream_kernel_calibrate(streams, waves_per_gen, 3, SP_CALIB_DEGREE, SP_CALIB_COLS, ticks.data(), device == current ? (hipStream_t)stream : (hipStream_t) nullptr);
+      if (device != current) (void)hipSetDevice(current);
+      if (rc == ISPLIB_NOT_ENOUGH_MEM) { clear_error(); return ISPLIB_SUCCESS; }
+      if (rc) return rc;
+      std::vector<uint32_t> c((size_t)waves_per_gen);
+      caps_from_ticks(streams, waves_per_gen, ticks.data(), c.data());
+      it = g_caps.emplace(key, std::move(c)).first;
+   }
+   memcpy(caps, it->second.data(), (size_t)waves_per_gen * sizeof(uint32_t));
+   if (levelled) *levelled = 1;
+   return ISPLIB_SUCCESS;
+}
+
+extern "C" int isplib_stream_plan_build_caps_hip(int64_t m, int64_t n, int64_t nnz, const int64_t *rowptr, const int64_t *col,
+                                                 const float *val, int streams, int slices, int chunk, int waves_per_gen,
+                                                 const uint32_t *caps, isplib_stream_plan *out, void *stream) {
+   clear_error();
+   int rpw = 0, resident = 0;
+   if (isplib_spmm_stream_geometry(streams, &rpw, &resident) != ISPLIB_SUCCESS) return ISPLIB_FAIL;
+   return stream_plan_build(m, n, nnz, rowptr, col, val, streams, rpw, resident, slices, chunk, waves_per_gen, out, stream, -1, caps);
+}
+
 extern "C" int isplib_stream_plan_build_hip(int64_t m, int64_t n, int64_t nnz, const int64_t *rowptr, const int64_t *col,
                                             const float *val, int streams, int slices, int chunk, int waves_per_gen,
                                             isplib_stream_plan *out, void *stream) {
    clear_error();
-   int rpw = 0, resident = 0;
+   int rpw = 0, resident = 0, levelled = 0;
    if (isplib_spmm_stream_geometry(streams, &rpw, &resident) != ISPLIB_SUCCESS) return ISPLIB_FAIL;
-   return stream_plan_build(m, n, nnz, rowptr, col, val, streams, rpw, resident, slices, chunk, waves_per_gen, out, stream);
+   std::vector<uint32_t> caps((size_t)(waves_per_gen > 0 ? waves_per_gen : resident));
+   const int rc = isplib_stream_capacities_hip(-1, streams, waves_per_gen, nnz, caps.data(), &levelled, stream);
+   if (rc) return rc;
+   return stream_plan_build(m, n, nnz, rowptr, col, val, streams, rpw, resident, slices, chunk, waves_per_gen, out, stream, -1,
+                            levelled ? caps.data() : nullptr);
 }
 
 __global__ __launch_bounds__(256) void sp_unsorted_kernel(int64_t m, int64_t nnz, const int64_t *__restrict__ rowptr,
diff --git a/isplib_amd/csrc/sweep_common.h b/isplib_amd/csrc/sweep_common.h
--- a/isplib_amd/csrc/sweep_common.h
+++ b/isplib_amd/csrc/sweep_common.h
@@ -107,9 +107,7 @@
    const float *g;
    int64_t ldg;
    float *dval;
-#ifdef ISPLIB_EXP_WAVE_TIMES
    unsigned long long *dbg;
-#endif
    float *part_val;
    int *part_idx;
    const int32_t *hub_row, *hub_off;
diff --git a/isplib_amd/plan.py b/isplib_amd/plan.py
--- a/isplib_amd/plan.py
+++ b/isplib_amd/plan.py
@@ -226,7 +226,8 @@
 
 
 def stream_plan_arrays(rowptr: torch.Tensor, col: torch.Tensor, ncols: int, slices: int, waves_per_gen: int,
-                       rows_per_wave: int = 16, streams: int = 4, chunk: int = 2048, pad_row: Optional[int] = None) -> dict:
+                       rows_per_wave: int = 16, streams: int = 4, chunk: int = 2048, pad_row: Optional[int] = None,
+                       capacities=None) -> dict:
     assert 1 <= slices <= 4096 and streams in (2, 4, 8) and waves_per_gen >= 1
     assert rows_per_wave % streams == 0 and rows_per_wave <= 128
     assert ncols < (1 << 24), "column ids share a 32-bit word with the local row and are multiplied in 24 bits"
@@ -252,17 +253,19 @@
     sid = torch.empty(nv, **i64)
     rnd = torch.empty(nv, **i64)
     loads = torch.zeros(ns, **i64)
-    bias = float(os.environ.get("ISPLIB_EXP_XCD_BIAS", "0"))
-    cost = None
-    if bias != 0.0:
-        blk = (torch.arange(ns, **i64) // streams % waves_per_gen) // 4
-        cost = torch.where(blk % 2 == 0, 1024 + int(round(1024 * bias)), 1024 - int(round(1024 * bias))).to(torch.int64)
+    cap_s = None
+    if capacities is not None:
+        caps = torch.as_tensor(capacities, dtype=torch.int64).to(dev)
+        assert caps.numel() == waves_per_gen and int(caps.min()) >= cabi.STREAM_CAP_ONE // 16 and int(caps.max()) <= cabi.STREAM_CAP_ONE * 16
+        if bool((caps != caps[0]).any()):
+            cap_s = caps[torch.arange(ns, **i64) // streams % waves_per_gen]
     for r in range(-(-nv // ns)):
         items = order[r * ns:(r + 1) * ns]
-        to = torch.sort(loads, stable=True).indices[:items.numel()]
+        keys = loads if cap_s is None else (loads * cabi.STREAM_CAP_ONE // cap_s).clamp(max=2 ** 32 - 1)
+        to = torch.sort(keys, stable=True).indices[:items.numel()]
         sid[items] = to
         rnd[items] = r
-        loads[to] += vlen[items] if cost is None else vlen[items] * cost[to]
+        loads[to] += vlen[items]
     wave, slot = sid // streams, sid % streams
     lrow = slot * per + rnd
     is_hub = nchunk[vrow] > 1
@@ -327,18 +330,19 @@
         rpw, resident = cabi.stream_geometry(streams)
     rows_per_wave = rpw if rows_per_wave is None else rows_per_wave
     waves_per_gen = resident if waves_per_gen is None else waves_per_gen
+    capacities = None if minmax or rows_per_wave != rpw else cabi.stream_capacities(col.device, streams, waves_per_gen, col.numel())
     plan = StreamPlan(**stream_plan_arrays(rowptr, col, ncols, slices, waves_per_gen, rows_per_wave, streams, chunk,
-                                           pad_row=rows_per_wave if minmax else None))
+                                           pad_row=rows_per_wave if minmax else None, capacities=capacities))
     plan.set_values(val)
     return plan
 
 
 def build_stream_plan_native(rowptr: torch.Tensor, col: torch.Tensor, ncols: int, slices: int, streams: int = 4,
-                             chunk: int = 512, minmax: bool = False) -> Optional[StreamPlan]:
+                             chunk: int = 512, minmax: bool = False, waves_per_gen: int = 0, capacities=None) -> Optional[StreamPlan]:
     if ncols >= cabi.STREAM_N_END or col.numel() >= cabi.STREAM_NNZ_END:
         return None
     try:
-        native = cabi.NativeStreamPlan(rowptr, col, None, ncols, streams, slices, chunk, 0, minmax)
+        native = cabi.NativeStreamPlan(rowptr, col, None, ncols, streams, slices, chunk, waves_per_gen, minmax, capacities=capacities)
     except cabi.IsplibError as e:
         if e.status == cabi.ISPLIB_FAIL:
             return None
```

After: 46.37 billion, median of 6. 2.2% higher.
